# tomvanbraeckel/amv-codec-tools

Measured on AMD Instinct MI355X. Metric: AMV frames/sec/GPU (160x120 decode, bit-exact), higher is better.
Workload: dtype int32; 1 GPU; 160x120 AMV decode, 160000-frame synthetic stream per GPU, chunks resident in HBM; parallelism=frame-range x1, frames_per_gpu=160000, stream=seeded synthetic source (BASELINE.md section 4), every frame

## Files before the change

### amv-codec-tools_amd/__init__.py

```python
import ctypes
import os

_HERE = os.path.dirname(os.path.abspath(__file__))
LIB_PATH = os.environ.get("AMVHIP_LIB") or os.path.join(_HERE, "libamvhip.so")

OK, ERR_ARG, ERR_DEVICE, ERR_NOMEM, ERR_SPACE = 0, -1, -2, -3, -4
ST_FORMAT, ST_OVERRUN, ST_TRUNCATED = 1, 2, 4
FLAG_ZIGZAG_FIXED = 1
FLAG_FFMPEG = 2
FLAG_FFMPEG_KEEP = 4
QBIAS_AMV, QBIAS_MJPEG = 0, 128
K_HUFFMAN, K_RECON, K_FDCT, K_PACK, K_ADPCM_DEC, K_ADPCM_ENC, K_SYNTH, K_HUFFMAN_SERIAL, K_UNSTUFF, K_PACK_SERIAL, K_COMPACT = range(11)
K_AUDIO_RESAMPLE = 11
K_PIXFMT = 12
(PIX_YUV420P, PIX_YUVJ420P, PIX_YUV422P, PIX_YUVJ422P, PIX_YUV444P, PIX_YUVJ444P, PIX_YUYV422, PIX_UYVY422, PIX_RGB24, PIX_BGR24,
 PIX_RGB32, PIX_RGB565, PIX_RGB555, PIX_GRAY8) = range(14)
PIX_COUNT = 14
AUDIO_RATE_MIN, AUDIO_RATE_MAX = 1000, 192000
ENTROPY_AUTO, ENTROPY_SERIAL = 0, 1

_vp, _u8p = ctypes.c_void_p, ctypes.c_void_p
_u32, _u64, _i32, _int = ctypes.c_uint32, ctypes.c_uint64, ctypes.c_int32, ctypes.c_int


class AMVInfo(ctypes.Structure):
    _fields_ = [("dwMicroSecPerFrame", ctypes.c_uint), ("dwWidth", ctypes.c_uint), ("dwHeight", ctypes.c_uint),
                ("dwSpeed", ctypes.c_uint), ("dwTimeSec", ctypes.c_uint), ("dwTimeMin", ctypes.c_uint),
                ("dwTimeHour", ctypes.c_uint), ("wFormatTag", ctypes.c_ushort), ("nChannels", ctypes.c_ushort),
                ("nSamplesPerSec", ctypes.c_uint), ("nAvgBytesPerSec", ctypes.c_uint),
                ("nBlockAlign", ctypes.c_ushort), ("wBitsPerSample", ctypes.c_ushort),
                ("cbSize", ctypes.c_ushort), ("wSamplesPerBlock", ctypes.c_ushort)]


class FRAMEBUFF(ctypes.Structure):
    _fields_ = [("videobuff", ctypes.POINTER(ctypes.c_ubyte)), ("audiobuff", ctypes.POINTER(ctypes.c_ubyte)),
                ("videobufflen", ctypes.c_uint), ("audiobufflen", ctypes.c_uint), ("framenum", ctypes.c_int)]


class VIDEOBUFF(ctypes.Structure):
    _fields_ = [("fbmpdat", ctypes.POINTER(ctypes.c_ubyte)), ("len", ctypes.c_uint)]


class AUDIOBUFF(ctypes.Structure):
    _fields_ = [("audiodata", ctypes.POINTER(ctypes.c_short)), ("len", ctypes.c_uint)]


class AMVDecoder(ctypes.Structure):
    _fields_ = [("amvfilename", ctypes.c_char_p), ("opened", ctypes.c_int), ("dataseekpos", ctypes.c_long),
                ("fileseekpos", ctypes.c_long), ("amvinfo", AMVInfo), ("currentframe", ctypes.c_uint),
                ("totalframe", ctypes.c_uint), ("framebuf", FRAMEBUFF), ("videobuf", VIDEOBUFF),
                ("audiobuf", AUDIOBUFF)]


class ADPCMChannelStatus(ctypes.Structure):
    _fields_ = [("predictor", ctypes.c_int), ("step_index", ctypes.c_short), ("step", ctypes.c_int),
                ("prev_sample", ctypes.c_int)]


class ADPCMContext(ctypes.Structure):
    _fields_ = [("channel", ctypes.c_int), ("status", ADPCMChannelStatus * 2), ("sample_buffer", ctypes.c_short * 32)]


SYMBOLS = {
    "PrepareForVideoDecode": (None, [ctypes.POINTER(AMVInfo)]),
    "AmvJpegDecode": (_int, [ctypes.POINTER(AMVInfo), ctypes.POINTER(FRAMEBUFF), ctypes.POINTER(VIDEOBUFF)]),
    "AdpcmImaDecodeFrame": (_int, [ctypes.POINTER(ADPCMContext), _vp, ctypes.POINTER(_int), _vp, _int]),
    "AdpcmImaEncodeFrame": (_int, [ctypes.POINTER(ADPCMContext), _int, _int, _vp, _int, _vp]),
    "AmvOpen": (ctypes.POINTER(AMVDecoder), [ctypes.c_char_p]),
    "AmvClose": (None, [ctypes.POINTER(AMVDecoder)]),
    "AmvReadNextFrame": (_int, [ctypes.POINTER(AMVDecoder)]),
    "AmvRewindFrameStart": (_int, [ctypes.POINTER(AMVDecoder)]),
    "AmvVideoDecode": (_int, [ctypes.POINTER(AMVDecoder)]),
    "AmvAudioDecode": (_int, [ctypes.POINTER(AMVDecoder)]),
    "AmvJpegPutHeader": (None, [_vp, ctypes.c_ushort, ctypes.c_ushort]),
    "AmvCreateJpegFileFromFrameBuffer": (_int, [ctypes.POINTER(AMVDecoder), ctypes.c_char_p]),
    "AmvCreateJpegFileFromBuffer": (_int, [ctypes.POINTER(AMVInfo), ctypes.POINTER(FRAMEBUFF), ctypes.c_char_p]),
    "AmvConvertJpegFileToBmpFile": (_int, [ctypes.c_char_p, ctypes.c_char_p]),
    "ConvertJpegFileToBmpFile": (_int, [ctypes.c_char_p, ctypes.c_char_p]),
    "AmvCreateWavFileFromAmvFile": (_int, [ctypes.POINTER(AMVDecoder), _int, ctypes.c_char_p]),
    "decode_amv_frame": (_int, [_vp, ctypes.c_uint, ctypes.c_uint, ctypes.c_uint, _vp]),
    "encode_amv_frame": (_int, [_vp, ctypes.c_uint, ctypes.c_uint, ctypes.c_uint, _int, _vp, ctypes.c_uint]),
    "amvhip_create": (_int, [ctypes.POINTER(_vp), _int]),
    "amvhip_destroy": (None, [_vp]),
    "amvhip_last_error": (ctypes.c_char_p, [_vp]),
    "amvhip_device": (_int, [_vp]),
    "amvhip_stride": (_u32, [_u32]),
    "amvhip_frame_bytes": (_u64, [_u32, _u32]),
    "amvhip_yuv420_frame_bytes": (_u64, [_u32, _u32]),
    "amvhip_encode_bound": (_u32, [_u32, _u32]),
    "amvhip_jpeg_header": (_u32, [ctypes.c_ushort, ctypes.c_ushort, _vp, _u32]),
    "amvhip_decode_batch_dev": (_int, [_vp, _vp, _u64, _vp, _vp, _u32, _u32, _u32, _u32, _vp, _vp, _vp]),
    "amvhip_decode_submit_dev": (_int, [_vp, _vp, _u64, _vp, _vp, _u32, _u32, _u32, _u32, _vp, _vp, _vp]),
    "amvhip_decode_collect_dev": (_int, [_vp, _vp]),
    "amvhip_decode_workspace_per_frame": (ctypes.c_double, [_vp]),
    "amvhip_decode_batch": (_int, [_vp, _vp, _u64, _vp, _vp, _u32, _u32, _u32, _u32, _vp, _vp]),
    "amvhip_decode_batch_async": (_int, [_vp, _vp, _u64, _vp, _vp, _u32, _u32, _u32, _u32, _vp, _vp]),
    "amvhip_sync": (_int, [_vp]),
    "amvhip_host_alloc": (_int, [_vp, ctypes.POINTER(_vp), ctypes.c_size_t]),
    "amvhip_host_free": (None, [_vp, _vp]),
    "amvhip_huffman_decode_dev": (_int, [_vp, _vp, _u64, _vp, _vp, _u32, _u32, _u32, _vp, _vp, _vp, _vp]),
    "amvhip_reconstruct_dev": (_int, [_vp, _vp, _vp, _u32, _u32, _u32, _u32, _vp, _vp]),
    "amvhip_encode_batch_dev": (_int, [_vp, _vp, _u32, _int, _u32, _u32, _u32, _u32, _vp, _u64, _vp, _vp, _vp]),
    "amvhip_encode_batch": (_int, [_vp, _vp, _u32, _int, _u32, _u32, _u32, _u32, _vp, _u64, _vp, _vp]),
    "amvhip_encode_yuv420_batch_dev": (_int, [_vp, _vp, _vp, _vp, _u32, _u32, _u64, _u64, _u32, _u32, _u32, _u32, _vp, _u64, _vp, _vp, _vp]),
    "amvhip_encode_yuv422_batch_dev": (_int, [_vp, _vp, _vp, _vp, _u32, _u32, _u64, _u64, _u32, _u32, _u32, _u32, _vp, _u64, _vp, _vp, _vp]),
    "amvhip_encode_yuv420_batch": (_int, [_vp, _vp, _vp, _vp, _u32, _u32, _u64, _u64, _u32, _u32, _u32, _u32, _vp, _u64, _vp, _vp]),
    "amvhip_encode_yuv422_batch": (_int, [_vp, _vp, _vp, _vp, _u32, _u32, _u64, _u64, _u32, _u32, _u32, _u32, _vp, _u64, _vp, _vp]),
    "amvhip_encode_nr_max": (_u32, [_u32, _u32]),
    "amvhip_encode_yuv420_nr_stream_dev": (_int, [_vp, _vp, _vp, _vp, _u32, _u32, _u64, _u64, _u32, _u32, _u32, _u32, _u32, _vp, _vp, _u64, _vp, _vp, _vp]),
    "amvhip_encode_yuv420_nr_stream": (_int, [_vp, _vp, _vp, _vp, _u32, _u32, _u64, _u64, _u32, _u32, _u32, _u32, _u32, _vp, _vp, _u64, _vp, _vp]),
    "amvhip_encode_nr_stream_dev": (_int, [_vp, _vp, _u32, _int, _u32, _u32, _u32, _u32, _u32, _vp, _vp, _u64, _vp, _vp, _vp]),
    "amvhip_encode_nr_stream": (_int, [_vp, _vp, _u32, _int, _u32, _u32, _u32, _u32, _u32, _vp, _vp, _u64, _vp, _vp]),
    "amvhip_resample_yuv420_dev": (_int, [_vp, _vp, _vp, _vp, _u32, _u32, _u64, _u64, _u32, _u32, _vp, _vp, _vp, _u32, _u32, _u64, _u64, _u32, _u32, _u32, _vp]),
    "amvhip_encode_yuv420_scaled_batch_dev": (_int, [_vp, _vp, _vp, _vp, _u32, _u32, _u64, _u64, _u32, _u32, _u32, _u32, _u32, _u32, _vp, _u64, _vp, _vp, _vp]),
    "amvhip_img_convert_supported": (_int, [_int, _int, _u32, _u32]),
    "amvhip_pix_frame_bytes": (_u64, [_int, _u32, _u32]),
    "amvhip_img_convert_dev": (_int, [_vp, _int, _vp, _vp, _vp, _u32, _u32, _u64, _u64, _int, _vp, _vp, _vp, _u32, _u32, _u64, _u64, _u32, _u32, _u32, _vp]),
    "amvhip_img_convert": (_int, [_vp, _int, _vp, _vp, _vp, _u32, _u32, _u64, _u64, _int, _vp, _vp, _vp, _u32, _u32, _u64, _u64, _u32, _u32, _u32]),
    "amvhip_sws_scale_dev": (_int, [_vp, _int, _vp, _vp, _vp, _u32, _u32, _u64, _u64, _u32, _u32, _int, _vp, _vp, _vp, _u32, _u32, _u64, _u64, _u32, _u32, _u32, _vp]),
    "amvhip_encode_fmt_scaled_batch_dev": (_int, [_vp, _int, _vp, _vp, _vp, _u32, _u32, _u64, _u64, _u32, _u32, _u32, _u32, _u32, _u32, _vp, _u64, _vp, _vp, _vp]),
    "amvhip_pad_color_from_rgb": (None, [_u32, _vp]),
    "amvhip_deinterlace_supported": (_int, [_int, _u32, _u32]),
    "amvhip_deinterlace_dev": (_int, [_vp, _int, _vp, _vp, _vp, _u32, _u32, _u64, _u64, _vp, _vp, _vp, _u32, _u32, _u64, _u64, _u32, _u32, _u32, _vp]),
    "amvhip_deinterlace": (_int, [_vp, _int, _vp, _vp, _vp, _u32, _u32, _u64, _u64, _vp, _vp, _vp, _u32, _u32, _u64, _u64, _u32, _u32, _u32]),
    "amvhip_video_frontend_dev": (_int, [_vp, _int, _vp, _vp, _vp, _u32, _u32, _u64, _u64, _u32, _u32, _u32, _vp, _vp, _vp, _vp, _u32, _u32, _u64, _u64, _u32, _u32, _vp]),
    "amvhip_encode_frontend_batch_dev": (_int, [_vp, _int, _vp, _vp, _vp, _u32, _u32, _u64, _u64, _u32, _u32, _u32, _vp, _u32, _u32, _u32, _vp, _u64, _vp, _vp, _vp]),
    "amvhip_decode_fmt_batch_dev": (_int, [_vp, _vp, _u64, _vp, _vp, _u32, _u32, _u32, _u32, _int, _vp, _u32, _vp, _vp]),
    "amvhip_lowres_dim": (_u32, [_u32, _u32]),
    "amvhip_lowres_frame_bytes": (_u64, [_u32, _u32, _u32]),
    "amvhip_decode_lowres_batch_dev": (_int, [_vp, _vp, _u64, _vp, _vp, _u32, _u32, _u32, _u32, _u32, _int, _vp, _u32, _vp, _vp]),
    "amvhip_decode_lowres_batch": (_int, [_vp, _vp, _u64, _vp, _vp, _u32, _u32, _u32, _u32, _u32, _int, _vp, _u32, _vp]),
    "amvhip_reconstruct_lowres_dev": (_int, [_vp, _vp, _vp, _u32, _u32, _u32, _u32, _vp, _vp]),
    "amvhip_audio_resample_out_samples": (_u64, [_u32, _u32, _u64]),
    "amvhip_audio_resample_batch_dev": (_int, [_vp, _vp, _vp, _vp, _u32, _u32, _u32, _vp, _vp, _u32, _u32, _vp]),
    "amvhip_audio_resample_batch": (_int, [_vp, _vp, _u64, _vp, _vp, _u32, _u32, _u32, _vp, _u64, _vp, _u32, _u32]),
    "amvhip_audio_resample_init": (_vp, [_vp, _int, _int, _int, _int]),
    "amvhip_audio_resample": (_int, [_vp, _vp, _vp, _int]),
    "amvhip_audio_resample_close": (None, [_vp]),
    "amvhip_encode_coefs_dev": (_int, [_vp, _vp, _u32, _int, _u32, _u32, _u32, _u32, _vp, _vp]),
    "amvhip_adpcm_decode_batch_dev": (_int, [_vp, _vp, _u64, _vp, _vp, _u32, _vp, _vp, _vp, _vp]),
    "amvhip_adpcm_encode_batch_dev": (_int, [_vp, _vp, _vp, _vp, _u32, _vp, _vp, _vp, _vp]),
    "amvhip_adpcm_decode_batch": (_int, [_vp, _vp, _u64, _vp, _vp, _u32, _vp, _u64, _vp, _vp]),
    "amvhip_adpcm_decode_batch_async": (_int, [_vp, _vp, _u64, _vp, _vp, _u32, _vp, _u64, _vp, _vp]),
    "amvhip_adpcm_encode_batch": (_int, [_vp, _vp, _u64, _vp, _vp, _u32, _vp, _vp, _u64, _vp]),
    "amvhip_adpcm_encode_frame": (_int, [_vp, _vp, _u32, ctypes.POINTER(_i32), _vp, _u32]),
    "amvhip_adpcm_encode_trellis_batch_dev": (_int, [_vp, _vp, _vp, _vp, _u32, _vp, _u32, _vp, _vp, _vp, _vp]),
    "amvhip_adpcm_encode_frame_trellis": (_int, [_vp, _vp, _u32, ctypes.POINTER(_i32), _u32, _vp, _u32]),
    "amvhip_adpcm_encode_trellis_stream_dev": (_int, [_vp, _vp, _vp, _vp, _u32, _i32, _u32, _vp, _vp, _vp, _vp]),
    "amvhip_adpcm_encode_trellis_stream": (_int, [_vp, _vp, _u64, _vp, _vp, _u32, _i32, _u32, _vp, _u64, _vp, _vp]),
    "amvhip_adpcm_trellis_chain_stats": (_int, [_vp, _vp]),
    "amvhip_amv_audio_pairs": (_u32, [_u32, _u32, ctypes.POINTER(_u32), ctypes.POINTER(_u64)]),
    "amvhip_amv_audio_frame_size": (_u32, [_u32, _u32, _u32]),
    "amvhip_adpcm_wav_encode_frame": (_int, [_vp, _vp, _int, _vp, _vp, _int]),
    "amvhip_synth_frames_dev": (_int, [_vp, _u32, _u32, _u32, _u32, _u32, _vp, _vp]),
    "amvhip_synth_audio_dev": (_int, [_vp, _u32, _u64, _u64, _vp, _vp]),
    "amvhip_set_entropy_mode": (_int, [_vp, _int]),
    "amvhip_entropy_stats": (_int, [_vp, _int, _vp]),
    "amvhip_entropy_trace": (_int, [_vp, _vp, _u32]),
    "amvhip_decode_split_stats": (_int, [_vp, _vp]),
    "amvhip_adpcm_chain_stats": (_int, [_vp, _vp]),
    "amvhip_adpcm_quotient_table": (None, [_vp]),
    "amvhip_prof_enable": (None, [_vp, _int]),
    "amvhip_prof_reset": (None, [_vp]),
    "amvhip_prof_read": (_int, [_vp, _int, ctypes.POINTER(_u64), ctypes.POINTER(ctypes.c_double)]),
    "amvhip_kernel_name": (ctypes.c_char_p, [_int]),
    "amvhip_mux_open": (_vp, [ctypes.c_char_p, _u32, _u32, _u32, _u32, _u32, _u32]),
    "amvhip_mux_write_frame": (_int, [_vp, _u8p, _u32, _u8p, _u32]),
    "amvhip_mux_close": (_int, [_vp]),
}

_lib = None


def load_library():
    global _lib
    if _lib is None:
        if not os.path.exists(LIB_PATH):
            raise RuntimeError(
                "libamvhip.so is not built (%s). Run `python amv-codec-tools_amd/build.py`; there is no CPU fallback."
                % LIB_PATH)
        try:
            import torch
        except ImportError:
            pass
        lib = ctypes.CDLL(LIB_PATH)
        for name, (res, args) in SYMBOLS.items():
            fn = getattr(lib, name)
            fn.restype = res
            fn.argtypes = args
        _lib = lib
    return _lib


class AmvHipError(RuntimeError):
    pass


class Frontend(ctypes.Structure):
    _fields_ = [("deinterlace", _u32), ("crop_top", _u32), ("crop_bottom", _u32), ("crop_left", _u32), ("crop_right", _u32),
                ("pad_top", _u32), ("pad_bottom", _u32), ("pad_left", _u32), ("pad_right", _u32), ("pad_color", ctypes.c_uint8 * 3)]

    def __init__(self, deinterlace=0, crop=(0, 0, 0, 0), pad=(0, 0, 0, 0), pad_color=(16, 128, 128)):
        super().__init__(int(deinterlace), *crop, *pad, (ctypes.c_uint8 * 3)(*pad_color))


def pad_color_from_rgb(rrggbb):
    out = (ctypes.c_uint8 * 3)()
    load_library().amvhip_pad_color_from_rgb(rrggbb, ctypes.cast(out, ctypes.c_void_p))
    return tuple(out)


def _ptr(x):
    if x is None:
        return None
    if isinstance(x, int):
        return x
    if hasattr(x, "data_ptr"):
        return x.data_ptr()
    if hasattr(x, "ctypes"):
        return x.ctypes.data
    if isinstance(x, bytes):
        return ctypes.cast(ctypes.c_char_p(x), ctypes.c_void_p).value
    raise TypeError("pass a torch tensor, numpy array, bytes or int address, not %s" % type(x).__name__)


class Context:

    def __init__(self, device=0):
        self.lib = load_library()
        h = ctypes.c_void_p()
        rc = self.lib.amvhip_create(ctypes.byref(h), int(device))
        if rc != OK:
            raise AmvHipError("amvhip_create(device=%d) failed with %d: no usable HIP device" % (device, rc))
        self.h = h

    def close(self):
        if getattr(self, "h", None):
            self.lib.amvhip_destroy(self.h)
            self.h = None

    __del__ = close

    def _check(self, rc, what):
        if rc < 0:
            raise AmvHipError("%s failed (%d): %s" % (what, rc, self.lib.amvhip_last_error(self.h).decode()))
        return rc

    def stride(self, w):
        return self.lib.amvhip_stride(w)

    def frame_bytes(self, w, h):
        return self.lib.amvhip_frame_bytes(w, h)

    def yuv420_frame_bytes(self, w, h):
        return self.lib.amvhip_yuv420_frame_bytes(w, h)

    def encode_bound(self, w, h):
        return self.lib.amvhip_encode_bound(w, h)

    def decode_batch_dev(self, blob, blob_bytes, offs, lens, n, w, h, flags, out, status, stream=None):
        return self._check(self.lib.amvhip_decode_batch_dev(self.h, _ptr(blob), blob_bytes, _ptr(offs), _ptr(lens), n,
                                                            w, h, flags, _ptr(out), _ptr(status), stream), "decode_batch_dev")

    def decode_submit_dev(self, blob, blob_bytes, offs, lens, n, w, h, flags, out, status, stream=None):
        return self._check(self.lib.amvhip_decode_submit_dev(self.h, _ptr(blob), blob_bytes, _ptr(offs), _ptr(lens), n,
                                                             w, h, flags, _ptr(out), _ptr(status), stream), "decode_submit_dev")

    def decode_collect_dev(self, stream=None):
        return self._check(self.lib.amvhip_decode_collect_dev(self.h, stream), "decode_collect_dev")

    def decode_workspace_per_frame(self):
        return self.lib.amvhip_decode_workspace_per_frame(self.h)

    def huffman_decode_dev(self, blob, blob_bytes, offs, lens, n, w, h, coef, status, nmcu_ok, stream=None):
        return self._check(self.lib.amvhip_huffman_decode_dev(self.h, _ptr(blob), blob_bytes, _ptr(offs), _ptr(lens), n,
                                                              w, h, _ptr(coef), _ptr(status), _ptr(nmcu_ok), stream),
                           "huffman_decode_dev")

    def reconstruct_dev(self, coef, nmcu_ok, n, w, h, flags, out, stream=None):
        return self._check(self.lib.amvhip_reconstruct_dev(self.h, _ptr(coef), _ptr(nmcu_ok), n, w, h, flags,
                                                           _ptr(out), stream), "reconstruct_dev")

    def encode_batch_dev(self, pix, pix_stride, is_bgr, n, w, h, qbias, blob, blob_cap, offs, lens, stream=None):
        return self._check(self.lib.amvhip_encode_batch_dev(self.h, _ptr(pix), pix_stride, is_bgr, n, w, h, qbias,
                                                            _ptr(blob), blob_cap, _ptr(offs), _ptr(lens), stream),
                           "encode_batch_dev")

    def encode_yuv420_batch_dev(self, y, cb, cr, y_stride, c_stride, y_frame, c_frame, n, w, h, qbias, blob, blob_cap, offs,
                                lens, stream=None):
        return self._check(self.lib.amvhip_encode_yuv420_batch_dev(self.h, _ptr(y), _ptr(cb), _ptr(cr), y_stride, c_stride,
                                                                   y_frame, c_frame, n, w, h, qbias, _ptr(blob), blob_cap,
                                                                   _ptr(offs), _ptr(lens), stream), "encode_yuv420_batch_dev")

    def encode_nr_max(self, w, h):
        return self.lib.amvhip_encode_nr_max(w, h)

    def encode_yuv420_nr_stream_dev(self, y, cb, cr, y_stride, c_stride, y_frame, c_frame, n, w, h, qbias, nr, state, blob, blob_cap,
                                    offs, lens, stream=None):
        return self._check(self.lib.amvhip_encode_yuv420_nr_stream_dev(self.h, _ptr(y), _ptr(cb), _ptr(cr), y_stride, c_stride,
                                                                       y_frame, c_frame, n, w, h, qbias, nr, _ptr(state), _ptr(blob),
                                                                       blob_cap, _ptr(offs), _ptr(lens), stream),
                           "encode_yuv420_nr_stream_dev")

    def encode_yuv420_nr_stream(self, y, cb, cr, y_stride, c_stride, y_frame, c_frame, n, w, h, qbias, nr, state, blob, blob_cap, offs,
                                lens):
        return self._check(self.lib.amvhip_encode_yuv420_nr_stream(self.h, _ptr(y), _ptr(cb), _ptr(cr), y_stride, c_stride,
                                                                   y_frame, c_frame, n, w, h, qbias, nr, _ptr(state), _ptr(blob),
                                                                   blob_cap, _ptr(offs), _ptr(lens)), "encode_yuv420_nr_stream")

    def encode_nr_stream_dev(self, pix, pix_stride, is_bgr, n, w, h, qbias, nr, state, blob, blob_cap, offs, lens, stream=None):
        return self._check(self.lib.amvhip_encode_nr_stream_dev(self.h, _ptr(pix), pix_stride, is_bgr, n, w, h, qbias, nr,
                                                                _ptr(state), _ptr(blob), blob_cap, _ptr(offs), _ptr(lens), stream),
# ... 35 lines not shown
                           "adpcm_encode_batch_dev")

    def adpcm_encode_trellis_stream_dev(self, pcm, pcm_offs, nsamp, n, first_step_index, trellis, blob, offs, step_out=None,
                                        stream=None):
        return self._check(self.lib.amvhip_adpcm_encode_trellis_stream_dev(self.h, _ptr(pcm), _ptr(pcm_offs), _ptr(nsamp), n,
                                                                           first_step_index, trellis, _ptr(blob), _ptr(offs),
                                                                           _ptr(step_out), stream),
                           "adpcm_encode_trellis_stream_dev")

    @staticmethod
    def _pic(pic):
        planes, stride, c_stride, frame, c_frame = pic
        planes = list(planes) + [None] * (3 - len(planes))
        return [_ptr(planes[0]), _ptr(planes[1]), _ptr(planes[2]), stride, c_stride, frame, c_frame]

    def img_convert_dev(self, src_fmt, src, dst_fmt, dst, w, h, n, stream=None):
        return self._check(self.lib.amvhip_img_convert_dev(self.h, src_fmt, *self._pic(src), dst_fmt, *self._pic(dst), w, h, n, stream),
                           "img_convert_dev")

    def img_convert(self, src_fmt, src, dst_fmt, dst, w, h, n):
        return self._check(self.lib.amvhip_img_convert(self.h, src_fmt, *self._pic(src), dst_fmt, *self._pic(dst), w, h, n), "img_convert")

    def sws_scale_dev(self, src_fmt, src, src_w, src_h, dst_fmt, dst, dst_w, dst_h, n, stream=None):
        return self._check(self.lib.amvhip_sws_scale_dev(self.h, src_fmt, *self._pic(src), src_w, src_h, dst_fmt, *self._pic(dst),
                                                         dst_w, dst_h, n, stream), "sws_scale_dev")

    def encode_fmt_scaled_batch_dev(self, src_fmt, src, src_w, src_h, n, w, h, qbias, blob, blob_cap, offs, lens, stream=None):
        return self._check(self.lib.amvhip_encode_fmt_scaled_batch_dev(self.h, src_fmt, *self._pic(src), src_w, src_h, n, w, h, qbias,
                                                                       _ptr(blob), blob_cap, _ptr(offs), _ptr(lens), stream),
                           "encode_fmt_scaled_batch_dev")

    @staticmethod
    def _fe(fe):
        return None if fe is None else ctypes.addressof(fe)

    def pad_color_from_rgb(self, rrggbb):
        return pad_color_from_rgb(rrggbb)

    def deinterlace_supported(self, fmt, w, h):
        return self.lib.amvhip_deinterlace_supported(fmt, w, h)

    def deinterlace_dev(self, fmt, src, dst, w, h, n, stream=None):
        return self._check(self.lib.amvhip_deinterlace_dev(self.h, fmt, *self._pic(src), *self._pic(dst), w, h, n, stream), "deinterlace_dev")

    def deinterlace(self, fmt, src, dst, w, h, n):
        return self._check(self.lib.amvhip_deinterlace(self.h, fmt, *self._pic(src), *self._pic(dst), w, h, n), "deinterlace")

    def video_frontend_dev(self, src_fmt, src, src_w, src_h, n, fe, dst, w, h, stream=None):
        return self._check(self.lib.amvhip_video_frontend_dev(self.h, src_fmt, *self._pic(src), src_w, src_h, n, self._fe(fe), *self._pic(dst),
                                                              w, h, stream), "video_frontend_dev")

    def encode_frontend_batch_dev(self, src_fmt, src, src_w, src_h, n, fe, w, h, qbias, blob, blob_cap, offs, lens, stream=None):
        return self._check(self.lib.amvhip_encode_frontend_batch_dev(self.h, src_fmt, *self._pic(src), src_w, src_h, n, self._fe(fe), w, h,
                                                                     qbias, _ptr(blob), blob_cap, _ptr(offs), _ptr(lens), stream),
                           "encode_frontend_batch_dev")

    def decode_fmt_batch_dev(self, blob, blob_bytes, offs, lens, n, w, h, flags, dst_fmt, out, out_stride, status, stream=None):
        return self._check(self.lib.amvhip_decode_fmt_batch_dev(self.h, _ptr(blob), blob_bytes, _ptr(offs), _ptr(lens), n, w, h, flags,
                                                                dst_fmt, _ptr(out), out_stride, _ptr(status), stream),
                           "decode_fmt_batch_dev")

    def lowres_dim(self, full, lowres):
        return self.lib.amvhip_lowres_dim(full, lowres)

    def lowres_frame_bytes(self, w, h, lowres):
        return self.lib.amvhip_lowres_frame_bytes(w, h, lowres)

    def decode_lowres_batch_dev(self, blob, blob_bytes, offs, lens, n, w, h, flags, lowres, dst_fmt, out, out_stride, status, stream=None):
        return self._check(self.lib.amvhip_decode_lowres_batch_dev(self.h, _ptr(blob), blob_bytes, _ptr(offs), _ptr(lens), n, w, h, flags,
                                                                   lowres, dst_fmt, _ptr(out), out_stride, _ptr(status), stream),
                           "decode_lowres_batch_dev")

    def decode_lowres_batch(self, blob, blob_bytes, offs, lens, n, w, h, flags, lowres, dst_fmt, out, out_stride, status):
        return self._check(self.lib.amvhip_decode_lowres_batch(self.h, _ptr(blob), blob_bytes, _ptr(offs), _ptr(lens), n, w, h, flags,
                                                               lowres, dst_fmt, _ptr(out), out_stride, _ptr(status)), "decode_lowres_batch")

    def reconstruct_lowres_dev(self, coef, nmcu_ok, n, w, h, lowres, out, stream=None):
        return self._check(self.lib.amvhip_reconstruct_lowres_dev(self.h, _ptr(coef), _ptr(nmcu_ok), n, w, h, lowres, _ptr(out), stream),
                           "reconstruct_lowres_dev")

    def audio_resample_out_samples(self, in_rate, out_rate, in_samples):
        return audio_resample_out_samples(in_rate, out_rate, in_samples)

    def audio_resample_batch_dev(self, pcm, pcm_offs, nsamp, n, in_channels, in_rate, out, out_offs, out_channels, out_rate,
                                 stream=None):
        return self._check(self.lib.amvhip_audio_resample_batch_dev(self.h, _ptr(pcm), _ptr(pcm_offs), _ptr(nsamp), n,
                                                                    in_channels, in_rate, _ptr(out), _ptr(out_offs),
                                                                    out_channels, out_rate, stream), "audio_resample_batch_dev")

    def audio_resampler(self, output_channels, input_channels, output_rate, input_rate):
        return AudioResampler(self, output_channels, input_channels, output_rate, input_rate)

    def synth_frames_dev(self, seed, first, n, w, h, rgb, stream=None):
        return self._check(self.lib.amvhip_synth_frames_dev(self.h, seed, first, n, w, h, _ptr(rgb), stream), "synth_frames_dev")

    def synth_audio_dev(self, seed, first, n, pcm, stream=None):
        return self._check(self.lib.amvhip_synth_audio_dev(self.h, seed, first, n, _ptr(pcm), stream), "synth_audio_dev")

    def decode_batch(self, blob, blob_bytes, offs, lens, n, w, h, flags, out, status):
        return self._check(self.lib.amvhip_decode_batch(self.h, _ptr(blob), blob_bytes, _ptr(offs), _ptr(lens), n, w, h,
                                                        flags, _ptr(out), _ptr(status)), "decode_batch")

    def encode_batch(self, pix, pix_stride, is_bgr, n, w, h, qbias, blob, blob_cap, offs, lens):
        return self._check(self.lib.amvhip_encode_batch(self.h, _ptr(pix), pix_stride, is_bgr, n, w, h, qbias, _ptr(blob),
                                                        blob_cap, _ptr(offs), _ptr(lens)), "encode_batch")

    def adpcm_decode_batch(self, blob, blob_bytes, offs, lens, n, pcm, pcm_samples, pcm_offs, final_state=None):
        return self._check(self.lib.amvhip_adpcm_decode_batch(self.h, _ptr(blob), blob_bytes, _ptr(offs), _ptr(lens), n,
                                                              _ptr(pcm), pcm_samples, _ptr(pcm_offs), _ptr(final_state)),
                           "adpcm_decode_batch")

    def adpcm_encode_batch(self, pcm, pcm_samples, pcm_offs, nsamp, n, step_in, blob, blob_bytes, offs):
        return self._check(self.lib.amvhip_adpcm_encode_batch(self.h, _ptr(pcm), pcm_samples, _ptr(pcm_offs), _ptr(nsamp),
                                                              n, _ptr(step_in), _ptr(blob), blob_bytes, _ptr(offs)),
                           "adpcm_encode_batch")

    def adpcm_encode_trellis_stream(self, pcm, pcm_samples, pcm_offs, nsamp, n, first_step_index, trellis, blob, blob_bytes, offs,
                                    step_out=None):
        return self._check(self.lib.amvhip_adpcm_encode_trellis_stream(self.h, _ptr(pcm), pcm_samples, _ptr(pcm_offs), _ptr(nsamp),
                                                                       n, first_step_index, trellis, _ptr(blob), blob_bytes,
                                                                       _ptr(offs), _ptr(step_out)),
                           "adpcm_encode_trellis_stream")

    def audio_resample_batch(self, pcm, pcm_samples, pcm_offs, nsamp, n, in_channels, in_rate, out, out_samples, out_offs,
                             out_channels, out_rate):
        return self._check(self.lib.amvhip_audio_resample_batch(self.h, _ptr(pcm), pcm_samples, _ptr(pcm_offs), _ptr(nsamp), n,
                                                                in_channels, in_rate, _ptr(out), out_samples, _ptr(out_offs),
                                                                out_channels, out_rate), "audio_resample_batch")

    def set_entropy_mode(self, mode):
        return self._check(self.lib.amvhip_set_entropy_mode(self.h, mode), "set_entropy_mode")

    def entropy_stats(self, enable=True):
        out = (ctypes.c_uint64 * 10)()
        self._check(self.lib.amvhip_entropy_stats(self.h, 1 if enable else 0, out), "entropy_stats")
        waves = max(out[9], 1)
        return {"frames": out[0], "rounds": out[1], "max_rounds": out[2], "handed_to_serial": out[3], "waves": out[9],
                "clocks_per_wave": {"zero": out[4] / waves, "first_walk": out[5] / waves, "sync_rounds": out[6] / waves,
                                    "write": out[7] / waves, "dc": out[8] / waves}}

    def entropy_trace(self, tasks):
        import numpy as np
        out = np.zeros((tasks, 8), np.uint64)
        got = self.lib.amvhip_entropy_trace(self.h, out.ctypes.data, tasks)
        if got < 0:
            self._check(got, "entropy_trace")
        return out[:got]

    def decode_split_stats(self):
        out = (ctypes.c_uint32 * 2)()
        self._check(self.lib.amvhip_decode_split_stats(self.h, out), "decode_split_stats")
        return {"heavy": int(out[0]), "light": int(out[1])}

    def adpcm_chain_stats(self):
        out = (ctypes.c_uint32 * 64)()
        self._check(self.lib.amvhip_adpcm_chain_stats(self.h, out), "adpcm_chain_stats")
        rec = list(out[1:63])
        while rec and rec[-1] == 0:
            rec.pop()
        return {"exhaustive": bool(out[0]), "recoded": rec}

    def adpcm_trellis_chain_stats(self):
        out = (ctypes.c_uint32 * 64)()
        self._check(self.lib.amvhip_adpcm_trellis_chain_stats(self.h, out), "adpcm_trellis_chain_stats")
        rec = list(out[1:63])
        while rec and rec[-1] == 0:
            rec.pop()
        return {"exhaustive": bool(out[0]), "recoded": rec}

    def prof_enable(self, on=True):
        self.lib.amvhip_prof_enable(self.h, 1 if on else 0)

    def prof_reset(self):
        self.lib.amvhip_prof_reset(self.h)

    def prof_read(self, kernel):
        n, ms = ctypes.c_uint64(), ctypes.c_double()
        self.lib.amvhip_prof_read(self.h, kernel, ctypes.byref(n), ctypes.byref(ms))
        return n.value, ms.value

    def kernel_name(self, kernel):
        return self.lib.amvhip_kernel_name(kernel).decode()


def audio_resample_out_samples(in_rate, out_rate, in_samples):
    return load_library().amvhip_audio_resample_out_samples(in_rate, out_rate, in_samples)


class AudioResampler:

    def __init__(self, ctx, output_channels, input_channels, output_rate, input_rate):
        self.ctx, self.out_ch, self.in_ch = ctx, output_channels, input_channels
        self.ratio = ctypes.c_float(ctypes.c_float(output_rate).value / ctypes.c_float(input_rate).value).value
        self.h = ctx.lib.amvhip_audio_resample_init(ctx.h, output_channels, input_channels, output_rate, input_rate)
        if not self.h:
            raise AmvHipError("amvhip_audio_resample_init failed: %s" % ctx.lib.amvhip_last_error(ctx.h).decode())

    def resample(self, pcm):
        import numpy as np
        pcm = np.ascontiguousarray(pcm, np.int16)
        nb = pcm.size // self.in_ch
        out = np.zeros((int(4 * nb * self.ratio) + 18) * self.out_ch, np.int16)
        got = self.ctx._check(self.ctx.lib.amvhip_audio_resample(self.h, out.ctypes.data, pcm.ctypes.data, nb), "audio_resample")
        return out[:got * self.out_ch]

    def close(self):
        if getattr(self, "h", None):
            self.ctx.lib.amvhip_audio_resample_close(self.h)
            self.h = None

    __del__ = close
```

### amv-codec-tools_amd/build.py

```python
import concurrent.futures
import os
import shutil
import subprocess
import sys

HERE = os.path.dirname(os.path.abspath(__file__))
OUT = os.path.join(HERE, "libamvhip.so")
OBJ = os.path.join(HERE, "build")
ARCH = "gfx950"

HIP_SOURCES = ["csrc/amv_decode.hip", "csrc/amv_decode_sync.hip", "csrc/amv_reconstruct.hip", "csrc/amv_reconstruct_ff.hip", "csrc/amv_reconstruct_lowres.hip", "csrc/amv_encode.hip", "csrc/amv_encode_par.hip", "csrc/amv_encode_nr.hip", "csrc/amv_resample.hip", "csrc/amv_pixfmt.hip", "csrc/amv_frontend.hip", "csrc/amv_audio_resample.hip", "csrc/amv_adpcm.hip", "csrc/amv_synth.hip",
               "csrc/amvhip_context.hip", "csrc/amvhip_decode.hip", "csrc/amvhip_encode.hip", "csrc/amvhip_pixfmt.hip", "csrc/amvhip_audio.hip"]
C_SOURCES = ["host/amvlib_compat.c", "host/amv_container.c"]
HEADERS = ["csrc/amv_tables.h", "csrc/amv_kernels.h", "csrc/amv_block_load.h", "csrc/amv_piece_map.h", "csrc/amv_segment.h", "csrc/amv_ff_dequant.h", "csrc/amv_encode_common.h", "csrc/amv_host_plan.h", "csrc/amv_nr_plan.h",
           "csrc/amvhip_ctx.h", "../include/amvhip.h"]

HIPFLAGS = ["-O3", "-std=c++17", "-fPIC", "-fwrapv", "-fno-strict-aliasing", f"--offload-arch={ARCH}",
            "-Wall", "-Wno-unused-function"]
CFLAGS = ["-O2", "-fPIC", "-Wall", "-Wextra", "-std=gnu11"]


def _hipcc():
    for cand in (shutil.which("hipcc"), "/opt/rocm/bin/hipcc"):
        if cand and os.path.exists(cand):
            return cand
    raise RuntimeError("hipcc not found: libamvhip.so cannot be built (there is no CPU fallback)")


def _stale(target, deps):
    if not os.path.exists(target):
        return True
    t = os.path.getmtime(target)
    return any(os.path.getmtime(d) > t for d in deps)


def _run(cmd):
    p = subprocess.run(cmd, cwd=HERE, capture_output=True, text=True)
    if p.returncode != 0:
        raise RuntimeError("command failed: %s\n%s\n%s" % (" ".join(cmd), p.stdout, p.stderr))
    return p.stderr


def build(force=False, verbose=False):
    os.makedirs(OBJ, exist_ok=True)
    hipcc = _hipcc()
    hdrs = [os.path.join(HERE, h) for h in HEADERS] + [os.path.abspath(__file__)]
    jobs = []
    objs = []
    for src in HIP_SOURCES:
        o = os.path.join(OBJ, os.path.basename(src) + ".o")
        objs.append(o)
        if force or _stale(o, [os.path.join(HERE, src)] + hdrs):
            jobs.append([hipcc] + HIPFLAGS + ["-c", src, "-o", o])
    for src in C_SOURCES:
        o = os.path.join(OBJ, os.path.basename(src) + ".o")
        objs.append(o)
        if force or _stale(o, [os.path.join(HERE, src)] + hdrs):
            jobs.append(["gcc"] + CFLAGS + ["-c", src, "-o", o])
    if jobs:
        with concurrent.futures.ThreadPoolExecutor(max_workers=4) as ex:
            for warn in ex.map(_run, jobs):
                if verbose and warn:
                    sys.stderr.write(warn)
    if jobs or force or _stale(OUT, objs):
        _run([hipcc, "-shared", "-fPIC", f"--offload-arch={ARCH}", "-o", OUT] + objs + ["-lpthread"])
    return OUT


if __name__ == "__main__":
    print(build(force="--force" in sys.argv, verbose=True))
```

### amv-codec-tools_amd/csrc/amv_block_load.h

```cpp
#pragma once
#include <cstdlib>

#include "amv_kernels.h"
#include "amv_piece_map.h"

namespace amv {

constexpr uint32_t kSegImageBytes = 60u * 128u;
constexpr uint32_t kScatterSwizzleMask = 0x38u;
constexpr uint32_t kScatterFieldShift = 6u;
constexpr uint32_t kScatterAddressMask = 0x11ffeu;

__device__ __forceinline__ void seg_sync() {
    __builtin_amdgcn_fence(__ATOMIC_SEQ_CST, "wavefront");
    __builtin_amdgcn_wave_barrier();
}

__device__ __forceinline__ bool select_frame(const FrameSel& sel, uint32_t n, uint32_t item, uint32_t& f, uint32_t& slot) {
    f = slot = item;
    if (!sel.round) return true;
    const uint32_t p = sel.base + item;
    if (item >= sel.round || p >= (sel.count ? *sel.count : n)) return false;
    f = sel.list ? sel.list[p] : p;
    return true;
}

struct Segment {
    uint32_t f, slot;
    uint32_t m0, cnt, ok, mcu0;
    uint32_t segidx, nsegs;
};
__device__ __forceinline__ Segment segment_of(uint32_t f, uint32_t slot, const uint32_t* __restrict__ nmcu_ok, const FrameGeom& g,
                                              uint32_t nseg, uint32_t my, uint32_t seg) {
    const uint32_t m0 = seg * kSegMcus;
    return {f, slot, m0, min(kSegMcus, g.mcu_cols - m0), nmcu_ok[f], my * g.mcu_cols + m0, my * nseg + seg, g.mcu_rows * nseg};
}
template <bool kRound>
__device__ __forceinline__ bool next_item(const PieceMap& pm, uint32_t& item) {
    if (!kRound) return false;
    seg_sync();
    item += piece_stride(pm);
    return true;
}

__device__ __forceinline__ bool load_segment_blocks(const SyncSinks& in, const Segment& sg, bool dense_only, const FrameGeom& g,
                                                    uint32_t lane, uint8_t* s_img, uint32_t (&c)[32], bool& skip) {
    const uint32_t f = sg.f, slot = sg.slot, segidx = sg.segidx, nsegs = sg.nsegs, mcu0 = sg.mcu0, cnt = sg.cnt, ok = sg.ok;
    const uint32_t nb = cnt * 6u;
    uint32_t rc = 0xffffffffu, r0 = 0u, r1 = 0u;
    if (in.rec != nullptr && !dense_only) {
        const uint32_t* ss = in.seg_start + ((uint64_t)f * (nsegs + 1u) + segidx) * 2u;
        rc = in.rec_count[f];
        r0 = ss[0];
        r1 = ss[3];
    }
    const bool records = rc != 0xffffffffu;
    skip = !records && in.rec != nullptr && !dense_only;
    if (skip) return false;
    int dc_base = 0;
    if (records) {
        const uint32_t ok_blocks = in.ok_in_blocks ? ok : ok * 6u;
        const uint32_t blocks_ok_here = ok_blocks > mcu0 * 6u ? min(nb, ok_blocks - mcu0 * 6u) : 0u;
        if (!blocks_ok_here) r1 = r0;
        struct __attribute__((packed, aligned(4))) Rec4 { uint32_t w[4]; };
        constexpr uint32_t kAhead = 3;
        const uint32_t* rec = in.rec + (uint64_t)in.rec_line[f] * 32u + r0;
        const uint32_t nrec = r1 - r0;
        Rec4 q[kAhead];
#pragma unroll
        for (uint32_t j = 0; j < kAhead; ++j) {
            const uint32_t i = j * 4u * kWave + lane * 4u;
            q[j] = Rec4{{kDummyRecord, kDummyRecord, kDummyRecord, kDummyRecord}};
            if (i < nrec) q[j] = *reinterpret_cast<const Rec4*>(rec + i);
        }
        uint4* img16 = reinterpret_cast<uint4*>(s_img);
        for (uint32_t i = lane; i < nb * 8u; i += kWave) img16[i] = make_uint4(0, 0, 0, 0);
        seg_sync();
        const uint32_t field0 = (mcu0 * 6u - g.blocks) & 63u;
        const uint32_t first6 = (uint32_t)__builtin_amdgcn_readfirstlane((int)((64u - field0) << kScatterFieldShift));
        const uint32_t ok7 = blocks_ok_here << 7;
        const uint32_t spare = kSegImageBytes + lane * 2u;
        for (uint32_t base = 0;;) {
#pragma unroll
            for (uint32_t j = 0; j < kAhead; ++j) {
                if (base + j * 4u * kWave >= nrec) break;
                if (base + (j + 1u) * 4u * kWave > nrec) {
                    const int32_t left = (int32_t)(nrec - base - j * 4u * kWave) - (int32_t)(lane * 4u);
#pragma unroll
                    for (uint32_t e = 0; e < 4u; ++e)
                        if (left <= (int32_t)e) q[j].w[e] = kDummyRecord;
                }
#pragma unroll
                for (uint32_t e = 0; e < 4u; ++e) {
                    const uint32_t w = q[j].w[e];
                    uint32_t t;
                    asm("v_add_lshl_u32 %0, %1, %2, 1" : "=v"(t) : "v"(w ^ ((w >> 3) & kScatterSwizzleMask)), "s"(first6));
                    const uint32_t at = t & kScatterAddressMask;
                    *reinterpret_cast<int16_t*>(s_img + (at < ok7 ? at : spare)) = (int16_t)(w >> 16);
                }
            }
            base += kAhead * 4u * kWave;
            if (base >= nrec) break;
#pragma unroll
            for (uint32_t j = 0; j < kAhead; ++j) {
                const uint32_t i = base + j * 4u * kWave + lane * 4u;
                if (i < nrec) q[j] = *reinterpret_cast<const Rec4*>(rec + i);
            }
        }
        const uint32_t frame_lanes = ((rc >> 24) & 63u) + 1u;
        if (frame_lanes > 1u) {
            const uint32_t babs = mcu0 * 6u + lane, k6 = lane % 6u;
            const uint4 ent = lane < frame_lanes ? reinterpret_cast<const uint4*>(in.lane_tab)[(uint64_t)f * in.lanes + lane]
                                                 : make_uint4(0xffffffffu, 0u, 0u, 0u);
            uint32_t at = 0u;
#pragma unroll
            for (uint32_t step = 32u; step >= 1u; step >>= 1) {
                const uint32_t probe = at + step;
                const uint32_t first = (uint32_t)__shfl((int)ent.x, (int)(probe & 63u));
                if (probe < frame_lanes && first <= babs) at = probe;
            }
            const int by = __shfl((int)ent.y, (int)at), bu = __shfl((int)ent.z, (int)at), bv = __shfl((int)ent.w, (int)at);
            dc_base = at ? (k6 < 4u ? by : (k6 == 4u ? bu : bv)) : 0;
        }
        seg_sync();
    }
    if (lane >= nb) return false;
    if (records) {
        const uint4* src = reinterpret_cast<const uint4*>(s_img) + lane * 8u;
        const uint32_t swz = (lane + mcu0 * 6u - g.blocks) & 7u;
#pragma unroll
        for (int i = 0; i < 8; ++i) {
            const uint4 q = src[(uint32_t)i ^ swz];
            c[4 * i] = q.x; c[4 * i + 1] = q.y; c[4 * i + 2] = q.z; c[4 * i + 3] = q.w;
        }
        c[0] = (c[0] & 0xffff0000u) | ((c[0] + (uint32_t)dc_base) & 0xffffu);
    } else {
        const uint4* src = reinterpret_cast<const uint4*>(in.coef + (((uint64_t)slot * g.mcus + mcu0) * 6u + lane) * 64u);
#pragma unroll
        for (int i = 0; i < 8; ++i) {
            const uint4 q = src[i];
            c[4 * i] = q.x; c[4 * i + 1] = q.y; c[4 * i + 2] = q.z; c[4 * i + 3] = q.w;
        }
    }
    return true;
}

__device__ __forceinline__ int coef_at(const uint32_t (&c)[32], int i) {
    return (i & 1) ? ((int)c[i >> 1] >> 16) : (int)(int16_t)(c[i >> 1] & 0xffffu);
}

template <class Kernel, class... Tail>
static inline void launch_segments(Kernel part, Kernel walk, uint32_t block, uint32_t row_groups, const SyncSinks& sinks, const uint32_t* nmcu_ok,
                            uint32_t n, const FrameSel& sel, uint32_t items, const FrameGeom& g, hipStream_t s, Tail... tail) {
    for_each_launch(row_groups, segs_per_row(g), items, sel.round != 0u, [&](const PieceMap& pm, uint32_t grid) {
        hipLaunchKernelGGL(sel.round ? walk : part, dim3(grid), dim3(block), 0, s, sinks, nmcu_ok, n, sel, g, pm, tail...);
    });
}

}
```

### amv-codec-tools_amd/csrc/amv_decode_sync.hip

```cpp
#include <atomic>

#include "amv_kernels.h"
#include "amv_segment.h"

namespace amv {

namespace {

constexpr uint32_t kRingWords = 16;
constexpr uint32_t kNever = 0xffffffffu;

__device__ __forceinline__ void wave_sync() {
    __builtin_amdgcn_fence(__ATOMIC_SEQ_CST, "wavefront");
    __builtin_amdgcn_wave_barrier();
}

template <int kWidth>
__device__ __forceinline__ uint32_t seg_excl_sum(uint32_t v, uint32_t sub, uint32_t& total) {
    uint32_t x = v;
#pragma unroll
    for (int d = 1; d < kWidth; d <<= 1) {
        const uint32_t y = __shfl_up(x, d, kWidth);
        if (sub >= (uint32_t)d) x += y;
    }
// ... 145 lines not shown
        }
    }
    if (lane == 0) {
        ws_bytes[frame] = retry ? kNever : total;
        if (retry) retry_list[atomicAdd(retry_count, 1u)] = frame;
    }
}

namespace {

struct Stream {
    const uint32_t* g;
    uint32_t nwords;
    uint32_t* ring;
    uint32_t hi;
    uint4 pf0, pf1;
};

constexpr int kStrideWrite = 8;

__device__ __forceinline__ uint4 stream_piece(const Stream& s, uint32_t x) {
    uint4 v = make_uint4(0, 0, 0, 0);
    if (x < s.nwords) v = *reinterpret_cast<const uint4*>(s.g + x);
    return v;
}

__device__ __forceinline__ void stream_request(Stream& s) {
    s.pf0 = stream_piece(s, s.hi);
    s.pf1 = stream_piece(s, s.hi + 4u);
}

struct SegGeom {
    uint32_t mcu_cols;
    uint32_t per_row;
    uint32_t count;
};

template <uint32_t kFlush>
__device__ __forceinline__ void stage_put(uint32_t* stage, uint32_t pos, uint32_t word) {
    stage[(pos & (2u * kFlush - 1u)) * kWave] = word;
}

template <uint32_t kFlush>
__device__ __forceinline__ void stage_flush(const uint32_t* stage, uint32_t* __restrict__ rec, uint32_t from, uint32_t rec_cap) {
    const uint32_t* p = stage + (from & (2u * kFlush - 1u)) * kWave;
    uint4 v[kFlush / 4u];
#pragma unroll
    for (uint32_t q = 0; q < kFlush / 4u; ++q)
        v[q] = make_uint4(p[(4u * q) * kWave], p[(4u * q + 1u) * kWave], p[(4u * q + 2u) * kWave], p[(4u * q + 3u) * kWave]);
    if (from + kFlush <= rec_cap) {
#pragma unroll
        for (uint32_t q = 0; q < kFlush / 4u; ++q) *reinterpret_cast<uint4*>(rec + from + 4u * q) = v[q];
    }
}

}

struct SyncOut {
    uint32_t* rec;
    const uint32_t* rec_line;
    uint32_t* seg_start;
    uint32_t* lane_tab;
    SegGeom sg;
    uint32_t lane_stride;
    uint32_t* rec_count;
    uint32_t* retry_list;
    uint32_t* retry_count;
    uint32_t ok_in_blocks;
};


namespace {

constexpr uint32_t kFastRegion = kFastWords * 4u;
constexpr uint32_t kFastTableBytes = 4u * kFastRegion;
constexpr uint32_t kServicePace = 4u;
template <int L> constexpr uint32_t skip_pace() { return L >= 16 ? 1u : kServicePace; }
constexpr uint32_t kSlot = kWave * 4u;
constexpr uint32_t kFastRingBytes = (kRingWords + 1u) * kSlot;
constexpr uint32_t kFastSumBytes = 4u * kSlot;
constexpr uint32_t fast_stage_bytes(uint32_t flush) { return 2u * flush * kSlot; }
constexpr uint32_t fast_per_wave(uint32_t flush) { return fast_stage_bytes(flush) + kFastSumBytes + kFastRingBytes; }
constexpr uint32_t fast_waves(uint32_t flush) {
    const uint32_t w = (160u * 1024u - kFastTableBytes) / fast_per_wave(flush);
    return w > 16u ? 16u : w;
}

struct FastState {
    uint32_t t;
    uint32_t k;
    uint32_t j;
    uint32_t togo6;
    uint32_t rp8;
    uint32_t dc;
};

typedef __attribute__((address_space(3))) uint32_t lds_u32;
__device__ __forceinline__ uint32_t lds_get(uint32_t a) { return *(const lds_u32*)(uintptr_t)a; }
__device__ __forceinline__ void lds_put(uint32_t a, uint32_t v) { *(lds_u32*)(uintptr_t)a = v; }
__device__ __forceinline__ uint32_t shl3_add(uint32_t x, uint32_t y) {
    uint32_t d;
    asm("v_lshl_add_u32 %0, %1, 3, %2" : "=v"(d) : "v"(x), "v"(y));
    return d;
}

__device__ __forceinline__ void fast_ring_put(const Stream& s, uint32_t x, const uint4& v) {
    uint32_t* d = s.ring + (x & (kRingWords - 1u)) * kWave;
    d[0] = v.x; d[kWave] = v.y; d[2 * kWave] = v.z; d[3 * kWave] = v.w;
    if ((x & (kRingWords - 1u)) == 0u) s.ring[kRingWords * kWave] = v.x;
}

__device__ __forceinline__ void fast_open(Stream& s) {
    const uint4 a = stream_piece(s, 0u), b = stream_piece(s, 4u), c = stream_piece(s, 8u), d = stream_piece(s, 12u);
    fast_ring_put(s, 0u, a);
    fast_ring_put(s, 4u, b);
    fast_ring_put(s, 8u, c);
    fast_ring_put(s, 12u, d);
    s.hi = kRingWords;
    stream_request(s);
}

template <uint32_t kPace>
__device__ __forceinline__ void fast_service_paced(Stream& s, uint32_t w, bool alive, bool& have, uint32_t stride_no) {
    if (alive && w + 9u > s.hi) {
        do {
            if (!have) stream_request(s);
            fast_ring_put(s, s.hi, s.pf0);
            fast_ring_put(s, s.hi + 4u, s.pf1);
            s.hi += 8u;
            have = false;
        } while (w + 9u > s.hi);
    }
    if ((stride_no & (kPace - 1u)) == 0u) {
        if (alive && !have) {
            stream_request(s);
            have = true;
        }
    }
}

__device__ __forceinline__ uint32_t fast_window(uint32_t ringb, uint32_t t) {
    const uint32_t ra = shl3_add(t & 0x1e0u, ringb);
    return __builtin_amdgcn_alignbit(lds_get(ra), lds_get(ra + kSlot), ~t);
}

__device__ __forceinline__ uint32_t fast_lookup(const FastState& s, uint32_t v) {
    const uint32_t toff = (((3u * kFastRegion) >> s.j) & kFastRegion) | (~s.dc & (2u * kFastRegion));
    const uint32_t e1 = lds_get(((v >> 21) & 0x7fcu) | toff);
    const uint32_t x2 = max(v >> 16, kFastLongFirst - 1u);
    const uint32_t e2 = lds_get((x2 << 2) + (toff + (kFastM2Word * 4u - 4u * (kFastLongFirst - 1u))));
    return e1 | e2;
}

template <uint32_t kFlush, bool kLimit>
__device__ __forceinline__ void fast_stride(uint32_t ringb, uint32_t stageb, uint32_t sumb, uint32_t lim1, FastState& s, uint32_t& seen,
                                            uint32_t& worst) {
#pragma unroll
    for (int it = 0; it < kStrideWrite; ++it) {
        const uint32_t ca = (((2u * kSlot) >> s.j) & (3u * kSlot)) | sumb;
        const uint32_t sum = lds_get(ca);
        const uint32_t v = fast_window(ringb, s.t);
        __builtin_amdgcn_sched_barrier(0);
        uint32_t run = (uint32_t)((int32_t)s.togo6 >> 31);
        if (kLimit) run &= (uint32_t)((int32_t)(s.t - lim1) >> 31);
        const uint32_t e = fast_lookup(s, v) & run;
        seen |= e;
        const uint32_t used = e >> 24;
        const int x = __builtin_amdgcn_sbfe((int)v, 0u - used, e);
        const uint32_t full = __builtin_amdgcn_ubfe(0xffffffffu, 0u, e);
        const uint32_t val = (uint32_t)x - (full ^ (uint32_t)(x >> 31));
        s.t += used;
        const uint32_t kn = s.k + ((e >> 16) & 255u);
        worst = min(worst, kn - 65u);
        uint32_t dcn = (uint32_t)__builtin_amdgcn_sbfe((int)kn, 6u, 1u);
        asm("" : "+v"(dcn));
        lds_put(ca, sum + (val & s.dc));
        const uint32_t rv = val + (sum & s.dc);
        lds_put((s.rp8 & ((2u * kFlush - 1u) << 8)) | stageb, (rv << 16) | (s.togo6 & 0xfc0u) | (kn - 1u));
        s.rp8 += e & kFastEmit;
        s.k = kn & ~dcn;
        s.togo6 += kn & 64u;
        s.j = min(s.j + dcn, 5u);
        s.dc = dcn;
    }
}

template <bool kLimit>
__device__ __forceinline__ uint32_t fast_replay(uint32_t ringb, uint32_t lim1, FastState& s) {
    for (int it = 0; it < kStrideWrite; ++it) {
        if (s.togo6 == 0u) break;
        if (kLimit && (int32_t)(s.t - lim1) >= 0) break;
        const uint32_t e = fast_lookup(s, fast_window(ringb, s.t));
        if (e & kFastInvalid) return 1u;
        const uint32_t kn = s.k + ((e >> 16) & 255u);
        s.t += e >> 24;
        if (kn - 65u < 15u) return 2u;
        const bool end = (kn & 64u) != 0u;
        s.rp8 += e & kFastEmit;
        s.k = end ? 0u : kn;
        s.togo6 += kn & 64u;
        s.j = end ? (s.j == 0u ? 5u : s.j - 1u) : s.j;
        s.dc = end ? ~0u : 0u;
    }
    return 0u;
}

__device__ __forceinline__ void fast_open_at(Stream& s, uint32_t w) {
    const uint32_t lo = w & ~7u;
    const uint4 a = stream_piece(s, lo), b = stream_piece(s, lo + 4u), c = stream_piece(s, lo + 8u), d = stream_piece(s, lo + 12u);
    fast_ring_put(s, lo, a);
    fast_ring_put(s, lo + 4u, b);
    fast_ring_put(s, lo + 8u, c);
    fast_ring_put(s, lo + 12u, d);
    s.hi = lo + kRingWords;
    stream_request(s);
}

template <uint32_t kPace>
__device__ __forceinline__ void fast_skip(Stream& win, uint32_t ringb, FastState& s, uint32_t lim1, uint32_t& nblk6, uint32_t& nrec8) {
    nblk6 = nrec8 = 0u;
    bool active = (int32_t)(s.t - lim1) < 0;
    if (!__ballot(active)) return;
    fast_open_at(win, active ? (s.t + 1u) >> 5 : 0u);
    bool have = true;
    uint32_t stride_no = 1u;
    while (__ballot(active) != 0ull) {
        fast_service_paced<kPace>(win, (s.t + 1u) >> 5, active, have, stride_no++);
#pragma unroll
        for (int it = 0; it < kStrideWrite; ++it) {
            const uint32_t v = fast_window(ringb, s.t);
            const uint32_t e = fast_lookup(s, v) & (uint32_t)((int32_t)(s.t - lim1) >> 31);
            s.t += e >> 24;
            const uint32_t kn = s.k + ((e >> 16) & 255u);
            uint32_t dcn = (uint32_t)__builtin_amdgcn_sbfe((int)kn, 6u, 1u);
            asm("" : "+v"(dcn));
            nrec8 += e & kFastEmit;
            nblk6 += kn & 64u;
            s.k = kn & ~dcn;
            s.j = min(s.j + dcn, 5u);
            s.dc = dcn;
        }
        active = (int32_t)(s.t - lim1) < 0;
    }
}

}

template <uint32_t kFlush>
__global__ __launch_bounds__(kWave * 16) void amv_huffman_fast_kernel(
    const uint32_t* __restrict__ ws, const uint32_t* __restrict__ ws_bytes, uint32_t n,
    const uint32_t* __restrict__ list, const uint32_t* __restrict__ list_count,
    uint32_t blocks_per_frame, const uint32_t* __restrict__ ws_line,
    const HuffDecodeImage* __restrict__ img, SyncOut out, int32_t* __restrict__ status,
    uint32_t* __restrict__ nmcu_ok, uint32_t* __restrict__ queue, unsigned long long* __restrict__ stats) {
    static_assert(kFlush == 8u, "amv_huffman_fast_kernel stages a stride's eight record slots");
    extern __shared__ __attribute__((aligned(16))) uint8_t s_mem[];
    const uint32_t wave = threadIdx.x >> 6, lane = threadIdx.x & 63u, nwaves = blockDim.x >> 6;
    {
        const uint4* src = reinterpret_cast<const uint4*>(&img->fast[0][0]);
        uint4* dst = reinterpret_cast<uint4*>(s_mem);
        for (uint32_t i = threadIdx.x; i < kFastTableBytes / 16u; i += blockDim.x) dst[i] = src[i];
    }
    __syncthreads();
    const bool lds_at_zero = (uint32_t)(uintptr_t)(__attribute__((address_space(3))) uint8_t*)s_mem == 0u;
    const uint32_t stageb = kFastTableBytes + wave * fast_stage_bytes(kFlush) + lane * 4u;
    const uint32_t sumb = kFastTableBytes + nwaves * fast_stage_bytes(kFlush) + wave * kFastSumBytes + lane * 4u;
    const uint32_t ringb = kFastTableBytes + nwaves * (fast_stage_bytes(kFlush) + kFastSumBytes) + wave * kFastRingBytes + lane * 4u;
    uint32_t* const stage = reinterpret_cast<uint32_t*>(s_mem + stageb);
    if (list) n = *list_count;
    const uint32_t ntasks = (n + kWave - 1) / kWave;
    const SegGeom sg = out.sg;
    for (;;) {
        uint32_t task = 0;
        if (lane == 0) task = atomicAdd(queue, 1u);
        task = __shfl(task, 0);
        if (task >= ntasks) return;
        const uint32_t idx = task * kWave + lane;
        const uint32_t frame = idx < n ? (list ? list[idx] : idx) : kNever;
        uint32_t total = frame != kNever ? ws_bytes[frame] : kNever;
        if (!lds_at_zero && total != kNever) {
            out.retry_list[atomicAdd(out.retry_count, 1u)] = frame;
            total = kNever;
        }
        if (frame != kNever && total == kNever) out.rec_count[frame] = kNever;
        if (!lds_at_zero) continue;
        const bool live = total != kNever;
        const uint32_t fsafe = live ? frame : 0u;
        const uint32_t line0 = out.rec_line[fsafe];
        uint32_t* const rec = out.rec + (uint64_t)line0 * 32u;
        const uint32_t line1 = out.rec_line[fsafe + 1u];
        const uint32_t cap_rec = line1 > line0 ? (line1 - line0) * 32u : 0u;
        uint2* const seg_out = reinterpret_cast<uint2*>(out.seg_start) + (uint64_t)fsafe * (sg.count + 1u);
        const uint32_t valid_bits = live ? total * 8u : 0u;
        Stream win{ws + (uint64_t)ws_line[fsafe] * 4u, live ? ((total + 15u) >> 4) * 4u : 0u, reinterpret_cast<uint32_t*>(s_mem + ringb), 0u,
                   make_uint4(0, 0, 0, 0), make_uint4(0, 0, 0, 0)};
        fast_open(win);
        for (uint32_t c = 0; c < 3u; ++c) lds_put(sumb + c * kSlot, 0u);

        FastState s{0xffffffffu, 0u, 5u, live ? 0u - (blocks_per_frame << 6) : 0u, 0u, ~0u};
        bool alive = live;
        uint32_t stop = 0;
        uint32_t stride_no = 0;
        bool have_words = true;
        uint32_t recpos = 0;
        uint32_t seg_next = 0, seg_col = 0, seg_blk = 0;
        uint32_t end_blocks = 0;
#pragma unroll
        for (uint32_t q = 0; q < 2u * kFlush; ++q) stage_put<kFlush>(stage, q, kDummyRecord);
        if (__ballot(alive) != 0ull) do {
            const bool line_live = alive;
            uint4 line[8];
#pragma unroll
            for (int quarter = 0; quarter < 4; ++quarter) {
                fast_service_paced<kServicePace>(win, (s.t + 1u) >> 5, alive, have_words, stride_no);
                const bool running = alive;
                s.rp8 = stride_no << 11;
                const FastState start = s;
                uint32_t worst = ~0u, seen = 0u;
                fast_stride<kFlush, false>(ringb, stageb, sumb, 0u, s, seen, worst);
                const bool trouble = alive && (worst < 15u || (seen & kFastInvalid) != 0u);
                if (__ballot(trouble) != 0ull) {
                    if (trouble) {
                        s = start;
                        stop = fast_replay<false>(ringb, 0u, s);
                        alive = false;
                        for (uint32_t q = s.rp8 >> 8; q < stride_no * 8u + 8u; ++q) stage_put<kFlush>(stage, q, kDummyRecord);
                    }
                }
                if (alive && s.togo6 == 0u) { stop = 3u; alive = false; }
                stage_put<kFlush>(stage, s.rp8 >> 8, kDummyRecord);
                {
                    uint32_t* p = stage + ((stride_no & 1u) * kFlush) * kWave;
                    line[2 * quarter] = make_uint4(p[0], p[kWave], p[2 * kWave], p[3 * kWave]);
                    line[2 * quarter + 1] = make_uint4(p[4 * kWave], p[5 * kWave], p[6 * kWave], p[7 * kWave]);
#pragma unroll
                    for (uint32_t q = 0; q < 8u; ++q) p[q * kWave] = kDummyRecord;
                }
                bool hit = false;
                uint32_t blocks = 0;
                if (running) {
                    blocks = blocks_per_frame + (uint32_t)((int32_t)s.togo6 >> 6);
                    hit = seg_next < sg.count && blocks + (s.k ? 1u : 0u) > seg_blk;
                    if (!alive) { end_blocks = blocks; s.togo6 = 0u; }
                }
                if (__ballot(hit) != 0ull) {
                    if (hit) {
                        seg_out[seg_next++] = make_uint2(start.rp8 >> 8, s.rp8 >> 8);
                        const bool last = seg_col + 1u == sg.per_row;
                        seg_blk += 6u * (last ? sg.mcu_cols - seg_col * kSegMcus : kSegMcus);
                        seg_col = last ? 0u : seg_col + 1u;
                    }
                }
                ++stride_no;
            }
            if (line_live) {
                const uint32_t at = (stride_no - 4u) * 8u;
                if (at + 32u <= cap_rec) {
                    uint4* d = reinterpret_cast<uint4*>(rec + at);
#pragma unroll
                    for (int q = 0; q < 8; ++q) d[q] = line[q];
                }
                recpos = at + 32u;
            }
        } while (__ballot(alive) != 0ull);
        if (live) {
            const uint32_t bits = s.t + 1u + (stop == 1u ? 17u : 0u);
            uint32_t st = stop == 1u ? kStFormat : (stop == 2u ? kStOverrun : 0u);
            if (bits > valid_bits) st |= kStTruncated;
            reinterpret_cast<uint4*>(out.lane_tab)[(uint64_t)frame * out.lane_stride] = make_uint4(0u, 0u, 0u, 0u);
            for (uint32_t m = seg_next; m <= sg.count; ++m) seg_out[m] = make_uint2(recpos, recpos);
            if (stats) atomicAdd(&stats[0], 1ull);
            if (recpos > cap_rec) {
                out.rec_count[frame] = kNever;
                out.retry_list[atomicAdd(out.retry_count, 1u)] = frame;
            } else {
                status[frame] = (int32_t)st;
                nmcu_ok[frame] = out.ok_in_blocks ? end_blocks : end_blocks / 6u;
                out.rec_count[frame] = recpos;
            }
        }
    }
}

template <int L>
__global__ __launch_bounds__(kWave * 16) void amv_huffman_sync2_kernel(
    const uint32_t* __restrict__ ws, const uint32_t* __restrict__ ws_bytes, uint32_t n,
    const uint32_t* __restrict__ list, const uint32_t* __restrict__ list_count,
    uint32_t blocks_per_frame, const uint32_t* __restrict__ ws_line,
    const HuffDecodeImage* __restrict__ img, SyncOut out, int32_t* __restrict__ status,
    uint32_t* __restrict__ nmcu_ok, uint32_t* __restrict__ queue, unsigned long long* __restrict__ stats) {
    constexpr int kFrames = kWave / L;
    constexpr uint32_t kFlush = 8u;
    constexpr uint32_t kNoLimit = 0x7ffffffeu;
    extern __shared__ __attribute__((aligned(16))) uint8_t s_mem[];
    const uint32_t wave = threadIdx.x >> 6, lane = threadIdx.x & 63u, nwaves = blockDim.x >> 6;
    const uint32_t slot = lane / L, sub = lane % L;
    if (list && *list_count == 0u) return;
    {
        const uint4* src = reinterpret_cast<const uint4*>(&img->fast[0][0]);
        uint4* dst = reinterpret_cast<uint4*>(s_mem);
        for (uint32_t i = threadIdx.x; i < kFastTableBytes / 16u; i += blockDim.x) dst[i] = src[i];
    }
    __syncthreads();
    const bool lds_at_zero = (uint32_t)(uintptr_t)(__attribute__((address_space(3))) uint8_t*)s_mem == 0u;
    const uint32_t stageb = kFastTableBytes + wave * fast_stage_bytes(kFlush) + lane * 4u;
    const uint32_t sumb = kFastTableBytes + nwaves * fast_stage_bytes(kFlush) + wave * kFastSumBytes + lane * 4u;
    const uint32_t ringb = kFastTableBytes + nwaves * (fast_stage_bytes(kFlush) + kFastSumBytes) + wave * kFastRingBytes + lane * 4u;
    uint32_t* const stage = reinterpret_cast<uint32_t*>(s_mem + stageb);
    if (list) n = *list_count;
    const uint32_t ntasks = (n + kFrames - 1) / kFrames;
    const SegGeom sg = out.sg;
    for (;;) {
        uint32_t task = 0;
        if (lane == 0) task = atomicAdd(queue, 1u);
        task = __shfl(task, 0);
        if (task >= ntasks) return;

        const bool timing = stats != nullptr && lane == 0;
        unsigned long long tc[6] = {0, 0, 0, 0, 0, 0};
        unsigned long long wall0 = 0;
        if (timing) { tc[0] = tc[1] = clock64(); wall0 = wall_clock64(); }

        const uint32_t idx = task * kFrames + slot;
        const uint32_t frame = idx < n ? (list ? list[idx] : idx) : kNever;
        uint32_t total = frame != kNever ? ws_bytes[frame] : kNever;
        if (!lds_at_zero && total != kNever) {
            if (sub == 0) out.retry_list[atomicAdd(out.retry_count, 1u)] = frame;
            total = kNever;
        }
        if (frame != kNever && total == kNever && sub == 0) out.rec_count[frame] = kNever;
        if (!lds_at_zero) continue;
        const bool live = total != kNever;
        const uint32_t fsafe = live ? frame : 0u;
        const uint32_t line0 = out.rec_line[fsafe];
        uint32_t* const rec = out.rec + (uint64_t)line0 * 32u;
        const uint32_t line1 = out.rec_line[fsafe + 1u];
        const uint32_t cap_rec = line1 > line0 ? (line1 - line0) * 32u : 0u;
        uint2* const seg_out = reinterpret_cast<uint2*>(out.seg_start) + (uint64_t)fsafe * (sg.count + 1u);
        const uint32_t valid_bits = live ? total * 8u : 0u;
        Stream win{ws + (uint64_t)ws_line[fsafe] * 4u, live ? ((total + 15u) >> 4) * 4u : 0u, reinterpret_cast<uint32_t*>(s_mem + ringb), 0u,
                   make_uint4(0, 0, 0, 0), make_uint4(0, 0, 0, 0)};

        uint32_t S = ((valid_bits + L - 1) / L + 31u) & ~31u;
        if (S < 64u) S = 64u;
        constexpr uint32_t kMemo = 5u, kPend = 4u;
        constexpr uint32_t kGuess = 5u << 11;
        const uint32_t stage0 = stageb - lane * 4u, sum0 = sumb - lane * 4u, col0 = slot * L;
        const uint64_t seg = L == 64 ? ~0ull : (((1ull << (L & 63)) - 1ull) << (slot * L));
        auto col_addr = [&](uint32_t col, uint32_t w) { return (w < 16u ? stage0 + w * kSlot : sum0 + (w - 16u) * kSlot) + col * 4u; };
        const bool walks = live && sub != L - 1;
        uint32_t my_blocks6 = 0u, my_recs8 = 0u, seeded = 0u, rounds = 0u;
        lds_put(col_addr(lane, 19u), 0u);
        {
            FastState st{sub * S - 1u, 0u, 5u, 0u, 0u, ~0u};
            const uint32_t lim1 = walks ? (sub + 1u) * S - 1u : 0u;
            if (!walks) st.t = lim1;
            uint32_t b6, r8;
            fast_skip<skip_pace<L>()>(win, ringb, st, lim1, b6, r8);
            if (walks) {
                lds_put(col_addr(lane, 0u), kGuess | (((st.t - lim1) | (st.k << 5) | (st.j << 11)) << 16));
                lds_put(col_addr(lane, 1u), b6);
                lds_put(col_addr(lane, 2u), r8);
                lds_put(col_addr(lane, 19u), 1u);
            }
        }
        if (timing) tc[2] = clock64();
        constexpr uint32_t kNone = 7u;
        uint32_t final_at = kNone, final_code = kGuess;
        bool settled = !live;
        for (int round = 0; round < L + 1; ++round) {
            wave_sync();
            const uint32_t held = lds_get(col_addr(lane, 19u));
            const uint32_t left_n = sub ? lds_get(col_addr(lane - 1u, 19u)) : 0u;
            uint32_t mine[kMemo], cand[kMemo];
#pragma unroll
            for (uint32_t q = 0; q < kMemo; ++q) {
                const uint32_t a = lds_get(col_addr(lane, 3u * q)), b = lds_get(col_addr(sub ? lane - 1u : lane, 3u * q));
                mine[q] = q < held ? a : kNever;
                cand[q] = q < left_n ? b >> 16 : kNever;
            }
            uint32_t link = (kNone << 15) | (kNone << 18) | (kNone << 21);
#pragma unroll
            for (uint32_t qp = 0; qp < kMemo; ++qp) {
                uint32_t to = kNone;
#pragma unroll
                for (uint32_t q = 0; q < kMemo; ++q) to = (mine[q] != kNever && (mine[q] & 0xffffu) == cand[qp]) ? q : to;
                if (sub == L - 1) to = cand[qp] != kNever ? 0u : kNone;
                link |= to << (3u * qp);
            }
            if (sub == 0) link = 0u;
            if (!live) link = 0u;
#pragma unroll
            for (int d = 1; d < L; d <<= 1) {
                const uint32_t before = __shfl_up(link, d, L);
                uint32_t both = 0u;
#pragma unroll
                for (uint32_t f = 0; f < 8u; ++f) both |= ((link >> (3u * ((before >> (3u * f)) & 7u))) & 7u) << (3u * f);
                if (sub >= (uint32_t)d) link = both;
            }
            final_at = link & 7u;
            const uint32_t left_at = wave_shr1(final_at);
            settled = !live || final_at != kNone;
            const bool front = live && !settled && sub != 0 && left_at != kNone;
            if (sub == 0) final_code = kGuess;
            else {
#pragma unroll
                for (uint32_t q = 0; q < kMemo; ++q) if (left_at == q) final_code = cand[q];
            }
            const uint64_t open = __ballot(!settled);
            if (!open) break;
            if (open & seg) ++rounds;
            uint32_t p = 0u;
            if (walks && front) {
                lds_put(col_addr(lane, 15u), final_code);
                p = 1u;
            } else if (walks && !settled) {
                const uint32_t most = min(kMemo - min(held, kMemo), kPend);
                uint32_t taken[kPend] = {kNever, kNever, kNever, kNever};
#pragma unroll
                for (uint32_t qq = 0; qq < kMemo; ++qq) {
                    const uint32_t c = cand[kMemo - 1u - qq];
                    bool known = c == kNever;
#pragma unroll
                    for (uint32_t m = 0; m < kMemo; ++m) known = known || (mine[m] & 0xffffu) == c;
#pragma unroll
                    for (uint32_t m = 0; m < kPend; ++m) known = known || taken[m] == c;
                    if (!known && p < most) {
#pragma unroll
                        for (uint32_t m = 0; m < kPend; ++m) if (m == p) taken[m] = c;
                        lds_put(col_addr(lane, 15u + p), c);
                        ++p;
                    }
                }
                while (seeded < 5u && p + 1u < most) {
                    ++seeded;
                    lds_put(col_addr(lane, 15u + p), (5u - seeded) << 11);
                    ++p;
                }
            }
            const uint32_t extras = p ? p - 1u : 0u;
            const bool idle = live && p == 0u;
            uint32_t all_extras, all_idle;
            const uint32_t ex_at = seg_excl_sum<L>(extras, sub, all_extras);
            const uint32_t id_at = seg_excl_sum<L>(idle ? 1u : 0u, sub, all_idle);
            wave_sync();
            uint32_t owner = sub, rank = 0u;
            bool work = p != 0u;
            if (__ballot(all_extras != 0u) != 0ull) {
                uint32_t lo = 0u;
#pragma unroll
                for (int d = L >> 1; d >= 1; d >>= 1) {
                    const uint32_t probe = __shfl(ex_at, (int)(lo + (uint32_t)d), L);
                    if (lo + (uint32_t)d < (uint32_t)L && probe <= id_at) lo += (uint32_t)d;
                }
                const uint32_t lo_at = __shfl(ex_at, (int)lo, L), lo_n = __shfl(extras, (int)lo, L);
                if (idle && id_at < all_extras && id_at - lo_at < lo_n) { owner = lo; rank = id_at - lo_at + 1u; work = true; }
            }
            FastState st{0u, 0u, 5u, 0u, 0u, ~0u};
            uint32_t lim1 = 0u, code = 0u;
            if (work) {
                code = lds_get(col_addr(col0 + owner, 15u + rank));
                lim1 = (owner + 1u) * S - 1u;
                st.t = owner * S - 1u + (code & 31u);
                st.k = (code >> 5) & 63u;
                st.j = code >> 11;
                st.dc = st.k ? 0u : ~0u;
            }
            uint32_t b6 = 0u, r8 = 0u;
            fast_skip<skip_pace<L>()>(win, ringb, st, lim1, b6, r8);
            if (work) {
                const uint32_t arr = (st.t - lim1) | (st.k << 5) | (st.j << 11);
                uint32_t at = lds_get(col_addr(col0 + owner, 19u)) + rank;
                if (rank == 0u && front) at = min(at, kMemo - 1u);
                if (at < kMemo) {
                    lds_put(col_addr(col0 + owner, 3u * at), code | (arr << 16));
                    lds_put(col_addr(col0 + owner, 3u * at + 1u), b6);
                    lds_put(col_addr(col0 + owner, 3u * at + 2u), r8);
                }
            }
            wave_sync();
            if (p) {
                const uint32_t done = 1u + min(extras, all_idle > ex_at ? all_idle - ex_at : 0u);
                lds_put(col_addr(lane, 19u), min(held + done, kMemo));
            }
        }
        if (walks && final_at != kNone) {
            my_blocks6 = lds_get(col_addr(lane, 3u * final_at + 1u));
            my_recs8 = lds_get(col_addr(lane, 3u * final_at + 2u));
        }
        if (timing) tc[3] = clock64();
        static_assert(16 + 11 < 32, "an arrival's offset behind the share's end must fit the state code's five bits");
        FastState entry{sub * S - 1u + (final_code & 31u), (final_code >> 5) & 63u, final_code >> 11, 0u, 0u, 0u};
        entry.dc = entry.k ? 0u : ~0u;
        if (sub == L - 1 || !live) { my_blocks6 = 0u; my_recs8 = 0u; }
        const bool unsettled = (__ballot(!settled) & seg) != 0ull;

        uint32_t all_blocks, all_recs;
        const uint32_t blk0 = seg_excl_sum<L>(my_blocks6 >> 6, sub, all_blocks);
        const uint32_t rec0 = seg_excl_sum<L>(((my_recs8 >> 8) + kFlush - 1u) & ~(kFlush - 1u), sub, all_recs);

        for (uint32_t c = 0; c < 3u; ++c) lds_put(sumb + c * kSlot, 0u);
        FastState s = entry;
        s.togo6 = (blk0 - blocks_per_frame) << 6;
        s.rp8 = rec0 << 8;
        bool alive = live && blk0 < blocks_per_frame;
        if (!alive) s.togo6 = 0u;
        const uint32_t wlim1 = sub == L - 1 ? kNoLimit : (sub + 1u) * S - 1u;
        const uint32_t dc_first = blk0 + (s.k ? 1u : 0u);
        uint32_t stop = 0;
        uint32_t flushed = rec0;
        uint32_t end_blocks = 0;
        uint32_t seg_next, seg_col, seg_blk;
        {
            const uint32_t m_first = (dc_first + 5u) / 6u;
            uint32_t row = m_first / sg.mcu_cols;
            const uint32_t col = m_first - row * sg.mcu_cols;
            seg_col = (col + kSegMcus - 1u) / kSegMcus;
            if (seg_col >= sg.per_row) { ++row; seg_col = 0u; }
            seg_next = row * sg.per_row + seg_col;
            seg_blk = (row * sg.mcu_cols + seg_col * kSegMcus) * 6u;
        }
        if (__ballot(alive) != 0ull) {
        fast_open_at(win, alive ? (s.t + 1u) >> 5 : 0u);
        bool have_words = true;
        uint32_t stride_no = 1u;
        do {
            fast_service_paced<kServicePace>(win, (s.t + 1u) >> 5, alive, have_words, stride_no++);
            if ((s.rp8 >> 8) - flushed >= kFlush) {
                stage_flush<kFlush>(stage, rec, flushed, cap_rec);
                flushed += kFlush;
            }
            const bool running = alive;
            const FastState start = s;
            uint32_t worst = ~0u, seen = 0u;
            fast_stride<kFlush, true>(ringb, stageb, sumb, wlim1, s, seen, worst);
            const bool trouble = alive && (worst < 15u || (seen & kFastInvalid) != 0u);
            if (__ballot(trouble) != 0ull) {
                if (trouble) {
                    s = start;
                    stop = fast_replay<true>(ringb, wlim1, s);
                    alive = false;
                }
            }
            if (alive && s.togo6 == 0u) { stop = 3u; alive = false; }
            if (alive && (int32_t)(s.t - wlim1) >= 0) alive = false;
            bool hit = false;
            if (running) {
                const uint32_t blocks = blocks_per_frame + (uint32_t)((int32_t)s.togo6 >> 6);
                hit = seg_next < sg.count && blocks + (s.k ? 1u : 0u) > seg_blk;
                if (!alive) { end_blocks = blocks; s.togo6 = 0u; }
            }
            if (__ballot(hit) != 0ull) {
                if (hit) {
                    seg_out[seg_next++] = make_uint2(start.rp8 >> 8, s.rp8 >> 8);
                    const bool last = seg_col + 1u == sg.per_row;
                    seg_blk += 6u * (last ? sg.mcu_cols - seg_col * kSegMcus : kSegMcus);
                    seg_col = last ? 0u : seg_col + 1u;
                }
            }
        } while (__ballot(alive) != 0ull);
        }
        const uint32_t recpos = s.rp8 >> 8;
        {
            const uint32_t end = (recpos + kFlush - 1u) & ~(kFlush - 1u);
            for (uint32_t q = recpos; q < end; ++q) stage_put<kFlush>(stage, q, kDummyRecord);
            while (flushed < end) {
                stage_flush<kFlush>(stage, rec, flushed, cap_rec);
                flushed += kFlush;
            }
        }
        if (timing) tc[4] = clock64();
        const uint32_t err = stop == 1u ? kStFormat : (stop == 2u ? kStOverrun : 0u);
        const uint32_t stop_p = s.t + 1u + (stop == 1u ? 17u : 0u);
        const uint64_t stop_mask = __ballot(stop != 0u) & seg;
        uint32_t st = 0, good_blocks = blocks_per_frame, rec_total = 0, seg_seen = 0;
        int stop_lane = 0;
        if (stop_mask) {
            stop_lane = __builtin_ctzll(stop_mask);
            const uint32_t e = __shfl(err, stop_lane);
            const uint32_t eb = __shfl(end_blocks, stop_lane);
            const uint32_t sp = __shfl(stop_p, stop_lane);
            rec_total = __shfl(recpos, stop_lane);
            seg_seen = __shfl(seg_next, stop_lane);
            st = e;
            if (e) good_blocks = eb;
            if (sp > valid_bits) st |= kStTruncated;
        } else {
            st = kStFormat; good_blocks = 0;
        }

        uint32_t tot;
        const uint32_t by = seg_excl_sum<L>(lds_get(sumb), sub, tot);
        const uint32_t bu = seg_excl_sum<L>(lds_get(sumb + kSlot), sub, tot);
        const uint32_t bv = seg_excl_sum<L>(lds_get(sumb + 2u * kSlot), sub, tot);
        if (live) {
            const bool real = (int)lane <= stop_lane && blk0 < blocks_per_frame;
            reinterpret_cast<uint4*>(out.lane_tab)[(uint64_t)frame * out.lane_stride + sub] = make_uint4(real ? dc_first : kNever, by, bu, bv);
            for (uint32_t m = seg_seen + sub; m <= sg.count; m += L) seg_out[m] = make_uint2(rec_total, rec_total);
        }
        uint32_t wave_rounds = rounds;
        if (stats) {
#pragma unroll
            for (int off = 32; off; off >>= 1) wave_rounds = max(wave_rounds, (uint32_t)__shfl_xor((int)wave_rounds, off));
        }
        if (timing) {
            tc[5] = clock64();
            for (int q = 0; q < 5; ++q) atomicAdd(&stats[4 + q], tc[q + 1] - tc[q]);
            atomicAdd(&stats[9], 1ull);
            if (task < kTraceTasks) {
                unsigned long long* tr = stats + kTraceBase + (unsigned long long)task * 8ull;
                tr[0] = wall0;
                tr[1] = wall_clock64();
                for (int q = 0; q < 4; ++q) tr[2 + q] = tc[q + 2] - tc[q + 1];
                tr[6] = wave_rounds | (unsigned long long)S << 32;
                tr[7] = (unsigned long long)blockIdx.x << 32 | (unsigned long long)wave << 16 | (unsigned long long)L;
            }
        }
        if (live && sub == 0) {
            if (stats) {
                atomicAdd(&stats[0], 1ull);
                atomicAdd(&stats[1], (unsigned long long)rounds);
                atomicMax(&stats[2], (unsigned long long)rounds);
            }
            if (rec_total > cap_rec || unsettled) {
                out.rec_count[frame] = kNever;
                out.retry_list[atomicAdd(out.retry_count, 1u)] = frame;
            } else {
                status[frame] = (int32_t)st;
                nmcu_ok[frame] = out.ok_in_blocks ? good_blocks : good_blocks / 6u;
                out.rec_count[frame] = rec_total | ((uint32_t)(L - 1) << 24);
            }
        }
    }
}

namespace {

template <uint32_t kFlush>
void launch_fast(const uint32_t* ws, const uint32_t* ws_bytes, uint32_t n, const uint32_t* list,
                 const uint32_t* list_count, const FrameGeom& g, const uint32_t* ws_line,
                 const HuffDecodeImage* d_img, const SyncOut& out, int32_t* status, uint32_t* nmcu_ok,
                 uint32_t* queue, unsigned long long* stats, uint32_t cus, hipStream_t s) {
    constexpr uint32_t kMaxWaves = fast_waves(kFlush);
    static std::atomic<uint64_t> raised{0};
    int dev = 0;
    (void)hipGetDevice(&dev);
    const uint64_t bit = 1ull << (dev & 63);
    if (!(raised.load(std::memory_order_relaxed) & bit)) {
        (void)hipFuncSetAttribute(reinterpret_cast<const void*>(amv_huffman_fast_kernel<kFlush>),
                                  hipFuncAttributeMaxDynamicSharedMemorySize, (int)(kFastTableBytes + kMaxWaves * fast_per_wave(kFlush)));
        raised.fetch_or(bit, std::memory_order_relaxed);
    }
    const uint32_t tasks = (n + (uint32_t)kWave - 1u) / (uint32_t)kWave;
    uint32_t waves = (tasks + cus - 1u) / cus;
    if (waves < 4u) waves = 4u;
    if (waves > kMaxWaves) waves = kMaxWaves;
    const uint32_t grid = tasks < cus ? tasks : cus;
    hipLaunchKernelGGL((amv_huffman_fast_kernel<kFlush>), dim3(grid), dim3(kWave * waves), kFastTableBytes + waves * fast_per_wave(kFlush), s,
                       ws, ws_bytes, n, list, list_count, g.blocks, ws_line, d_img, out, status, nmcu_ok, queue, stats);
}

template <int L>
void launch_sync2(const uint32_t* ws, const uint32_t* ws_bytes, uint32_t n, const uint32_t* list,
                  const uint32_t* list_count, const FrameGeom& g, const uint32_t* ws_line,
                  const HuffDecodeImage* d_img, const SyncOut& out, int32_t* status, uint32_t* nmcu_ok,
                  uint32_t* queue, unsigned long long* stats, uint32_t cus, hipStream_t s) {
    constexpr uint32_t kMaxWaves = fast_waves(8u);
    static std::atomic<uint64_t> raised{0};
    int dev = 0;
    (void)hipGetDevice(&dev);
    const uint64_t bit = 1ull << (dev & 63);
    if (!(raised.load(std::memory_order_relaxed) & bit)) {
        (void)hipFuncSetAttribute(reinterpret_cast<const void*>(amv_huffman_sync2_kernel<L>),
                                  hipFuncAttributeMaxDynamicSharedMemorySize, (int)(kFastTableBytes + kMaxWaves * fast_per_wave(8u)));
        raised.fetch_or(bit, std::memory_order_relaxed);
    }
    const uint32_t tasks = (n + (uint32_t)(kWave / L) - 1u) / (uint32_t)(kWave / L);
    uint32_t waves = (tasks + cus - 1u) / cus;
    if (waves < 4u) waves = 4u;
    if (waves > kMaxWaves) waves = kMaxWaves;
    const uint32_t grid = tasks < cus ? tasks : cus;
    hipLaunchKernelGGL((amv_huffman_sync2_kernel<L>), dim3(grid), dim3(kWave * waves), kFastTableBytes + waves * fast_per_wave(8u), s, ws,
                       ws_bytes, n, list, list_count, g.blocks, ws_line, d_img, out, status, nmcu_ok, queue, stats);
}

}

int huffman_sync_lanes(uint32_t n, uint32_t cus, int wanted, uint64_t pixels) {
    if (wanted == 1 || wanted == 2 || wanted == 4 || wanted == 8 || wanted == 16 || wanted == 32 || wanted == 64) return wanted;
    if (n >= cus * 230u) return 1;
    if (n >= cus * 150u) return 2;
    const uint64_t resident = (uint64_t)cus * fast_waves(8u);
    if (pixels <= 30000u && (uint64_t)n * 8u > resident * 64u) return 2;
    int full = 8;
    while (full < 64 && (uint64_t)full * 25000u <= pixels) full *= 2;
    int fill = 8;
    if (n <= resident) fill = 64;
    else if (n <= 2u * resident) fill = 32;
    else if (n <= 4u * resident) fill = 16;
    int cap = 8;
    while (cap < 64 && (uint64_t)cap * 2u * 500u <= pixels) cap *= 2;
    if (n <= cus * 5u) cap = 64;
    if (fill > cap) fill = cap;
    return fill > full ? fill : full;
}

__global__ __launch_bounds__(256) void amv_split_kernel(const uint32_t* __restrict__ lens, uint32_t n, const uint32_t* __restrict__ ws_line,
                                                        uint32_t* __restrict__ heavy, uint32_t* __restrict__ light, uint32_t* __restrict__ count) {
    const uint32_t i = blockIdx.x * 256u + threadIdx.x, lane = threadIdx.x & 63u;
    const bool in = i < n;
    const uint64_t all = ws_line[n];
    const bool is_heavy = in && (((uint64_t)lens[in ? i : 0u] + 47u) >> 4) * n > 2u * all;
    const uint64_t hm = __ballot(is_heavy), lm = __ballot(in && !is_heavy);
    uint32_t hb = 0u, lb = 0u;
    if (lane == 0u) {
        if (hm) hb = atomicAdd(&count[0], (uint32_t)__builtin_popcountll(hm));
        if (lm) lb = atomicAdd(&count[1], (uint32_t)__builtin_popcountll(lm));
    }
    hb = (uint32_t)__shfl((int)hb, 0);
    lb = (uint32_t)__shfl((int)lb, 0);
    const uint64_t below = (1ull << lane) - 1ull;
    if (is_heavy) heavy[hb + (uint32_t)__builtin_popcountll(hm & below)] = i;
    else if (in) light[lb + (uint32_t)__builtin_popcountll(lm & below)] = i;
}

void launch_split_by_weight(const uint32_t* lens, uint32_t n, const uint32_t* ws_line, uint32_t* heavy, uint32_t* light, uint32_t* count,
                            hipStream_t s) {
    if (n == 0) return;
    hipLaunchKernelGGL(amv_split_kernel, dim3((n + 255u) / 256u), dim3(256), 0, s, lens, n, ws_line, heavy, light, count);
}

void launch_unstuff(const uint8_t* blob, uint64_t blob_bytes, const uint64_t* offs, const uint32_t* lens, uint32_t n,
                    const uint32_t* ws_line, uint32_t* ws, uint32_t* ws_bytes, uint32_t* retry_list, uint32_t* retry_count,
                    hipStream_t s) {
    if (n == 0) return;
    hipLaunchKernelGGL(amv_unstuff_kernel, dim3((n + 3u) / 4u), dim3(256), 0, s, blob, blob_bytes, offs, lens, n,
                       ws_line, ws, ws_bytes, retry_list, retry_count);
}

void launch_huffman_sync(const uint32_t* ws, const uint32_t* ws_bytes, uint32_t n, const uint32_t* list,
                         const uint32_t* list_count, const FrameGeom& g, const uint32_t* ws_line, int lanes_per_frame,
                         const HuffDecodeImage* d_img, const SyncSinks& sinks, int32_t* status, uint32_t* nmcu_ok,
                         uint32_t* queue, unsigned long long* stats, uint32_t cus, hipStream_t s) {
    if (n == 0) return;
    const uint32_t per_row = segs_per_row(g);
    SyncOut out{sinks.rec, sinks.rec_line, sinks.seg_start, sinks.lane_tab, SegGeom{g.mcu_cols, per_row, per_row * g.mcu_rows},
                sinks.lanes, sinks.rec_count, sinks.retry_list, sinks.retry_count, sinks.ok_in_blocks};
#define AMV_SYNC_ARGS ws, ws_bytes, n, list, list_count, g, ws_line, d_img, out, status, nmcu_ok, queue, stats, cus, s
    switch (lanes_per_frame) {
        case 64: launch_sync2<64>(AMV_SYNC_ARGS); break;
        case 32: launch_sync2<32>(AMV_SYNC_ARGS); break;
        case 8: launch_sync2<8>(AMV_SYNC_ARGS); break;
        case 4: launch_sync2<4>(AMV_SYNC_ARGS); break;
        case 2: launch_sync2<2>(AMV_SYNC_ARGS); break;
        case 1: launch_fast<8>(AMV_SYNC_ARGS); break;
        default: launch_sync2<16>(AMV_SYNC_ARGS); break;
    }
#undef AMV_SYNC_ARGS
}

namespace {
constexpr uint32_t kLayoutBlock = 256;

__device__ __forceinline__ uint32_t layout_lines(uint32_t len, const LayoutSpec& sp) {
    const uint64_t want = ((uint64_t)len * sp.per_byte_x2 >> 1) + sp.add;
    return (uint32_t)((min(want, (uint64_t)sp.hi) + ((1u << sp.unit_shift) - 1u)) >> sp.unit_shift);
}

struct Sum2 { uint64_t x, y; };
__device__ __forceinline__ Sum2 block_scan2(uint2 v, Sum2* s_wave, Sum2& tot) {
    const uint32_t lane = threadIdx.x & 63u, wave = threadIdx.x >> 6;
    Sum2 inc{v.x, v.y};
#pragma unroll
    for (int d = 1; d < 64; d <<= 1) {
        const uint64_t ax = (uint64_t)__shfl_up((unsigned long long)inc.x, d), ay = (uint64_t)__shfl_up((unsigned long long)inc.y, d);
        if (lane >= (uint32_t)d) { inc.x += ax; inc.y += ay; }
    }
    if (lane == 63u) s_wave[wave] = inc;
    __syncthreads();
    Sum2 base{0u, 0u};
    tot = Sum2{0u, 0u};
    for (uint32_t k = 0; k < kLayoutBlock / 64u; ++k) {
        const Sum2 w = s_wave[k];
// ... 148 lines not shown
```

### amv-codec-tools_amd/csrc/amv_reconstruct.hip

```cpp
#include "amv_block_load.h"

namespace amv {

namespace {

struct __attribute__((aligned(4))) Px12 { uint32_t w[3]; };

constexpr int kRowsPerGroup = 4;

__device__ __forceinline__ int mad24(int x, int w, int c) {
    int d;
    asm("v_mad_i32_i24 %0, %1, %2, %3" : "=v"(d) : "v"(x), "s"(w), "v"(c));
    return d;
}

enum RowKind { kRowPlain, kRow0, kRow4 };

template <bool kColumn, RowKind kKind = kRowPlain>
__device__ __forceinline__ void idct8(int& v0, int& v1, int& v2, int& v3, int& v4, int& v5, int& v6, int& v7) {
    constexpr int W1 = 2841, W2 = 2676, W3 = 2408, W5 = 1609, W6 = 1108, W7 = 565;
    constexpr int kBias = kKind == kRow0 ? 128 + 8192 : 128;
    constexpr int kRound = kColumn ? 4 : 0;
    constexpr int kDown = kColumn ? 3 : 0;
    constexpr int kOut = kColumn ? 14 : 8;
    int a0 = kColumn ? v0 : v0 * 2048 + kBias, a1 = kColumn ? v4 : v4 * 2048;
    const int i2 = v6, i3 = v2, i4 = v1, i5 = v7, i6 = v5, i7 = v3;
    int t;
    int a4 = mad24(i4, W1, mad24(i5, W7, kRound)) >> kDown;
    int a5 = mad24(i4, W7, mad24(i5, -W1, kRound)) >> kDown;
    int a6 = mad24(i6, W5, mad24(i7, W3, kRound)) >> kDown;
    int a7 = mad24(i6, W3, mad24(i7, -W5, kRound)) >> kDown;
    t = a0 + a1;
    a0 -= a1;
    int a2 = mad24(i3, W6, mad24(i2, -W2, kRound)) >> kDown;
    int a3 = mad24(i3, W2, mad24(i2, W6, kRound)) >> kDown;
    a1 = a4 + a6;
    a4 -= a6;
    a6 = a5 + a7;
    a5 -= a7;
    a7 = t + a3;
    t -= a3;
    a3 = a0 + a2;
    a0 -= a2;
    a2 = (181 * (a4 + a5) + 128) >> 8;
    a4 = (181 * (a4 - a5) + 128) >> 8;
    v0 = a7 + a1;
    v1 = a3 + a2;
    v2 = a0 + a4;
    v3 = t + a6;
    v4 = t - a6;
    v5 = a0 - a4;
    v6 = a3 - a2;
    v7 = a7 - a1;
    if (kKind == kRowPlain) {
        v0 >>= kOut; v1 >>= kOut; v2 >>= kOut; v3 >>= kOut; v4 >>= kOut; v5 >>= kOut; v6 >>= kOut; v7 >>= kOut;
    } else {
        v0 &= ~255; v1 &= ~255; v2 &= ~255; v3 &= ~255; v4 &= ~255; v5 &= ~255; v6 &= ~255; v7 &= ~255;
    }
}

struct QuantWords { uint32_t w[2][16]; };
constexpr QuantWords pack_quant() {
    QuantWords q{};
    for (int i = 0; i < 64; ++i) {
        q.w[0][i >> 2] |= (uint32_t)kQuantLuma[i] << (8 * (i & 3));
        q.w[1][i >> 2] |= (uint32_t)kQuantChroma[i] << (8 * (i & 3));
    }
    return q;
}
__device__ const QuantWords kQuantWords = pack_quant();

__device__ __forceinline__ int clamp_iclp(int x) { return min(max(x, -256), 255); }

constexpr uint32_t pair16(int lo, int hi) { return ((uint32_t)lo & 0xffffu) | ((uint32_t)hi << 16); }
__device__ __forceinline__ uint32_t dot2_bias(uint32_t a, uint32_t w) {
    uint32_t d;
    asm("v_dot2_i32_i16 %0, %1, %2, %3" : "=v"(d) : "v"(a), "s"(w), "v"(32768u));
    return d;
}

__device__ __forceinline__ uint32_t sat_pair(uint32_t yy, uint32_t cc) {
    uint32_t sum, d;
    asm("v_pk_add_i16 %0, %1, %2" : "=v"(sum) : "v"(yy), "v"(cc));
    asm("v_sat_pk_u8_i16 %0, %1" : "=v"(d) : "v"(sum));
    return d;
}

}

template <bool kRound, int kRows>
__global__ __launch_bounds__(kWave * kRows) void amv_reconstruct_kernel(
    SyncSinks in, const uint32_t* __restrict__ nmcu_ok, uint32_t n, FrameSel sel,
    FrameGeom g, PieceMap pm, uint32_t flags, uint8_t* __restrict__ out) {
    constexpr uint32_t kPitchY = kSegMcus * 16, kPitchC = kSegMcus * 8;
    __shared__ __attribute__((aligned(16))) int16_t s_all[kRows][16 * kPitchY + 2 * 8 * kPitchC + 64];
    static_assert((16 * kPitchY + 2 * 8 * kPitchC) * 2 == kSegImageBytes, "the planes reuse the image");
    const uint32_t lane = threadIdx.x & 63u, wave = (uint32_t)__builtin_amdgcn_readfirstlane((int)(threadIdx.x >> 6));
    uint32_t item, row_group, seg;
    if (!locate_piece(pm, blockIdx.x, item, row_group, seg)) return;
    const uint32_t my = row_group * kRows + wave;
    if (my >= g.mcu_rows) return;
    int16_t* const s_mem = s_all[wave];
    int16_t* const s_y = s_mem;
    int16_t* const s_u = s_mem + 16 * kPitchY;
    int16_t* const s_v = s_u + 8 * kPitchC;
    uint8_t* const s_img = reinterpret_cast<uint8_t*>(s_mem);

    uint32_t qw[16];
    {
        const uint4* q4 = reinterpret_cast<const uint4*>(kQuantWords.w[lane % 6u >= 4u ? 1 : 0]);
#pragma unroll
        for (int i = 0; i < 4; ++i) {
            const uint4 q = q4[i];
            qw[4 * i] = q.x; qw[4 * i + 1] = q.y; qw[4 * i + 2] = q.z; qw[4 * i + 3] = q.w;
        }
    }
    do {
    uint32_t f, slot;
    if (!select_frame(sel, n, item, f, slot)) return;
    const Segment sg = segment_of(f, slot, nmcu_ok, g, pm.nseg, my, seg);
    const uint32_t m0 = sg.m0, cnt = sg.cnt, ok = sg.ok, mcu0 = sg.mcu0;

    uint32_t c[32];
    bool skip;
    if (load_segment_blocks(in, sg, kRound, g, lane, s_img, c, skip)) {
        const uint32_t m = lane / 6u, k6 = lane % 6u;
        const bool chroma = k6 >= 4u;
        int v[64];
#pragma unroll
        for (int nat = 0; nat < 64; ++nat) {
            const int scan = kScanOfNatural[nat];
            v[nat] = coef_at(c, scan) * (int)((qw[scan >> 2] >> (8 * (scan & 3))) & 255u);
        }
        if (!(flags & kFlagZigzagFixed))
            v[kAmvlibQuirkNatural] = coef_at(c, kAmvlibQuirkScan) * (int)((qw[kAmvlibQuirkScan >> 2] >> (8 * (kAmvlibQuirkScan & 3))) & 255u);
#pragma unroll
        for (int r = 0; r < 8; ++r) {
            if (r == 0) idct8<false, kRow0>(v[0], v[1], v[2], v[3], v[4], v[5], v[6], v[7]);
            else if (r == 4) idct8<false, kRow4>(v[32], v[33], v[34], v[35], v[36], v[37], v[38], v[39]);
            else idct8<false>(v[8 * r], v[8 * r + 1], v[8 * r + 2], v[8 * r + 3], v[8 * r + 4], v[8 * r + 5], v[8 * r + 6], v[8 * r + 7]);
        }
#pragma unroll
        for (int col = 0; col < 8; ++col)
            idct8<true>(v[col], v[8 + col], v[16 + col], v[24 + col], v[32 + col], v[40 + col], v[48 + col], v[56 + col]);
        int16_t* dst = chroma ? (k6 == 4u ? s_u : s_v) + m * 8u
                              : s_y + ((k6 >> 1) * 8u) * kPitchY + m * 16u + (k6 & 1u) * 8u;
        const uint32_t pitch = chroma ? kPitchC : kPitchY;
#pragma unroll
        for (int r = 0; r < 8; ++r) {
            uint32_t w[4];
#pragma unroll
            for (int q = 0; q < 4; ++q) {
                const int lo = clamp_iclp(v[8 * r + 2 * q]);
                const int hi = clamp_iclp(v[8 * r + 2 * q + 1]);
                w[q] = __builtin_amdgcn_perm((uint32_t)hi, (uint32_t)lo, 0x05040100u);
            }
            *reinterpret_cast<uint4*>(dst + r * pitch) = make_uint4(w[0], w[1], w[2], w[3]);
        }
    }
    if (skip) return;
    seg_sync();

    const uint32_t vr = min(16u, g.height - my * 16u);
    const uint32_t px = min(cnt * 16u, g.width - m0 * 16u);
    const uint32_t groups = cnt * 4u;
    const bool all_decoded = mcu0 + cnt <= ok;
    const uint32_t pairs = (vr + 1u) >> 1;
    const uint32_t step_i2 = kWave / groups, step_gi = kWave - step_i2 * groups;
    uint32_t i2 = lane / groups, gi = lane - i2 * groups;
    uint8_t* const frame = out + (uint64_t)f * g.frame_bytes;
    const uint32_t row0 = (g.height - 1u - my * 16u) * g.stride + m0 * 48u;
    for (; i2 < pairs; i2 += step_i2, gi += step_gi) {
        if (gi >= groups) { gi -= groups; ++i2; if (i2 >= pairs) break; }
        const uint32_t lc = gi * 4u;
        uint2 ya = *reinterpret_cast<const uint2*>(s_y + (2u * i2) * kPitchY + lc);
        uint2 yb = *reinterpret_cast<const uint2*>(s_y + (2u * i2 + 1u) * kPitchY + lc);
        uint32_t uu = *reinterpret_cast<const uint32_t*>(s_u + i2 * kPitchC + (lc >> 1));
        uint32_t vv = *reinterpret_cast<const uint32_t*>(s_v + i2 * kPitchC + (lc >> 1));
        if (!all_decoded && (mcu0 + (gi >> 2)) >= ok) {
            constexpr uint32_t kDark = 0xfc00fc00u;
            ya.x = ya.y = yb.x = yb.y = kDark;
            uu = vv = 0u;
        }
        uint32_t cr[2], cg[2], cb[2];
#pragma unroll
        for (int e = 0; e < 2; ++e) {
            const uint32_t uv = __builtin_amdgcn_perm(vv, uu, e ? 0x07060302u : 0x05040100u);
            const uint32_t r = dot2_bias(uv, pair16(18, 367));
            const uint32_t gg = dot2_bias(uv, pair16(-159, -220));
            const uint32_t b = dot2_bias(uv, pair16(411, -29));
            cr[e] = __builtin_amdgcn_perm(r, r, 0x02010201u);
            cg[e] = __builtin_amdgcn_perm(gg, gg, 0x02010201u);
            cb[e] = __builtin_amdgcn_perm(b, b, 0x02010201u);
        }
        if (lc >= px) continue;
        uint32_t off = row0 - 2u * i2 * g.stride + lc * 3u;
#pragma unroll
        for (int row = 0; row < 2; ++row) {
            const uint2 yy = row ? yb : ya;
            const uint32_t b01 = sat_pair(yy.x, cb[0]), g01 = sat_pair(yy.x, cg[0]), r01 = sat_pair(yy.x, cr[0]);
            const uint32_t b23 = sat_pair(yy.y, cb[1]), g23 = sat_pair(yy.y, cg[1]), r23 = sat_pair(yy.y, cr[1]);
            const uint32_t gr = g01 | (r01 << 16);
            const uint32_t bg = b23 | (g23 << 16);
            Px12 v;
            v.w[0] = __builtin_amdgcn_perm(gr, b01, 0x01060400u);
            v.w[1] = __builtin_amdgcn_perm(bg, gr, 0x06040301u);
            v.w[2] = __builtin_amdgcn_perm(bg, r23, 0x01070500u);
            if (2u * i2 + (uint32_t)row >= vr) break;
            if (lc + 4u <= px) {
                *reinterpret_cast<Px12*>(frame + off) = v;
            } else {
#pragma unroll
                for (uint32_t q = 0; q < 9u; ++q)
                    if (q < (px - lc) * 3u) frame[off + q] = (uint8_t)(v.w[q >> 2] >> (8u * (q & 3u)));
            }
            off -= g.stride;
        }
    }
    } while (next_item<kRound>(pm, item));
}

template <int kRows, class... Args>
static void launch_rows(const FrameGeom& g, Args... args) {
    launch_segments(amv_reconstruct_kernel<false, kRows>, amv_reconstruct_kernel<true, kRows>, kWave * kRows, (g.mcu_rows + kRows - 1) / kRows, args...);
}

void launch_reconstruct(const SyncSinks& sinks, const uint32_t* nmcu_ok, uint32_t n, const FrameSel& sel, uint32_t items,
                        const FrameGeom& g, uint32_t flags, uint8_t* out, hipStream_t s) {
    const uint32_t slots4 = (g.mcu_rows + 3u) / 4u * 4u, slots5 = (g.mcu_rows + 4u) / 5u * 5u;
    const uint32_t waste4 = slots4 - g.mcu_rows, waste5 = slots5 - g.mcu_rows;
    if (10u * waste4 * slots5 >= 10u * waste5 * slots4 + slots4 * slots5) launch_rows<5>(g, sinks, nmcu_ok, n, sel, items, g, s, flags, out);
    else launch_rows<kRowsPerGroup>(g, sinks, nmcu_ok, n, sel, items, g, s, flags, out);
}

__global__ __launch_bounds__(kWave * 4) void amv_expand_records_kernel(SyncSinks in, const uint32_t* __restrict__ nmcu_ok, uint32_t n,
                                                                        FrameGeom g, uint32_t nseg, int16_t* __restrict__ coef) {
    __shared__ __attribute__((aligned(16))) uint8_t s_img[4][kSegImageBytes + 128];
    const uint32_t lane = threadIdx.x & 63u, wave = threadIdx.x >> 6;
    const uint32_t segs = g.mcu_rows * nseg;
    const uint64_t pairs = (uint64_t)n * segs;
    for (uint64_t p = (uint64_t)blockIdx.x * 4u + wave; p < pairs; p += (uint64_t)gridDim.x * 4u) {
        const uint32_t f = (uint32_t)(p / segs), segidx = (uint32_t)(p % segs);
        const Segment sg = segment_of(f, f, nmcu_ok, g, nseg, segidx / nseg, segidx % nseg);
        uint32_t c[32];
        bool skip;
        if (load_segment_blocks(in, sg, false, g, lane, s_img[wave], c, skip)) {
            const uint32_t blk = sg.mcu0 * 6u + lane;
            if (blk >= (in.ok_in_blocks ? sg.ok : sg.ok * 6u)) {
#pragma unroll
                for (int i = 0; i < 32; ++i) c[i] = 0u;
            }
            uint4* d = reinterpret_cast<uint4*>(coef + ((uint64_t)f * g.blocks + blk) * 64u);
#pragma unroll
            for (int i = 0; i < 8; ++i) d[i] = make_uint4(c[4 * i], c[4 * i + 1], c[4 * i + 2], c[4 * i + 3]);
        }
        seg_sync();
    }
}

void launch_expand_records(const SyncSinks& sinks, const uint32_t* nmcu_ok, uint32_t n, const FrameGeom& g, int16_t* coef,
                           hipStream_t s) {
    const uint32_t nseg = segs_per_row(g);
    const uint64_t groups = ((uint64_t)n * g.mcu_rows * nseg + 3u) / 4u;
    if (groups == 0) return;
    hipLaunchKernelGGL(amv_expand_records_kernel, dim3(groups < 65536u ? (uint32_t)groups : 65536u), dim3(kWave * 4), 0, s, sinks,
                       nmcu_ok, n, g, nseg, coef);
}

}
```

### amv-codec-tools_amd/csrc/amv_segment.h

```cpp
#pragma once
#include "amv_tables.h"
#if defined(__HIPCC__)
#define AMV_HD __host__ __device__
#else
#define AMV_HD
#endif
namespace amv {
constexpr int kWave = 64;
constexpr uint32_t kSegMcus = 10;
AMV_HD inline uint32_t segs_per_row(const FrameGeom& g) { return (g.mcu_cols + kSegMcus - 1u) / kSegMcus; }
constexpr uint32_t kDummyRecord = 0x8000u;
constexpr uint32_t kRoundWalkers = 512;
}
```

### amv-codec-tools_amd/csrc/amvhip_context.hip

```cpp
#include <stdlib.h>

#include "amvhip_ctx.h"

using namespace amv;

namespace amv {

int fail(amvhip_ctx* c, int code, const char* fmt, ...) {
    char buf[512];
    va_list ap;
    va_start(ap, fmt);
    vsnprintf(buf, sizeof buf, fmt, ap);
    va_end(ap);
    if (c) c->err = buf;
    return code;
}

int ensure(amvhip_ctx* c, DevBuf& b, size_t bytes) {
    if (bytes <= b.cap) return AMVHIP_OK;
    if (c->front) {
        HIP_TRY(c, hipStreamSynchronize(c->front));
        HIP_TRY(c, hipStreamSynchronize(c->back));
    }
    if (b.p) HIP_TRY(c, hipFree(b.p));
// ... 67 lines not shown
    if (const char* e = getenv("AMVHIP_LAYOUT")) c->layout_large = strcmp(e, "large") == 0;
    if (const char* e = getenv("AMVHIP_ADPCM_SWEEPS")) {
        if (strcmp(e, "nosettle") == 0) {
            c->adpcm_settle = false;
        } else {
            c->adpcm_sweeps_set = true;
            c->adpcm_sweeps = strcmp(e, "map") == 0 ? -1 : (atoi(e) < 0 ? 0 : (atoi(e) > 60 ? 60 : atoi(e)));
        }
    }
    if (const char* e = getenv("AMVHIP_ADPCM_TRELLIS_SWEEPS"))
        c->trellis_sweeps = strcmp(e, "map") == 0 ? -1 : (atoi(e) < 0 ? 0 : (atoi(e) > (int)kTrellisSweepsMost ? (int)kTrellisSweepsMost : atoi(e)));
}

extern "C" int amvhip_create(amvhip_ctx** out, int device) {
    if (!out) return AMVHIP_ERR_ARG;
    *out = nullptr;
    int count = 0;
    if (hipGetDeviceCount(&count) != hipSuccess || count <= 0 || device < 0 || device >= count)
        return AMVHIP_ERR_DEVICE;
    amvhip_ctx* c = new amvhip_ctx;
    c->device = device;
    static HuffDecodeImage dec;
    static HuffEncodeImage enc;
    static std::once_flag once;
    std::call_once(once, [] { build_images(dec, enc); });
    auto die = [&](int code) { amvhip_destroy(c); return code; };
    if (hipSetDevice(device) != hipSuccess) return die(AMVHIP_ERR_DEVICE);
    int cus = 0;
    if (hipDeviceGetAttribute(&cus, hipDeviceAttributeMultiprocessorCount, device) == hipSuccess && cus > 0) c->cus = (uint32_t)cus;
    read_knobs(c);
    if (hipMalloc(&c->d_dec.p, sizeof dec) != hipSuccess) return die(AMVHIP_ERR_NOMEM);
    if (hipMalloc(&c->d_enc.p, sizeof enc) != hipSuccess) return die(AMVHIP_ERR_NOMEM);
    if (hipMemcpy(c->d_dec.p, &dec, sizeof dec, hipMemcpyHostToDevice) != hipSuccess) return die(AMVHIP_ERR_DEVICE);
    if (hipMemcpy(c->d_enc.p, &enc, sizeof enc, hipMemcpyHostToDevice) != hipSuccess) return die(AMVHIP_ERR_DEVICE);
    *out = c;
    return AMVHIP_OK;
}

extern "C" void amvhip_destroy(amvhip_ctx* c) {
    if (!c) return;
    (void)hipSetDevice(c->device);
    drain(c);
    for (hipEvent_t e : c->pool) (void)hipEventDestroy(e);
    if (c->hstream) { (void)hipStreamSynchronize(c->hstream); (void)hipStreamDestroy(c->hstream); }
    if (c->dstream) { (void)hipStreamSynchronize(c->dstream); (void)hipStreamDestroy(c->dstream); }
    for (hipEvent_t e : {c->ev_decoded, c->ev_copied[0], c->ev_copied[1]})
        if (e) (void)hipEventDestroy(e);
    for (hipStream_t q : {c->front, c->back})
        if (q) { (void)hipStreamSynchronize(q); (void)hipStreamDestroy(q); }
    for (hipEvent_t e : {c->ev_in, c->ev_front, c->ev_done[0], c->ev_done[1]})
        if (e) (void)hipEventDestroy(e);
    delete c;
}

extern "C" const char* amvhip_last_error(const amvhip_ctx* c) { return c ? c->err.c_str() : "null context"; }
extern "C" int amvhip_device(const amvhip_ctx* c) { return c ? c->device : -1; }

extern "C" uint32_t amvhip_stride(uint32_t w) { return (w * 24 + 31) / 32 * 4; }
extern "C" uint64_t amvhip_frame_bytes(uint32_t w, uint32_t h) { return (uint64_t)amvhip_stride(w) * h; }
extern "C" uint64_t amvhip_yuv420_frame_bytes(uint32_t w, uint32_t h) {
    return (uint64_t)w * h + 2ull * ((w + 1) / 2) * ((h + 1) / 2);
}
extern "C" uint32_t amvhip_encode_bound(uint32_t w, uint32_t h) {
    return 4 + ((w + 15) / 16) * ((h + 15) / 16) * 6 * 64 * 4 * 2;
}

extern "C" int amvhip_sync(amvhip_ctx* c) {
    if (!c) return AMVHIP_ERR_ARG;
    if (int r = use_device(c)) return r;
    if (c->hstream) HIP_TRY(c, hipStreamSynchronize(c->hstream));
    if (c->dstream) HIP_TRY(c, hipStreamSynchronize(c->dstream));
    return AMVHIP_OK;
}

extern "C" int amvhip_host_alloc(amvhip_ctx* c, void** p, size_t bytes) {
    if (!c || !p) return AMVHIP_ERR_ARG;
    *p = nullptr;
    if (int r = use_device(c)) return r;
    HIP_TRY(c, hipHostMalloc(p, bytes ? bytes : 1, hipHostMallocDefault));
    return AMVHIP_OK;
}

extern "C" void amvhip_host_free(amvhip_ctx* c, void* p) {
    if (!c || !p) return;
    (void)hipSetDevice(c->device);
    (void)hipHostFree(p);
}

extern "C" int amvhip_synth_frames_dev(amvhip_ctx* c, uint32_t seed, uint32_t first, uint32_t n, uint32_t w,
                                       uint32_t h, uint8_t* d_rgb, void* stream) {
    if (!c) return AMVHIP_ERR_ARG;
    if (!size_ok(w, h) || (n && !d_rgb)) return fail(c, AMVHIP_ERR_ARG, "synth: bad argument");
    if (int r = use_device(c)) return r;
    {
        Timed t(c, AMVHIP_K_SYNTH, (hipStream_t)stream);
        launch_synth_frames(seed, first, n, w, h, d_rgb, (hipStream_t)stream);
    }
    return check_launch(c, "synth_frames");
}

extern "C" int amvhip_synth_audio_dev(amvhip_ctx* c, uint32_t seed, uint64_t first, uint64_t n, int16_t* d_pcm, void* stream) {
    if (!c) return AMVHIP_ERR_ARG;
    if (n && !d_pcm) return fail(c, AMVHIP_ERR_ARG, "synth: bad argument");
    if (int r = use_device(c)) return r;
    launch_synth_audio(seed, first, n, d_pcm, (hipStream_t)stream);
    return check_launch(c, "synth_audio");
}

extern "C" int amvhip_set_entropy_mode(amvhip_ctx* c, int mode) {
    if (!c || (mode != AMVHIP_ENTROPY_AUTO && mode != AMVHIP_ENTROPY_SERIAL)) return AMVHIP_ERR_ARG;
    c->entropy_mode = mode;
    return AMVHIP_OK;
}

extern "C" int amvhip_entropy_stats(amvhip_ctx* c, int enable, uint64_t out[10]) {
    if (!c) return AMVHIP_ERR_ARG;
    if (int r = use_device(c)) return r;
    std::lock_guard<std::mutex> lk(c->mu);
    if (int r = ensure(c, c->stats, amv::kStatsBytes)) return r;
    HIP_TRY(c, hipDeviceSynchronize());
    if (out) {
        if (c->want_stats) HIP_TRY(c, hipMemcpy(out, c->stats.p, 80, hipMemcpyDeviceToHost));
        else memset(out, 0, 80);
        uint32_t handed = 0;
        if (c->last_decode_retry && c->last_decode_retry->p) HIP_TRY(c, hipMemcpy(&handed, c->last_decode_retry->p, 4, hipMemcpyDeviceToHost));
        out[3] = handed;
    }
    HIP_TRY(c, hipMemset(c->stats.p, 0, enable ? amv::kStatsBytes : 128));
    c->want_stats = enable != 0;
    return AMVHIP_OK;
}

extern "C" int amvhip_entropy_trace(amvhip_ctx* c, uint64_t* out, uint32_t tasks) {
    if (!c || (tasks && !out)) return AMVHIP_ERR_ARG;
    if (int r = use_device(c)) return r;
    std::lock_guard<std::mutex> lk(c->mu);
    if (tasks > amv::kTraceTasks) tasks = amv::kTraceTasks;
    if (!c->stats.p || c->stats.cap < amv::kStatsBytes) return fail(c, AMVHIP_ERR_ARG, "entropy_trace: gathering was never switched on");
    HIP_TRY(c, hipDeviceSynchronize());
    HIP_TRY(c, hipMemcpy(out, (const uint64_t*)c->stats.p + amv::kTraceBase, (size_t)tasks * 64, hipMemcpyDeviceToHost));
    return (int)tasks;
}

extern "C" int amvhip_decode_split_stats(amvhip_ctx* c, uint32_t out[2]) {
    if (!c || !out) return AMVHIP_ERR_ARG;
    if (int r = use_device(c)) return r;
    std::lock_guard<std::mutex> lk(c->mu);
    HIP_TRY(c, hipDeviceSynchronize());
    out[0] = out[1] = 0;
    if (c->last_split && c->split.p) HIP_TRY(c, hipMemcpy(out, c->split.p, 8, hipMemcpyDeviceToHost));
    return AMVHIP_OK;
}

extern "C" void amvhip_prof_enable(amvhip_ctx* c, int on) { if (c) c->prof = on != 0; }

extern "C" void amvhip_prof_reset(amvhip_ctx* c) {
    if (!c) return;
    (void)hipSetDevice(c->device);
    drain(c);
    for (int k = 0; k < AMVHIP_K_COUNT; ++k) { c->launches[k] = 0; c->total_ms[k] = 0; }
}

extern "C" int amvhip_prof_read(amvhip_ctx* c, int kernel, uint64_t* launches, double* total_ms) {
    if (!c || kernel < 0 || kernel >= AMVHIP_K_COUNT) return AMVHIP_ERR_ARG;
    (void)hipSetDevice(c->device);
    drain(c);
    if (launches) *launches = c->launches[kernel];
    if (total_ms) *total_ms = c->total_ms[kernel];
    return AMVHIP_OK;
}

extern "C" uint32_t amvhip_jpeg_header(uint16_t height, uint16_t width, uint8_t* out, uint32_t cap) {
    std::vector<uint8_t> b;
    auto put = [&](std::initializer_list<int> v) { for (int x : v) b.push_back((uint8_t)x); };
    put({0xff, 0xd8});
    put({0xff, 0xe0, 0x00, 0x10, 'J', 'F', 'I', 'F', 0x00, 0x01, 0x01, 0x01, 0x00, 0x60, 0x00, 0x60, 0x00, 0x00});
    for (int t = 0; t < 2; ++t) {
        put({0xff, 0xdb, 0x00, 2 + 1 + 64, t});
        for (int i = 0; i < 64; ++i) b.push_back(t ? kQuantChroma[i] : kQuantLuma[i]);
    }
    put({0xff, 0xc0, 0, 17, 8, height >> 8, height & 0xff, width >> 8, width & 0xff, 3,
         1, 0x22, 0, 2, 0x11, 1, 3, 0x11, 1});
    const int order[4] = {0, 2, 1, 3};
    for (int j = 0; j < 4; ++j) {
        const int t = order[j];
        int nsym = 0;
        for (int l = 0; l < 16; ++l) nsym += kHuffCount[t][l];
        const int len = 2 + 1 + 16 + nsym;
        put({0xff, 0xc4, len >> 8, len & 0xff, ((t >= 2 ? 1 : 0) << 4) | (t & 1)});
        for (int l = 0; l < 16; ++l) b.push_back(kHuffCount[t][l]);
        const uint8_t* syms = symbols_of(t);
        for (int i = 0; i < nsym; ++i) b.push_back(syms[i]);
    }
    put({0xff, 0xda, 0, 12, 3, 1, 0x00, 2, 0x11, 3, 0x11, 0, 63, 0});
    if (out && cap >= b.size()) memcpy(out, b.data(), b.size());
    return (uint32_t)b.size();
}

extern "C" const char* amvhip_kernel_name(int kernel) {
    switch (kernel) {
        case AMVHIP_K_HUFFMAN: return "amv_huffman_fast_kernel|sync2|sync";
        case AMVHIP_K_UNSTUFF: return "amv_unstuff_kernel";
        case AMVHIP_K_HUFFMAN_SERIAL: return "amv_huffman_kernel";
        case AMVHIP_K_RECON: return "amv_reconstruct_kernel";
        case AMVHIP_K_FDCT: return "amv_forward_kernel";
        case AMVHIP_K_PACK: return "amv_encode_frame_kernel";
        case AMVHIP_K_PACK_SERIAL: return "amv_pack_kernel";
        case AMVHIP_K_COMPACT: return "amv_scan_kernel+amv_gather_kernel";
        case AMVHIP_K_ADPCM_DEC: return "amv_adpcm_decode_kernel";
        case AMVHIP_K_ADPCM_ENC: return "amv_adpcm_guess_kernel+amv_adpcm_sweep_kernel*+front+settle+check (+map, chain, encode_mapped when the chain does not settle)";
        case AMVHIP_K_SYNTH: return "amv_synth_frames_kernel";
        case AMVHIP_K_AUDIO_RESAMPLE: return "amv_audio_tiles_kernel+amv_audio_resample_kernel";
        case AMVHIP_K_PIXFMT: return "amv_pix_*_kernel";
        default: return "";
    }
}
```

### amv-codec-tools_amd/csrc/amvhip_ctx.h

```cpp
#pragma once
#include <hip/hip_runtime.h>
#include <stdarg.h>
#include <stdio.h>

#include <map>
#include <mutex>
#include <string>
#include <utility>
#include <vector>

#include "amv_host_plan.h"
#include "amv_kernels.h"
#include "amv_nr_plan.h"

namespace amv {

struct DevBuf {
    void* p = nullptr;
    size_t cap = 0;
    DevBuf() = default;
    DevBuf(const DevBuf&) = delete;
    DevBuf& operator=(const DevBuf&) = delete;
    ~DevBuf() {
        if (p) (void)hipFree(p);
    }
};

struct DecodeSet {
    DevBuf nmcu, retry, rec, rec_line, seg_start, lane_tab, rec_count;
    size_t cap() const { return nmcu.cap + retry.cap + rec.cap + rec_line.cap + seg_start.cap + lane_tab.cap + rec_count.cap; }
};

struct ProfRec {
    int kernel;
    hipEvent_t a, b;
};

}

struct amvhip_ctx {
    using DevBuf = amv::DevBuf;
    int device = 0;
    std::string err;
    DevBuf d_dec, d_enc;
    DevBuf coef, tmp, flag, map, start, enc_retry, stats, ws, ws_line, layout, ws_bytes, scaled, trellis_ws, trellis_chain, chain, split;
    DevBuf nr_ws, nr_state;
    DevBuf pix_in, pix_out, pix_dec;
    DevBuf fe_deint;
    std::map<uint64_t, DevBuf> audio_banks;
    DevBuf audio_tiles;
    amv::DecodeSet set[2];
    hipStream_t front = nullptr, back = nullptr;
    hipEvent_t ev_in = nullptr, ev_front = nullptr, ev_done[2] = {nullptr, nullptr};
    uint64_t submitted = 0, collected = 0;
    DevBuf* last_decode_retry = nullptr;
    int sync_lanes = 0;
    bool split_heavy = true;
    uint32_t heavy_lanes = 16;
    bool last_split = false;
    uint32_t cus = 256;
    bool want_stats = false;
    bool layout_large = false;
    double ws_bytes_per_frame = 0.0;
    int entropy_mode = AMVHIP_ENTROPY_AUTO;
    int adpcm_sweeps = 0;
    bool adpcm_sweeps_set = false;
    bool adpcm_settle = true;
    uint32_t chain_n = 0;
    int trellis_sweeps = (int)amv::kTrellisSweeps;
    uint32_t trellis_chain_n = 0;
    DevBuf h_in, h_offs, h_lens, h_out, h_status, h_aux, a_in, a_tab, a_out, r_in, r_tab, r_out;
    hipStream_t hstream = nullptr;
    hipStream_t dstream = nullptr;
    DevBuf v_out[2], v_status[2];
    hipEvent_t ev_decoded = nullptr, ev_copied[2] = {nullptr, nullptr};
    uint64_t async_calls = 0;
    bool prof = false;
    std::vector<amv::ProfRec> recs;
    std::vector<hipEvent_t> pool;
    uint64_t launches[AMVHIP_K_COUNT] = {};
    double total_ms[AMVHIP_K_COUNT] = {};
    std::mutex mu;
    std::mutex hmu;
};

namespace amv {

int fail(amvhip_ctx* c, int code, const char* fmt, ...);

#define HIP_TRY(ctx, expr)                                                                     \
    do {                                                                                       \
        hipError_t e_ = (expr);                                                                \
        if (e_ != hipSuccess)                                                                  \
            return fail((ctx), e_ == hipErrorOutOfMemory ? AMVHIP_ERR_NOMEM : AMVHIP_ERR_DEVICE, \
                        "%s: %s", #expr, hipGetErrorString(e_));                               \
    } while (0)

int ensure(amvhip_ctx* c, DevBuf& b, size_t bytes);
int stage(amvhip_ctx* c, DevBuf& b, size_t room, const void* src, size_t bytes, hipStream_t st);
void drain(amvhip_ctx* c);
int check_launch(amvhip_ctx* c, const char* what);
int select_device(amvhip_ctx* c);
int use_device(amvhip_ctx* c);
int host_stream(amvhip_ctx* c, hipStream_t* out);

struct Timed {
    amvhip_ctx* c;
    hipStream_t s;
    ProfRec r{};
    bool on;
    Timed(amvhip_ctx* ctx, int kernel, hipStream_t st) : c(ctx), s(st), on(ctx->prof) {
        if (!on) return;
        r.kernel = kernel;
        for (hipEvent_t* e : {&r.a, &r.b}) {
            if (!c->pool.empty()) { *e = c->pool.back(); c->pool.pop_back(); }
            else if (hipEventCreate(e) != hipSuccess) { on = false; return; }
        }
        (void)hipEventRecord(r.a, s);
    }
    ~Timed() {
        if (!on) return;
        (void)hipEventRecord(r.b, s);
        c->recs.push_back(r);
    }
};

constexpr FrameSel kAllFrames{};

inline PixPicture make_picture(const uint8_t* p0, const uint8_t* p1, const uint8_t* p2, uint32_t stride, uint32_t c_stride, uint64_t frame,
                               uint64_t c_frame) {
    return PixPicture{{const_cast<uint8_t*>(p0), const_cast<uint8_t*>(p1), const_cast<uint8_t*>(p2)}, {stride, c_stride, c_stride},
                      {frame, c_frame, c_frame}};
}

inline PixPicture tight_420(uint8_t* p, uint32_t w, uint32_t h) {
    const uint32_t cw = (w + 1) / 2, chh = (h + 1) / 2;
    const uint64_t fb = (uint64_t)w * h + 2ull * cw * chh;
    return PixPicture{{p, p + (uint64_t)w * h, p + (uint64_t)w * h + (uint64_t)cw * chh}, {w, cw, cw}, {fb, fb, fb}};
}

inline YuvSource yuv_source_of(const PixPicture& p) {
    return YuvSource{p.p[0], p.p[1], p.p[2], p.stride[0], p.stride[1], p.frame[0], p.frame[1], 0u};
}

int decode_args_ok(amvhip_ctx* c, const uint8_t* d_blob, const uint64_t* d_offs, const uint32_t* d_lens, uint32_t n, uint32_t w,
                   uint32_t h, uint32_t flags, const uint8_t* d_out, const int32_t* d_status);
int decode_core(amvhip_ctx* c, const uint8_t* d_blob, uint64_t blob_bytes, const uint64_t* d_offs, const uint32_t* d_lens,
                uint32_t n, uint32_t w, uint32_t h, uint32_t flags, uint8_t* d_out, int32_t* d_status, DecodeSet& b,
                hipStream_t front, hipStream_t back, uint32_t lowres = 0);

int pix_convert_launch(amvhip_ctx* c, int src_fmt, const PixPicture& src, int dst_fmt, const PixPicture& dst, uint32_t w, uint32_t h, uint32_t n,
                       hipStream_t st);

inline bool encode_size_ok(uint32_t w, uint32_t h, uint32_t qbias) { return size_ok(w, h) && !(w & 1) && !(h & 1) && qbias <= 255; }
int encode_scaled_tail(amvhip_ctx* c, uint32_t n, uint32_t w, uint32_t h, uint32_t qbias, uint8_t* d_blob, uint64_t blob_cap,
                       uint64_t* d_offs, uint32_t* d_lens, hipStream_t stream);
int resample_launch(amvhip_ctx* c, const PixPicture& src, uint32_t src_w, uint32_t src_h, const PixPicture& dst, uint32_t dst_w, uint32_t dst_h,
                    uint32_t n, bool to_jpeg, hipStream_t st);

}
```

### amv-codec-tools_amd/csrc/amvhip_decode.hip

```cpp
#include "amvhip_ctx.h"

using namespace amv;

struct Fallback {
    const uint32_t* list;
    const uint32_t* count;
    uint32_t items;
};

static int entropy_front(amvhip_ctx* c, const uint8_t* d_blob, uint64_t blob_bytes, const uint64_t* d_offs, const uint32_t* d_lens, uint32_t n,
                         const FrameGeom& g, SyncSinks sinks, int32_t* d_status, uint32_t* d_nmcu_ok, DevBuf& retry, hipStream_t st,
                         Fallback& fb, int lanes, int heavy_lanes, uint64_t ws_lines, const LayoutSpec& rec_layout) {
    if (c->entropy_mode == AMVHIP_ENTROPY_SERIAL || g.blocks >= 16384u) {
        HIP_TRY(c, hipMemsetAsync(sinks.rec_count, 0xff, (size_t)n * 4, st));
        fb = Fallback{nullptr, nullptr, n};
        c->last_split = false;
        return AMVHIP_OK;
    }
    if (int r = ensure(c, retry, ((size_t)n + 8) * 4)) return r;
    if (int r = ensure(c, c->ws, (size_t)ws_lines * 16 + 64)) return r;
    if (int r = ensure(c, c->ws_line, ((size_t)n + 1) * 4)) return r;
    if (int r = ensure(c, c->ws_bytes, (size_t)n * 4)) return r;
    if (int r = ensure(c, c->layout, layout_workspace(n))) return r;
    uint32_t* retry_count = (uint32_t*)retry.p;
    uint32_t* retry_list = retry_count + 8;
    sinks.retry_list = retry_list;
    sinks.retry_count = retry_count;
    launch_layout(d_lens, n, LayoutSpec{2u, 32u, 0xffffffe0u, 4u, (uint32_t)ws_lines, (uint32_t*)c->ws_line.p}, rec_layout, c->layout.p,
                  retry_count, 8u, c->layout_large, st);
    if (int r = check_launch(c, "layout")) return r;
    {
        Timed t(c, AMVHIP_K_UNSTUFF, st);
        launch_unstuff(d_blob, blob_bytes, d_offs, d_lens, n, (const uint32_t*)c->ws_line.p, (uint32_t*)c->ws.p, (uint32_t*)c->ws_bytes.p,
                       retry_list, retry_count, st);
    }
    if (int r = check_launch(c, "unstuff")) return r;
    unsigned long long* stats = c->want_stats ? (unsigned long long*)c->stats.p : nullptr;
    const HuffDecodeImage* dec = (const HuffDecodeImage*)c->d_dec.p;
    c->last_split = heavy_lanes != 0;
    if (heavy_lanes) {
        if (int r = ensure(c, c->split, ((size_t)n * 2 + 8) * 4)) return r;
        uint32_t* split_count = (uint32_t*)c->split.p;
        uint32_t *heavy = split_count + 8, *light = heavy + n;
        HIP_TRY(c, hipMemsetAsync(split_count, 0, 32, st));
        launch_split_by_weight(d_lens, n, (const uint32_t*)c->ws_line.p, heavy, light, split_count, st);
        if (int r = check_launch(c, "split")) return r;
        Timed t(c, AMVHIP_K_HUFFMAN, st);
        launch_huffman_sync((const uint32_t*)c->ws.p, (const uint32_t*)c->ws_bytes.p, n, heavy, split_count, g, (const uint32_t*)c->ws_line.p,
                            heavy_lanes, dec, sinks, d_status, d_nmcu_ok, retry_count + 2, stats, c->cus, st);
        launch_huffman_sync((const uint32_t*)c->ws.p, (const uint32_t*)c->ws_bytes.p, n, light, split_count + 1, g, (const uint32_t*)c->ws_line.p,
                            lanes, dec, sinks, d_status, d_nmcu_ok, retry_count + 1, stats, c->cus, st);
    } else {
        Timed t(c, AMVHIP_K_HUFFMAN, st);
        launch_huffman_sync((const uint32_t*)c->ws.p, (const uint32_t*)c->ws_bytes.p, n, nullptr, nullptr, g, (const uint32_t*)c->ws_line.p,
                            lanes, dec, sinks, d_status, d_nmcu_ok, retry_count + 1, stats, c->cus, st);
    }
    fb = Fallback{retry_list, retry_count, n};
    return check_launch(c, "huffman_sync");
}

struct BackHalf {
    enum Kind { kBgr, kYuv, kYuvLowres } kind;
    uint32_t flags, lowres;
    uint64_t frame_bytes;
    bool covered;
};
static BackHalf back_half(uint32_t flags, uint32_t lowres, const FrameGeom& g) {
    const bool keep = (flags & AMVHIP_FLAG_FFMPEG_KEEP) != 0;
    if (lowres)
        return {BackHalf::kYuvLowres, flags, lowres, lowres_frame_bytes(g.width, g.height, lowres), keep || lowres_store_covers_planes(g.height, lowres)};
    if (flags & AMVHIP_FLAG_FFMPEG)
        return {BackHalf::kYuv, flags, 0u, amvhip_yuv420_frame_bytes(g.width, g.height), keep || yuv_store_covers_planes(g)};
    return {BackHalf::kBgr, flags, 0u, g.frame_bytes, keep || g.stride == g.width * 3};
}

static int reconstruct_launch(amvhip_ctx* c, const SyncSinks& sinks, const uint32_t* d_nmcu_ok, uint32_t n, const FrameSel& sel,
                              uint32_t items, const FrameGeom& g, const BackHalf& bh, uint8_t* d_out, hipStream_t st) {
    Timed t(c, AMVHIP_K_RECON, st);
    switch (bh.kind) {
        case BackHalf::kYuvLowres: launch_reconstruct_yuv_lowres(sinks, d_nmcu_ok, n, sel, items, g, bh.lowres, d_out, st); break;
        case BackHalf::kYuv: launch_reconstruct_yuv(sinks, d_nmcu_ok, n, sel, items, g, bh.frame_bytes, d_out, st); break;
        case BackHalf::kBgr: launch_reconstruct(sinks, d_nmcu_ok, n, sel, items, g, bh.flags, d_out, st); break;
    }
    return check_launch(c, "reconstruct");
}

static int clear_unwritten(amvhip_ctx* c, uint32_t n, const BackHalf& bh, uint8_t* d_out, hipStream_t st) {
    if (!bh.covered) HIP_TRY(c, hipMemsetAsync(d_out, 0, bh.frame_bytes * n, st));
    return AMVHIP_OK;
}

static int reconstruct_dense(amvhip_ctx* c, const char* who, const int16_t* d_coef, const uint32_t* d_nmcu_ok, uint32_t n, uint32_t w,
                             uint32_t h, uint32_t flags, uint32_t lowres, uint8_t* d_out, void* stream) {
    if (!size_ok(w, h) || (n && (!d_coef || !d_nmcu_ok || !d_out))) return fail(c, AMVHIP_ERR_ARG, "%s: bad argument", who);
    if (((uintptr_t)d_out & 3u) || ((uintptr_t)d_coef & 15u)) return fail(c, AMVHIP_ERR_ARG, "%s: out must be 4-byte, coef 16-byte aligned", who);
    if (int r = use_device(c)) return r;
    if (n == 0) return AMVHIP_OK;
    const FrameGeom g = make_geom(w, h);
    const BackHalf bh = back_half(flags, lowres, g);
    SyncSinks sinks{};
    sinks.coef = const_cast<int16_t*>(d_coef);
    if (int r = clear_unwritten(c, n, bh, d_out, (hipStream_t)stream)) return r;
    return reconstruct_launch(c, sinks, d_nmcu_ok, n, kAllFrames, n, g, bh, d_out, (hipStream_t)stream);
}

extern "C" int amvhip_reconstruct_dev(amvhip_ctx* c, const int16_t* d_coef, const uint32_t* d_nmcu_ok, uint32_t n, uint32_t w, uint32_t h,
                                      uint32_t flags, uint8_t* d_out, void* stream) {
    if (!c) return AMVHIP_ERR_ARG;
    return reconstruct_dense(c, "reconstruct", d_coef, d_nmcu_ok, n, w, h, flags, 0u, d_out, stream);
}

int amv::decode_args_ok(amvhip_ctx* c, const uint8_t* d_blob, const uint64_t* d_offs, const uint32_t* d_lens, uint32_t n, uint32_t w,
                          uint32_t h, uint32_t flags, const uint8_t* d_out, const int32_t* d_status) {
    if (!size_ok(w, h)) return fail(c, AMVHIP_ERR_ARG, "decode: bad size %ux%u", w, h);
    if ((flags & AMVHIP_FLAG_FFMPEG_KEEP) && !(flags & AMVHIP_FLAG_FFMPEG))
        return fail(c, AMVHIP_ERR_ARG, "decode: AMVHIP_FLAG_FFMPEG_KEEP is a mode of AMVHIP_FLAG_FFMPEG");
    if (n == 0) return AMVHIP_OK;
    if (!d_blob || !d_offs || !d_lens || !d_out || !d_status) return fail(c, AMVHIP_ERR_ARG, "decode: null argument");
    if (((uintptr_t)d_blob & 3u) || ((uintptr_t)d_out & 3u)) return fail(c, AMVHIP_ERR_ARG, "decode: blob and out must be 4-byte aligned");
    return AMVHIP_OK;
}

static int entropy_records(amvhip_ctx* c, const uint8_t* d_blob, uint64_t blob_bytes, const uint64_t* d_offs, const uint32_t* d_lens,
                           uint32_t n, const FrameGeom& g, bool ok_in_blocks, int32_t* d_status, uint32_t* d_nmcu_ok, DecodeSet& b,
                           hipStream_t st, SyncSinks& sinks, Fallback& fb) {
    const EntropyPlan p = entropy_plan(n, blob_bytes, g);
    const uint32_t lanes = (uint32_t)huffman_sync_lanes(n, c->cus, c->sync_lanes, (uint64_t)g.width * g.height);
    const uint32_t heavy_lanes = lanes == 1u && c->split_heavy ? c->heavy_lanes : 0u;
    const uint32_t tab_lanes = heavy_lanes ? heavy_lanes : lanes;
    if (int r = ensure(c, b.rec, (size_t)p.cap_lines * 128 + 16)) return r;
    if (int r = ensure(c, b.rec_line, ((size_t)n + 1) * 4)) return r;
    const LayoutSpec rec_layout{4u, p.add_rec, p.hi_rec, 5u, (uint32_t)p.cap_lines, (uint32_t*)b.rec_line.p};
    if (int r = ensure(c, b.seg_start, (size_t)n * (p.segs + 1) * 8)) return r;
    if (int r = ensure(c, b.lane_tab, (size_t)n * tab_lanes * 16)) return r;
    if (int r = ensure(c, b.rec_count, (size_t)n * 4)) return r;
    sinks = SyncSinks{};
    sinks.rec = (uint32_t*)b.rec.p;
    sinks.rec_line = (const uint32_t*)b.rec_line.p;
    sinks.seg_start = (uint32_t*)b.seg_start.p;
    sinks.lane_tab = (uint32_t*)b.lane_tab.p;
    sinks.lanes = tab_lanes;
    sinks.rec_count = (uint32_t*)b.rec_count.p;
    sinks.ok_in_blocks = ok_in_blocks ? 1u : 0u;
    c->last_decode_retry = &b.retry;
    return entropy_front(c, d_blob, blob_bytes, d_offs, d_lens, n, g, sinks, d_status, d_nmcu_ok, b.retry, st, fb, (int)lanes, (int)heavy_lanes,
                         p.ws_lines, rec_layout);
}

extern "C" int amvhip_huffman_decode_dev(amvhip_ctx* c, const uint8_t* d_blob, uint64_t blob_bytes, const uint64_t* d_offs,
                                         const uint32_t* d_lens, uint32_t n, uint32_t w, uint32_t h, int16_t* d_coef, int32_t* d_status,
                                         uint32_t* d_nmcu_ok, void* stream) {
    if (!c) return AMVHIP_ERR_ARG;
    if (!size_ok(w, h) || (n && (!d_blob || !d_offs || !d_lens || !d_coef || !d_status || !d_nmcu_ok)))
        return fail(c, AMVHIP_ERR_ARG, "huffman_decode: bad argument");
    if (((uintptr_t)d_blob & 3u) || ((uintptr_t)d_coef & 15u)) return fail(c, AMVHIP_ERR_ARG, "huffman_decode: blob must be 4-byte, coef 16-byte aligned");
    if (int r = use_device(c)) return r;
    if (n == 0) return AMVHIP_OK;
    std::lock_guard<std::mutex> lk(c->mu);
    const FrameGeom g = make_geom(w, h);
    hipStream_t st = (hipStream_t)stream;
    SyncSinks sinks;
    Fallback fb;
    if (int r = entropy_records(c, d_blob, blob_bytes, d_offs, d_lens, n, g, false, d_status, d_nmcu_ok, c->set[0], st, sinks, fb))
        return r;
    if (fb.list) {
        launch_expand_records(sinks, d_nmcu_ok, n, g, d_coef, st);
        if (int r = check_launch(c, "expand_records")) return r;
    }
    {
        Timed t(c, AMVHIP_K_HUFFMAN_SERIAL, st);
        launch_huffman(d_blob, blob_bytes, d_offs, d_lens, n, g, (const HuffDecodeImage*)c->d_dec.p, d_coef, d_status, d_nmcu_ok, fb.list,
                       fb.count, 0u, fb.items, false, false, st);
    }
    return check_launch(c, "huffman");
}

int amv::decode_core(amvhip_ctx* c, const uint8_t* d_blob, uint64_t blob_bytes, const uint64_t* d_offs, const uint32_t* d_lens,
                       uint32_t n, uint32_t w, uint32_t h, uint32_t flags, uint8_t* d_out, int32_t* d_status, DecodeSet& b,
                       hipStream_t front, hipStream_t back, uint32_t lowres) {
    const FrameGeom g = make_geom(w, h);
    const BackHalf bh = back_half(flags, lowres, g);
    const uint32_t round = fallback_round(n, g, 16384u, 4u);
    if (int r = ensure(c, c->coef, (size_t)round * g.blocks * 128)) return r;
    if (int r = ensure(c, b.nmcu, (size_t)n * 4)) return r;
    uint32_t* d_nmcu = (uint32_t*)b.nmcu.p;
    SyncSinks sinks;
    Fallback fb;
    if (int r = entropy_records(c, d_blob, blob_bytes, d_offs, d_lens, n, g, (flags & AMVHIP_FLAG_FFMPEG_KEEP) != 0, d_status, d_nmcu, b, front,
                                sinks, fb))
        return r;
    sinks.coef = (int16_t*)c->coef.p;
    if (back != front) {
// ... 198 lines not shown
```

### include/amvhip.h

```cpp
#ifndef AMVHIP_H
#define AMVHIP_H

#include <stdint.h>
#include <stddef.h>
#include <stdio.h>

#ifdef __cplusplus
extern "C" {
#endif


typedef struct _amv_important_header_data {
    unsigned int dwMicroSecPerFrame;
    unsigned int dwWidth;
    unsigned int dwHeight;
    unsigned int dwSpeed;
    unsigned int dwTimeSec;
    unsigned int dwTimeMin;
    unsigned int dwTimeHour;
    unsigned short wFormatTag;
    unsigned short nChannels;
    unsigned int nSamplesPerSec;
    unsigned int nAvgBytesPerSec;
    unsigned short nBlockAlign;
    unsigned short wBitsPerSample;
    unsigned short cbSize;
    unsigned short wSamplesPerBlock;
} AMVInfo;

typedef struct _frame_buffer_struct {
    unsigned char *videobuff;
    unsigned char *audiobuff;
    unsigned int videobufflen;
    unsigned int audiobufflen;
    int framenum;
} FRAMEBUFF;

typedef struct _video_buffer_struct {
    unsigned char *fbmpdat;
    unsigned int len;
} VIDEOBUFF;

#define AUDIO_FILE_TYPE_PCM 0
#define AUDIO_FILE_TYPE_ADPCM_IMA 1
typedef struct _audio_buffer_struct {
    short *audiodata;
    unsigned int len;
} AUDIOBUFF;

typedef struct _amv_decode_struct {
    char *amvfilename;
    int opened;
    long dataseekpos;
    long fileseekpos;
    AMVInfo amvinfo;
    unsigned int currentframe;
    unsigned int totalframe;
    FRAMEBUFF framebuf;
    VIDEOBUFF videobuf;
    AUDIOBUFF audiobuf;
} AMVDecoder;

typedef struct ADPCMChannelStatus {
    int predictor;
    short int step_index;
    int step;
    int prev_sample;
} ADPCMChannelStatus;

typedef struct ADPCMContext {
    int channel;
    ADPCMChannelStatus status[2];
    short sample_buffer[32];
} ADPCMContext;

void PrepareForVideoDecode(AMVInfo *info);
int AmvJpegDecode(AMVInfo *info, FRAMEBUFF *inbuff, VIDEOBUFF *video);

int AdpcmImaDecodeFrame(ADPCMContext *c, void *data, int *data_size, unsigned char *buf, int buf_size);
int AdpcmImaEncodeFrame(ADPCMContext *c, int channels, int frame_size, unsigned char *frame,
                        int buf_size, void *data);

AMVDecoder *AmvOpen(const char *amvname);
void AmvClose(AMVDecoder *amv);
int AmvReadNextFrame(AMVDecoder *amv);
int AmvRewindFrameStart(AMVDecoder *amv);
int AmvVideoDecode(AMVDecoder *amv);
int AmvAudioDecode(AMVDecoder *amv);

void AmvJpegPutHeader(FILE *fp, unsigned short height, unsigned short width);
int AmvCreateJpegFileFromFrameBuffer(AMVDecoder *amv, const char *dirname);
int AmvCreateJpegFileFromBuffer(AMVInfo *amvinfo, FRAMEBUFF *framebuf, const char *filename);
int AmvConvertJpegFileToBmpFile(const char *jpgname, const char *bmpname);
int ConvertJpegFileToBmpFile(const char *jpgname, const char *bmpname);
int AmvCreateWavFileFromAmvFile(AMVDecoder *amv, int type, const char *wavfile);

int decode_amv_frame(const unsigned char *chunk, unsigned int len, unsigned int width,
                     unsigned int height, unsigned char *bgr_out);
int encode_amv_frame(const unsigned char *pixels, unsigned int stride, unsigned int width,
                     unsigned int height, int is_bgr, unsigned char *chunk_out, unsigned int cap);


typedef struct amvhip_ctx amvhip_ctx;

#define AMVHIP_MAX_DIM 16384
#define AMVHIP_OK 0
#define AMVHIP_ERR_ARG -1
#define AMVHIP_ERR_DEVICE -2
#define AMVHIP_ERR_NOMEM -3
#define AMVHIP_ERR_SPACE -4

#define AMVHIP_ST_FORMAT 1u
#define AMVHIP_ST_OVERRUN 2u
#define AMVHIP_ST_TRUNCATED 4u

#define AMVHIP_FLAG_ZIGZAG_FIXED 1u
#define AMVHIP_FLAG_FFMPEG 2u
#define AMVHIP_FLAG_FFMPEG_KEEP 4u

#define AMVHIP_QBIAS_AMV 0
#define AMVHIP_QBIAS_MJPEG 128

int amvhip_create(amvhip_ctx **ctx, int device);
void amvhip_destroy(amvhip_ctx *ctx);
const char *amvhip_last_error(const amvhip_ctx *ctx);
int amvhip_device(const amvhip_ctx *ctx);

uint32_t amvhip_stride(uint32_t width);
uint64_t amvhip_frame_bytes(uint32_t width, uint32_t height);
uint64_t amvhip_yuv420_frame_bytes(uint32_t width, uint32_t height);
uint32_t amvhip_encode_bound(uint32_t width, uint32_t height);
uint32_t amvhip_jpeg_header(uint16_t height, uint16_t width, uint8_t *out, uint32_t cap);

int amvhip_decode_batch_dev(amvhip_ctx *ctx, const uint8_t *d_blob, uint64_t blob_bytes,
                            const uint64_t *d_offs, const uint32_t *d_lens, uint32_t n,
                            uint32_t width, uint32_t height, uint32_t flags,
                            uint8_t *d_out, int32_t *d_status, void *stream);

int amvhip_decode_submit_dev(amvhip_ctx *ctx, const uint8_t *d_blob, uint64_t blob_bytes,
                             const uint64_t *d_offs, const uint32_t *d_lens, uint32_t n,
                             uint32_t width, uint32_t height, uint32_t flags,
                             uint8_t *d_out, int32_t *d_status, void *stream);
int amvhip_decode_collect_dev(amvhip_ctx *ctx, void *stream);

double amvhip_decode_workspace_per_frame(const amvhip_ctx *ctx);

int amvhip_decode_batch(amvhip_ctx *ctx, const uint8_t *blob, uint64_t blob_bytes,
                        const uint64_t *offs, const uint32_t *lens, uint32_t n,
                        uint32_t width, uint32_t height, uint32_t flags,
                        uint8_t *out, int32_t *status);

int amvhip_decode_batch_async(amvhip_ctx *ctx, const uint8_t *blob, uint64_t blob_bytes,
                              const uint64_t *offs, const uint32_t *lens, uint32_t n,
                              uint32_t width, uint32_t height, uint32_t flags,
                              uint8_t *out, int32_t *status);
int amvhip_sync(amvhip_ctx *ctx);
int amvhip_host_alloc(amvhip_ctx *ctx, void **p, size_t bytes);
void amvhip_host_free(amvhip_ctx *ctx, void *p);

#define AMVHIP_ENTROPY_AUTO 0
#define AMVHIP_ENTROPY_SERIAL 1
int amvhip_set_entropy_mode(amvhip_ctx *ctx, int mode);
int amvhip_entropy_stats(amvhip_ctx *ctx, int enable, uint64_t out[10]);
int amvhip_entropy_trace(amvhip_ctx *ctx, uint64_t *out, uint32_t tasks);
int amvhip_decode_split_stats(amvhip_ctx *ctx, uint32_t out[2]);

int amvhip_huffman_decode_dev(amvhip_ctx *ctx, const uint8_t *d_blob, uint64_t blob_bytes,
                              const uint64_t *d_offs, const uint32_t *d_lens, uint32_t n,
                              uint32_t width, uint32_t height,
                              int16_t *d_coef, int32_t *d_status, uint32_t *d_nmcu_ok, void *stream);
int amvhip_reconstruct_dev(amvhip_ctx *ctx, const int16_t *d_coef, const uint32_t *d_nmcu_ok,
                           uint32_t n, uint32_t width, uint32_t height, uint32_t flags,
                           uint8_t *d_out, void *stream);

int amvhip_encode_batch_dev(amvhip_ctx *ctx, const uint8_t *d_pix, uint32_t pix_stride, int is_bgr,
                            uint32_t n, uint32_t width, uint32_t height, uint32_t qbias,
                            uint8_t *d_blob, uint64_t blob_cap, uint64_t *d_offs, uint32_t *d_lens,
                            void *stream);
int amvhip_encode_batch(amvhip_ctx *ctx, const uint8_t *pix, uint32_t pix_stride, int is_bgr,
                        uint32_t n, uint32_t width, uint32_t height, uint32_t qbias,
                        uint8_t *blob, uint64_t blob_cap, uint64_t *offs, uint32_t *lens);
int amvhip_encode_yuv420_batch_dev(amvhip_ctx *ctx, const uint8_t *d_y, const uint8_t *d_cb, const uint8_t *d_cr,
                                   uint32_t y_stride, uint32_t c_stride, uint64_t y_frame_stride,
                                   uint64_t c_frame_stride, uint32_t n, uint32_t width, uint32_t height,
                                   uint32_t qbias, uint8_t *d_blob, uint64_t blob_cap, uint64_t *d_offs,
                                   uint32_t *d_lens, void *stream);
int amvhip_encode_yuv420_batch(amvhip_ctx *ctx, const uint8_t *y, const uint8_t *cb, const uint8_t *cr,
                               uint32_t y_stride, uint32_t c_stride, uint64_t y_frame_stride,
                               uint64_t c_frame_stride, uint32_t n, uint32_t width, uint32_t height,
                               uint32_t qbias, uint8_t *blob, uint64_t blob_cap, uint64_t *offs, uint32_t *lens);
uint32_t amvhip_encode_nr_max(uint32_t width, uint32_t height);
int amvhip_encode_yuv420_nr_stream_dev(amvhip_ctx *ctx, const uint8_t *d_y, const uint8_t *d_cb, const uint8_t *d_cr,
                                       uint32_t y_stride, uint32_t c_stride, uint64_t y_frame_stride,
                                       uint64_t c_frame_stride, uint32_t n, uint32_t width, uint32_t height,
                                       uint32_t qbias, uint32_t nr, int32_t *d_state, uint8_t *d_blob, uint64_t blob_cap,
                                       uint64_t *d_offs, uint32_t *d_lens, void *stream);
int amvhip_encode_yuv420_nr_stream(amvhip_ctx *ctx, const uint8_t *y, const uint8_t *cb, const uint8_t *cr,
                                   uint32_t y_stride, uint32_t c_stride, uint64_t y_frame_stride,
                                   uint64_t c_frame_stride, uint32_t n, uint32_t width, uint32_t height,
                                   uint32_t qbias, uint32_t nr, int32_t *state, uint8_t *blob, uint64_t blob_cap,
                                   uint64_t *offs, uint32_t *lens);
int amvhip_encode_nr_stream_dev(amvhip_ctx *ctx, const uint8_t *d_pix, uint32_t pix_stride, int is_bgr,
                                uint32_t n, uint32_t width, uint32_t height, uint32_t qbias, uint32_t nr,
                                int32_t *d_state, uint8_t *d_blob, uint64_t blob_cap, uint64_t *d_offs,
                                uint32_t *d_lens, void *stream);
int amvhip_encode_nr_stream(amvhip_ctx *ctx, const uint8_t *pix, uint32_t pix_stride, int is_bgr,
                            uint32_t n, uint32_t width, uint32_t height, uint32_t qbias, uint32_t nr,
                            int32_t *state, uint8_t *blob, uint64_t blob_cap, uint64_t *offs, uint32_t *lens);
int amvhip_encode_yuv422_batch_dev(amvhip_ctx *ctx, const uint8_t *d_y, const uint8_t *d_cb, const uint8_t *d_cr,
                                   uint32_t y_stride, uint32_t c_stride, uint64_t y_frame_stride,
                                   uint64_t c_frame_stride, uint32_t n, uint32_t width, uint32_t height,
                                   uint32_t qbias, uint8_t *d_blob, uint64_t blob_cap, uint64_t *d_offs,
                                   uint32_t *d_lens, void *stream);
int amvhip_encode_yuv422_batch(amvhip_ctx *ctx, const uint8_t *y, const uint8_t *cb, const uint8_t *cr,
                               uint32_t y_stride, uint32_t c_stride, uint64_t y_frame_stride,
                               uint64_t c_frame_stride, uint32_t n, uint32_t width, uint32_t height,
                               uint32_t qbias, uint8_t *blob, uint64_t blob_cap, uint64_t *offs, uint32_t *lens);
int amvhip_resample_yuv420_dev(amvhip_ctx *ctx, const uint8_t *d_src_y, const uint8_t *d_src_cb, const uint8_t *d_src_cr,
                               uint32_t src_y_stride, uint32_t src_c_stride, uint64_t src_y_frame_stride,
                               uint64_t src_c_frame_stride, uint32_t src_width, uint32_t src_height,
                               uint8_t *d_dst_y, uint8_t *d_dst_cb, uint8_t *d_dst_cr,
                               uint32_t dst_y_stride, uint32_t dst_c_stride, uint64_t dst_y_frame_stride,
                               uint64_t dst_c_frame_stride, uint32_t dst_width, uint32_t dst_height, uint32_t n, void *stream);
int amvhip_encode_yuv420_scaled_batch_dev(amvhip_ctx *ctx, const uint8_t *d_y, const uint8_t *d_cb, const uint8_t *d_cr,
                                          uint32_t y_stride, uint32_t c_stride, uint64_t y_frame_stride,
                                          uint64_t c_frame_stride, uint32_t src_width, uint32_t src_height, uint32_t n,
                                          uint32_t width, uint32_t height, uint32_t qbias, uint8_t *d_blob,
                                          uint64_t blob_cap, uint64_t *d_offs, uint32_t *d_lens, void *stream);
#define AMVHIP_PIX_YUV420P 0
#define AMVHIP_PIX_YUVJ420P 1
#define AMVHIP_PIX_YUV422P 2
#define AMVHIP_PIX_YUVJ422P 3
#define AMVHIP_PIX_YUV444P 4
#define AMVHIP_PIX_YUVJ444P 5
#define AMVHIP_PIX_YUYV422 6
#define AMVHIP_PIX_UYVY422 7
#define AMVHIP_PIX_RGB24 8
#define AMVHIP_PIX_BGR24 9
#define AMVHIP_PIX_RGB32 10
#define AMVHIP_PIX_RGB565 11
#define AMVHIP_PIX_RGB555 12
#define AMVHIP_PIX_GRAY8 13
#define AMVHIP_PIX_COUNT 14
int amvhip_img_convert_supported(int src_fmt, int dst_fmt, uint32_t width, uint32_t height);
uint64_t amvhip_pix_frame_bytes(int fmt, uint32_t stride, uint32_t height);
int amvhip_img_convert_dev(amvhip_ctx *ctx, int src_fmt, const uint8_t *d_src0, const uint8_t *d_src1, const uint8_t *d_src2,
                           uint32_t src_stride, uint32_t src_c_stride, uint64_t src_frame_stride, uint64_t src_c_frame_stride,
                           int dst_fmt, uint8_t *d_dst0, uint8_t *d_dst1, uint8_t *d_dst2,
                           uint32_t dst_stride, uint32_t dst_c_stride, uint64_t dst_frame_stride, uint64_t dst_c_frame_stride,
                           uint32_t width, uint32_t height, uint32_t n, void *stream);
int amvhip_img_convert(amvhip_ctx *ctx, int src_fmt, const uint8_t *src0, const uint8_t *src1, const uint8_t *src2,
                       uint32_t src_stride, uint32_t src_c_stride, uint64_t src_frame_stride, uint64_t src_c_frame_stride,
                       int dst_fmt, uint8_t *dst0, uint8_t *dst1, uint8_t *dst2,
                       uint32_t dst_stride, uint32_t dst_c_stride, uint64_t dst_frame_stride, uint64_t dst_c_frame_stride,
                       uint32_t width, uint32_t height, uint32_t n);
int amvhip_sws_scale_dev(amvhip_ctx *ctx, int src_fmt, const uint8_t *d_src0, const uint8_t *d_src1, const uint8_t *d_src2,
                         uint32_t src_stride, uint32_t src_c_stride, uint64_t src_frame_stride, uint64_t src_c_frame_stride,
                         uint32_t src_width, uint32_t src_height,
                         int dst_fmt, uint8_t *d_dst0, uint8_t *d_dst1, uint8_t *d_dst2,
                         uint32_t dst_stride, uint32_t dst_c_stride, uint64_t dst_frame_stride, uint64_t dst_c_frame_stride,
                         uint32_t dst_width, uint32_t dst_height, uint32_t n, void *stream);
int amvhip_encode_fmt_scaled_batch_dev(amvhip_ctx *ctx, int src_fmt, const uint8_t *d_src0, const uint8_t *d_src1, const uint8_t *d_src2,
                                       uint32_t src_stride, uint32_t src_c_stride, uint64_t src_frame_stride,
                                       uint64_t src_c_frame_stride, uint32_t src_width, uint32_t src_height, uint32_t n,
                                       uint32_t width, uint32_t height, uint32_t qbias, uint8_t *d_blob, uint64_t blob_cap,
                                       uint64_t *d_offs, uint32_t *d_lens, void *stream);
typedef struct amvhip_frontend {
    uint32_t deinterlace;
    uint32_t crop_top, crop_bottom, crop_left, crop_right;
    uint32_t pad_top, pad_bottom, pad_left, pad_right;
    uint8_t pad_color[3];
} amvhip_frontend;
void amvhip_pad_color_from_rgb(uint32_t rrggbb, uint8_t out[3]);
int amvhip_deinterlace_supported(int fmt, uint32_t width, uint32_t height);
int amvhip_deinterlace_dev(amvhip_ctx *ctx, int fmt, const uint8_t *d_src0, const uint8_t *d_src1, const uint8_t *d_src2,
                           uint32_t src_stride, uint32_t src_c_stride, uint64_t src_frame_stride, uint64_t src_c_frame_stride,
                           uint8_t *d_dst0, uint8_t *d_dst1, uint8_t *d_dst2,
                           uint32_t dst_stride, uint32_t dst_c_stride, uint64_t dst_frame_stride, uint64_t dst_c_frame_stride,
                           uint32_t width, uint32_t height, uint32_t n, void *stream);
int amvhip_deinterlace(amvhip_ctx *ctx, int fmt, const uint8_t *src0, const uint8_t *src1, const uint8_t *src2,
                       uint32_t src_stride, uint32_t src_c_stride, uint64_t src_frame_stride, uint64_t src_c_frame_stride,
                       uint8_t *dst0, uint8_t *dst1, uint8_t *dst2,
                       uint32_t dst_stride, uint32_t dst_c_stride, uint64_t dst_frame_stride, uint64_t dst_c_frame_stride,
                       uint32_t width, uint32_t height, uint32_t n);
int amvhip_video_frontend_dev(amvhip_ctx *ctx, int src_fmt, const uint8_t *d_src0, const uint8_t *d_src1, const uint8_t *d_src2,
                              uint32_t src_stride, uint32_t src_c_stride, uint64_t src_frame_stride, uint64_t src_c_frame_stride,
                              uint32_t src_width, uint32_t src_height, uint32_t n, const amvhip_frontend *fe,
                              uint8_t *d_y, uint8_t *d_cb, uint8_t *d_cr, uint32_t y_stride, uint32_t c_stride,
                              uint64_t y_frame_stride, uint64_t c_frame_stride, uint32_t width, uint32_t height, void *stream);
int amvhip_encode_frontend_batch_dev(amvhip_ctx *ctx, int src_fmt, const uint8_t *d_src0, const uint8_t *d_src1, const uint8_t *d_src2,
                                     uint32_t src_stride, uint32_t src_c_stride, uint64_t src_frame_stride,
                                     uint64_t src_c_frame_stride, uint32_t src_width, uint32_t src_height, uint32_t n,
                                     const amvhip_frontend *fe, uint32_t width, uint32_t height, uint32_t qbias, uint8_t *d_blob,
                                     uint64_t blob_cap, uint64_t *d_offs, uint32_t *d_lens, void *stream);
int amvhip_decode_fmt_batch_dev(amvhip_ctx *ctx, const uint8_t *d_blob, uint64_t blob_bytes,
                                const uint64_t *d_offs, const uint32_t *d_lens, uint32_t n,
                                uint32_t width, uint32_t height, uint32_t flags, int dst_fmt,
                                uint8_t *d_out, uint32_t out_stride, int32_t *d_status, void *stream);
uint32_t amvhip_lowres_dim(uint32_t full, uint32_t lowres);
uint64_t amvhip_lowres_frame_bytes(uint32_t width, uint32_t height, uint32_t lowres);
int amvhip_decode_lowres_batch_dev(amvhip_ctx *ctx, const uint8_t *d_blob, uint64_t blob_bytes,
                                   const uint64_t *d_offs, const uint32_t *d_lens, uint32_t n,
                                   uint32_t width, uint32_t height, uint32_t flags, uint32_t lowres, int dst_fmt,
                                   uint8_t *d_out, uint32_t out_stride, int32_t *d_status, void *stream);
int amvhip_decode_lowres_batch(amvhip_ctx *ctx, const uint8_t *blob, uint64_t blob_bytes,
                               const uint64_t *offs, const uint32_t *lens, uint32_t n,
                               uint32_t width, uint32_t height, uint32_t flags, uint32_t lowres, int dst_fmt,
                               uint8_t *out, uint32_t out_stride, int32_t *status);
int amvhip_reconstruct_lowres_dev(amvhip_ctx *ctx, const int16_t *d_coef, const uint32_t *d_nmcu_ok, uint32_t n,
                                  uint32_t width, uint32_t height, uint32_t lowres, uint8_t *d_out, void *stream);
#define AMVHIP_AUDIO_RATE_MIN 1000
#define AMVHIP_AUDIO_RATE_MAX 192000
uint64_t amvhip_audio_resample_out_samples(uint32_t in_rate, uint32_t out_rate, uint64_t in_samples);
int amvhip_audio_resample_batch_dev(amvhip_ctx *ctx, const int16_t *d_pcm, const uint64_t *d_pcm_offs, const uint64_t *d_nsamp,
                                    uint32_t n, uint32_t in_channels, uint32_t in_rate, int16_t *d_out,
                                    const uint64_t *d_out_offs, uint32_t out_channels, uint32_t out_rate, void *stream);
int amvhip_audio_resample_batch(amvhip_ctx *ctx, const int16_t *pcm, uint64_t pcm_samples, const uint64_t *pcm_offs,
                                const uint64_t *nsamp, uint32_t n, uint32_t in_channels, uint32_t in_rate, int16_t *out,
// ... 87 lines not shown
```

Before: 29.79 million frames/s.

## Mark big-AC frames in Huffman pass and use packed 16-bit row IDCT

The Huffman sync decoder now tracks the largest AC size code seen per frame using an SDWA max, and flags frames whose coefficients exceed a threshold in the record count high bit, counting them atomically. The reconstruct kernel reads that flag and, for unflagged frames, runs a new packed path: coefficients are dequantized as 16-bit pairs and the row IDCT uses dot2_i16 and mad24 instructions, while flagged frames keep the general 32-bit path. This aims to cut row-IDCT ALU work and register pressure for typical blocks, at the cost of extra branching, an atomic per flagged frame and a new diagnostic API.

New measurement: 29.69 million frames/s. No clear change (-0.3%).

```diff
diff --git a/amv-codec-tools_amd/__init__.py b/amv-codec-tools_amd/__init__.py
--- a/amv-codec-tools_amd/__init__.py
+++ b/amv-codec-tools_amd/__init__.py
@@ -158,6 +158,7 @@
     "amvhip_entropy_stats": (_int, [_vp, _int, _vp]),
     "amvhip_entropy_trace": (_int, [_vp, _vp, _u32]),
     "amvhip_decode_split_stats": (_int, [_vp, _vp]),
+    "amvhip_decode_marked_frames": (_int, [_vp, _vp]),
     "amvhip_adpcm_chain_stats": (_int, [_vp, _vp]),
     "amvhip_adpcm_quotient_table": (None, [_vp]),
     "amvhip_prof_enable": (None, [_vp, _int]),
@@ -499,6 +500,11 @@
         self._check(self.lib.amvhip_decode_split_stats(self.h, out), "decode_split_stats")
         return {"heavy": int(out[0]), "light": int(out[1])}
 
+    def decode_marked_frames(self):
+        out = ctypes.c_uint32(0)
+        self._check(self.lib.amvhip_decode_marked_frames(self.h, ctypes.byref(out)), "decode_marked_frames")
+        return int(out.value)
+
     def adpcm_chain_stats(self):
         out = (ctypes.c_uint32 * 64)()
         self._check(self.lib.amvhip_adpcm_chain_stats(self.h, out), "adpcm_chain_stats")
diff --git a/amv-codec-tools_amd/build.py b/amv-codec-tools_amd/build.py
--- a/amv-codec-tools_amd/build.py
+++ b/amv-codec-tools_amd/build.py
@@ -12,7 +12,7 @@
 HIP_SOURCES = ["csrc/amv_decode.hip", "csrc/amv_decode_sync.hip", "csrc/amv_reconstruct.hip", "csrc/amv_reconstruct_ff.hip", "csrc/amv_reconstruct_lowres.hip", "csrc/amv_encode.hip", "csrc/amv_encode_par.hip", "csrc/amv_encode_nr.hip", "csrc/amv_resample.hip", "csrc/amv_pixfmt.hip", "csrc/amv_frontend.hip", "csrc/amv_audio_resample.hip", "csrc/amv_adpcm.hip", "csrc/amv_synth.hip",
                "csrc/amvhip_context.hip", "csrc/amvhip_decode.hip", "csrc/amvhip_encode.hip", "csrc/amvhip_pixfmt.hip", "csrc/amvhip_audio.hip"]
 C_SOURCES = ["host/amvlib_compat.c", "host/amv_container.c"]
-HEADERS = ["csrc/amv_tables.h", "csrc/amv_kernels.h", "csrc/amv_block_load.h", "csrc/amv_piece_map.h", "csrc/amv_segment.h", "csrc/amv_ff_dequant.h", "csrc/amv_encode_common.h", "csrc/amv_host_plan.h", "csrc/amv_nr_plan.h",
+HEADERS = ["csrc/amv_tables.h", "csrc/amv_kernels.h", "csrc/amv_block_load.h", "csrc/amv_piece_map.h", "csrc/amv_segment.h", "csrc/amv_idct_rows.h", "csrc/amv_ff_dequant.h", "csrc/amv_encode_common.h", "csrc/amv_host_plan.h", "csrc/amv_nr_plan.h",
            "csrc/amvhip_ctx.h", "../include/amvhip.h"]
 
 HIPFLAGS = ["-O3", "-std=c++17", "-fPIC", "-fwrapv", "-fno-strict-aliasing", f"--offload-arch={ARCH}",
diff --git a/amv-codec-tools_amd/csrc/amv_block_load.h b/amv-codec-tools_amd/csrc/amv_block_load.h
--- a/amv-codec-tools_amd/csrc/amv_block_load.h
+++ b/amv-codec-tools_amd/csrc/amv_block_load.h
@@ -43,9 +43,13 @@
     return true;
 }
 
-__device__ __forceinline__ bool load_segment_blocks(const SyncSinks& in, const Segment& sg, bool dense_only, const FrameGeom& g,
-                                                    uint32_t lane, uint8_t* s_img, uint32_t (&c)[32], bool& skip) {
-    const uint32_t f = sg.f, slot = sg.slot, segidx = sg.segidx, nsegs = sg.nsegs, mcu0 = sg.mcu0, cnt = sg.cnt, ok = sg.ok;
+struct BlockAt {
+    bool records;
+    int dc_base;
+};
+__device__ __forceinline__ bool place_segment_blocks(const SyncSinks& in, const Segment& sg, bool dense_only, const FrameGeom& g,
+                                                     uint32_t lane, uint8_t* s_img, BlockAt& where, bool& skip, uint32_t& big_ac) {
+    const uint32_t f = sg.f, segidx = sg.segidx, nsegs = sg.nsegs, mcu0 = sg.mcu0, cnt = sg.cnt, ok = sg.ok;
     const uint32_t nb = cnt * 6u;
     uint32_t rc = 0xffffffffu, r0 = 0u, r1 = 0u;
     if (in.rec != nullptr && !dense_only) {
@@ -55,6 +59,9 @@
         r1 = ss[3];
     }
     const bool records = rc != 0xffffffffu;
+    big_ac = (uint32_t)__builtin_amdgcn_readfirstlane((int)(rc & kRecBigAc));
+    where.records = records;
+    where.dc_base = 0;
     skip = !records && in.rec != nullptr && !dense_only;
     if (skip) return false;
     int dc_base = 0;
@@ -124,8 +131,15 @@
         }
         seg_sync();
     }
-    if (lane >= nb) return false;
-    if (records) {
+    where.dc_base = dc_base;
+    return lane < nb;
+}
+
+__device__ __forceinline__ void read_block(const SyncSinks& in, const Segment& sg, const FrameGeom& g, uint32_t lane, const uint8_t* s_img,
+                                           const BlockAt& where, uint32_t (&c)[32]) {
+    const uint32_t slot = sg.slot, mcu0 = sg.mcu0;
+    const int dc_base = where.dc_base;
+    if (where.records) {
         const uint4* src = reinterpret_cast<const uint4*>(s_img) + lane * 8u;
         const uint32_t swz = (lane + mcu0 * 6u - g.blocks) & 7u;
 #pragma unroll
@@ -142,7 +156,20 @@
             c[4 * i] = q.x; c[4 * i + 1] = q.y; c[4 * i + 2] = q.z; c[4 * i + 3] = q.w;
         }
     }
+}
+
+__device__ __forceinline__ bool load_segment_blocks(const SyncSinks& in, const Segment& sg, bool dense_only, const FrameGeom& g,
+                                                    uint32_t lane, uint8_t* s_img, uint32_t (&c)[32], bool& skip, uint32_t& big_ac) {
+    BlockAt where;
+    if (!place_segment_blocks(in, sg, dense_only, g, lane, s_img, where, skip, big_ac)) return false;
+    read_block(in, sg, g, lane, s_img, where, c);
     return true;
+}
+
+__device__ __forceinline__ bool load_segment_blocks(const SyncSinks& in, const Segment& sg, bool dense_only, const FrameGeom& g,
+                                                    uint32_t lane, uint8_t* s_img, uint32_t (&c)[32], bool& skip) {
+    uint32_t big_ac;
+    return load_segment_blocks(in, sg, dense_only, g, lane, s_img, c, skip, big_ac);
 }
 
 __device__ __forceinline__ int coef_at(const uint32_t (&c)[32], int i) {
diff --git a/amv-codec-tools_amd/csrc/amv_decode_sync.hip b/amv-codec-tools_amd/csrc/amv_decode_sync.hip
--- a/amv-codec-tools_amd/csrc/amv_decode_sync.hip
+++ b/amv-codec-tools_amd/csrc/amv_decode_sync.hip
@@ -321,6 +321,12 @@
     return e1 | e2;
 }
 
+__device__ __forceinline__ uint32_t max_low_byte(uint32_t e, uint32_t seen) {
+    uint32_t d;
+    asm("v_max_u32_sdwa %0, %1, %2 dst_sel:DWORD dst_unused:UNUSED_PAD src0_sel:BYTE_0 src1_sel:DWORD" : "=v"(d) : "v"(e), "v"(seen));
+    return d;
+}
+
 template <uint32_t kFlush, bool kLimit>
 __device__ __forceinline__ void fast_stride(uint32_t ringb, uint32_t stageb, uint32_t sumb, uint32_t lim1, FastState& s, uint32_t& seen,
                                             uint32_t& worst) {
@@ -333,7 +339,7 @@
         uint32_t run = (uint32_t)((int32_t)s.togo6 >> 31);
         if (kLimit) run &= (uint32_t)((int32_t)(s.t - lim1) >> 31);
         const uint32_t e = fast_lookup(s, v) & run;
-        seen |= e;
+        seen = max_low_byte(e, seen);
         const uint32_t used = e >> 24;
         const int x = __builtin_amdgcn_sbfe((int)v, 0u - used, e);
         const uint32_t full = __builtin_amdgcn_ubfe(0xffffffffu, 0u, e);
@@ -468,7 +474,7 @@
 
         FastState s{0xffffffffu, 0u, 5u, live ? 0u - (blocks_per_frame << 6) : 0u, 0u, ~0u};
         bool alive = live;
-        uint32_t stop = 0;
+        uint32_t seen = 0u;
         uint32_t stride_no = 0;
         bool have_words = true;
         uint32_t recpos = 0;
@@ -485,18 +491,18 @@
                 const bool running = alive;
                 s.rp8 = stride_no << 11;
                 const FastState start = s;
-                uint32_t worst = ~0u, seen = 0u;
+                uint32_t worst = ~0u;
                 fast_stride<kFlush, false>(ringb, stageb, sumb, 0u, s, seen, worst);
                 const bool trouble = alive && (worst < 15u || (seen & kFastInvalid) != 0u);
                 if (__ballot(trouble) != 0ull) {
                     if (trouble) {
                         s = start;
-                        stop = fast_replay<false>(ringb, 0u, s);
+                        seen |= fast_replay<false>(ringb, 0u, s) << 8;
                         alive = false;
                         for (uint32_t q = s.rp8 >> 8; q < stride_no * 8u + 8u; ++q) stage_put<kFlush>(stage, q, kDummyRecord);
                     }
                 }
-                if (alive && s.togo6 == 0u) { stop = 3u; alive = false; }
+                if (alive && s.togo6 == 0u) { seen |= 3u << 8; alive = false; }
                 stage_put<kFlush>(stage, s.rp8 >> 8, kDummyRecord);
                 {
                     uint32_t* p = stage + ((stride_no & 1u) * kFlush) * kWave;
@@ -533,6 +539,7 @@
             }
         } while (__ballot(alive) != 0ull);
         if (live) {
+            const uint32_t stop = seen >> 8;
             const uint32_t bits = s.t + 1u + (stop == 1u ? 17u : 0u);
             uint32_t st = stop == 1u ? kStFormat : (stop == 2u ? kStOverrun : 0u);
             if (bits > valid_bits) st |= kStTruncated;
@@ -545,7 +552,9 @@
             } else {
                 status[frame] = (int32_t)st;
                 nmcu_ok[frame] = out.ok_in_blocks ? end_blocks : end_blocks / 6u;
-                out.rec_count[frame] = recpos;
+                const bool big = (seen & 255u) >= kBigAcSize;
+                if (big) atomicAdd(out.retry_count + kBigAcCounter, 1u);
+                out.rec_count[frame] = recpos | (big ? kRecBigAc : 0u);
             }
         }
     }
@@ -776,7 +785,7 @@
         if (!alive) s.togo6 = 0u;
         const uint32_t wlim1 = sub == L - 1 ? kNoLimit : (sub + 1u) * S - 1u;
         const uint32_t dc_first = blk0 + (s.k ? 1u : 0u);
-        uint32_t stop = 0;
+        uint32_t seen = 0u;
         uint32_t flushed = rec0;
         uint32_t end_blocks = 0;
         uint32_t seg_next, seg_col, seg_blk;
@@ -801,17 +810,17 @@
             }
             const bool running = alive;
             const FastState start = s;
-            uint32_t worst = ~0u, seen = 0u;
+            uint32_t worst = ~0u;
             fast_stride<kFlush, true>(ringb, stageb, sumb, wlim1, s, seen, worst);
             const bool trouble = alive && (worst < 15u || (seen & kFastInvalid) != 0u);
             if (__ballot(trouble) != 0ull) {
                 if (trouble) {
                     s = start;
-                    stop = fast_replay<true>(ringb, wlim1, s);
+                    seen |= fast_replay<true>(ringb, wlim1, s) << 8;
                     alive = false;
                 }
             }
-            if (alive && s.togo6 == 0u) { stop = 3u; alive = false; }
+            if (alive && s.togo6 == 0u) { seen |= 3u << 8; alive = false; }
             if (alive && (int32_t)(s.t - wlim1) >= 0) alive = false;
             bool hit = false;
             if (running) {
@@ -830,6 +839,7 @@
         } while (__ballot(alive) != 0ull);
         }
         const uint32_t recpos = s.rp8 >> 8;
+        const uint32_t stop = seen >> 8;
         {
             const uint32_t end = (recpos + kFlush - 1u) & ~(kFlush - 1u);
             for (uint32_t q = recpos; q < end; ++q) stage_put<kFlush>(stage, q, kDummyRecord);
@@ -842,8 +852,10 @@
         const uint32_t err = stop == 1u ? kStFormat : (stop == 2u ? kStOverrun : 0u);
         const uint32_t stop_p = s.t + 1u + (stop == 1u ? 17u : 0u);
         const uint64_t stop_mask = __ballot(stop != 0u) & seg;
+        const uint64_t big_mask = __ballot((seen & 255u) >= kBigAcSize) & seg;
         uint32_t st = 0, good_blocks = blocks_per_frame, rec_total = 0, seg_seen = 0;
         int stop_lane = 0;
+        bool big = big_mask != 0ull;
         if (stop_mask) {
             stop_lane = __builtin_ctzll(stop_mask);
             const uint32_t e = __shfl(err, stop_lane);
@@ -851,6 +863,7 @@
             const uint32_t sp = __shfl(stop_p, stop_lane);
             rec_total = __shfl(recpos, stop_lane);
             seg_seen = __shfl(seg_next, stop_lane);
+            big = (big_mask & ((2ull << stop_lane) - 1ull)) != 0ull;
             st = e;
             if (e) good_blocks = eb;
             if (sp > valid_bits) st |= kStTruncated;
@@ -897,7 +910,8 @@
             } else {
                 status[frame] = (int32_t)st;
                 nmcu_ok[frame] = out.ok_in_blocks ? good_blocks : good_blocks / 6u;
-                out.rec_count[frame] = rec_total | ((uint32_t)(L - 1) << 24);
+                if (big) atomicAdd(out.retry_count + kBigAcCounter, 1u);
+                out.rec_count[frame] = rec_total | ((uint32_t)(L - 1) << 24) | (big ? kRecBigAc : 0u);
             }
         }
     }
diff --git a/amv-codec-tools_amd/csrc/amv_idct_rows.h b/amv-codec-tools_amd/csrc/amv_idct_rows.h
--- /dev/null
+++ b/amv-codec-tools_amd/csrc/amv_idct_rows.h
@@ -0,0 +1,160 @@
+#pragma once
+#include "amv_tables.h"
+
+namespace amv {
+
+constexpr uint32_t pair16(int lo, int hi) { return ((uint32_t)lo & 0xffffu) | ((uint32_t)hi << 16); }
+
+#if defined(__HIPCC__)
+#define AMV_ROWS __device__ __forceinline__
+#define AMV_ROWS_UNROLL _Pragma("unroll")
+AMV_ROWS int mad24(int x, int w, int c) {
+    int d;
+    asm("v_mad_i32_i24 %0, %1, %2, %3" : "=v"(d) : "v"(x), "s"(w), "v"(c));
+    return d;
+}
+template <int kC>
+AMV_ROWS int mad24c(int x, int w) {
+    static_assert(kC >= 0 && kC <= 64, "an inline constant");
+    int d;
+    asm("v_mad_i32_i24 %0, %1, %2, %3" : "=v"(d) : "v"(x), "s"(w), "n"(kC));
+    return d;
+}
+AMV_ROWS int dot2_i16(uint32_t a, uint32_t w) {
+    int d;
+    asm("v_dot2_i32_i16 %0, %1, %2, 0" : "=v"(d) : "v"(a), "s"(w));
+    return d;
+}
+AMV_ROWS uint32_t pk_mul_lo16(uint32_t a, uint32_t b) {
+    uint32_t d;
+    asm("v_pk_mul_lo_u16 %0, %1, %2" : "=v"(d) : "v"(a), "v"(b));
+    return d;
+}
+AMV_ROWS uint32_t perm_bytes(uint32_t hi, uint32_t lo, uint32_t sel) { return __builtin_amdgcn_perm(hi, lo, sel); }
+#else
+#define AMV_ROWS static inline
+#define AMV_ROWS_UNROLL
+AMV_ROWS int mad24(int x, int w, int c) { return (int)((uint32_t)x * (uint32_t)w + (uint32_t)c); }
+template <int kC>
+AMV_ROWS int mad24c(int x, int w) { return mad24(x, w, kC); }
+AMV_ROWS int dot2_i16(uint32_t a, uint32_t w) {
+    return (int)((uint32_t)((int)(int16_t)(a & 0xffffu) * (int)(int16_t)(w & 0xffffu)) + (uint32_t)((int)(int16_t)(a >> 16) * (int)(int16_t)(w >> 16)));
+}
+AMV_ROWS uint32_t pk_mul_lo16(uint32_t a, uint32_t b) {
+    return (((a & 0xffffu) * (b & 0xffffu)) & 0xffffu) | (((a >> 16) * (b >> 16)) << 16);
+}
+AMV_ROWS uint32_t perm_bytes(uint32_t hi, uint32_t lo, uint32_t sel) {
+    const uint64_t both = ((uint64_t)hi << 32) | lo;
+    uint32_t d = 0;
+    for (int q = 0; q < 4; ++q) d |= (uint32_t)((both >> (8u * ((sel >> (8 * q)) & 7u))) & 255u) << (8 * q);
+    return d;
+}
+#endif
+
+enum RowKind { kRowPlain, kRow0, kRow4 };
+
+constexpr int kW1 = 2841, kW2 = 2676, kW3 = 2408, kW5 = 1609, kW6 = 1108, kW7 = 565;
+
+template <bool kColumn, RowKind kKind>
+AMV_ROWS void idct8_tail(int a0, int a1, int a2, int a3, int a4, int a5, int a6, int a7,
+                         int& v0, int& v1, int& v2, int& v3, int& v4, int& v5, int& v6, int& v7) {
+    constexpr int kOut = kColumn ? 14 : 8;
+    int t = a0 + a1;
+    a0 -= a1;
+    a1 = a4 + a6;
+    a4 -= a6;
+    a6 = a5 + a7;
+    a5 -= a7;
+    a7 = t + a3;
+    t -= a3;
+    a3 = a0 + a2;
+    a0 -= a2;
+    a2 = (181 * (a4 + a5) + 128) >> 8;
+    a4 = (181 * (a4 - a5) + 128) >> 8;
+    v0 = a7 + a1;
+    v1 = a3 + a2;
+    v2 = a0 + a4;
+    v3 = t + a6;
+    v4 = t - a6;
+    v5 = a0 - a4;
+    v6 = a3 - a2;
+    v7 = a7 - a1;
+    if (kKind == kRowPlain) {
+        v0 >>= kOut; v1 >>= kOut; v2 >>= kOut; v3 >>= kOut; v4 >>= kOut; v5 >>= kOut; v6 >>= kOut; v7 >>= kOut;
+    } else {
+        v0 &= ~255; v1 &= ~255; v2 &= ~255; v3 &= ~255; v4 &= ~255; v5 &= ~255; v6 &= ~255; v7 &= ~255;
+    }
+}
+
+template <bool kColumn, RowKind kKind = kRowPlain>
+AMV_ROWS void idct8(int& v0, int& v1, int& v2, int& v3, int& v4, int& v5, int& v6, int& v7) {
+    constexpr int kBias = kKind == kRow0 ? 128 + 8192 : 128;
+    constexpr int kRound = kColumn ? 4 : 0;
+    constexpr int kDown = kColumn ? 3 : 0;
+    const int a0 = kColumn ? v0 : v0 * 2048 + kBias, a1 = kColumn ? v4 : v4 * 2048;
+    const int i2 = v6, i3 = v2, i4 = v1, i5 = v7, i6 = v5, i7 = v3;
+    const int a4 = mad24(i4, kW1, mad24c<kRound>(i5, kW7)) >> kDown;
+    const int a5 = mad24(i4, kW7, mad24c<kRound>(i5, -kW1)) >> kDown;
+    const int a6 = mad24(i6, kW5, mad24c<kRound>(i7, kW3)) >> kDown;
+    const int a7 = mad24(i6, kW3, mad24c<kRound>(i7, -kW5)) >> kDown;
+    const int a2 = mad24(i3, kW6, mad24c<kRound>(i2, -kW2)) >> kDown;
+    const int a3 = mad24(i3, kW2, mad24c<kRound>(i2, kW6)) >> kDown;
+    idct8_tail<kColumn, kKind>(a0, a1, a2, a3, a4, a5, a6, a7, v0, v1, v2, v3, v4, v5, v6, v7);
+}
+
+
+struct QuantPairs { uint32_t w[2][32]; };
+constexpr QuantPairs pack_quant_pairs() {
+    QuantPairs q{};
+    for (int i = 0; i < 64; ++i) {
+        q.w[0][i >> 1] |= (uint32_t)kQuantLuma[i] << (16 * (i & 1));
+        q.w[1][i >> 1] |= (uint32_t)kQuantChroma[i] << (16 * (i & 1));
+    }
+    return q;
+}
+
+struct RowIn {
+    int x0, x4;
+    uint32_t p17, p53, p26;
+};
+
+AMV_ROWS int half_at(const uint32_t (&d)[32], int scan) {
+    return (scan & 1) ? ((int)d[scan >> 1] >> 16) : (int)(int16_t)(d[scan >> 1] & 0xffffu);
+}
+AMV_ROWS uint32_t pair_at(const uint32_t (&d)[32], int sa, int sb) {
+    if ((sa >> 1) == (sb >> 1) && !(sa & 1) && (sb & 1)) return d[sa >> 1];
+    const uint32_t la = 2u * (uint32_t)(sa & 1), hb = 4u + 2u * (uint32_t)(sb & 1);
+    return perm_bytes(d[sb >> 1], d[sa >> 1], la | ((la + 1u) << 8) | (hb << 16) | ((hb + 1u) << 24));
+}
+
+AMV_ROWS void dequant_pairs(const uint32_t (&c)[32], const uint32_t (&qp)[32], uint32_t (&d)[32], int& dc) {
+    AMV_ROWS_UNROLL
+    for (int i = 0; i < 32; ++i) d[i] = pk_mul_lo16(c[i], qp[i]);
+    dc = (int)(int16_t)(c[0] & 0xffffu) * (int)(qp[0] & 0xffffu);
+}
+AMV_ROWS RowIn row_in(const uint32_t (&d)[32], int dc, int r, bool zigzag_fixed) {
+    const uint8_t* sc = kScanOfNatural + 8 * r;
+    RowIn in;
+    in.x0 = r == 0 ? dc : half_at(d, sc[0]);
+    in.x4 = half_at(d, sc[4]);
+    if (8 * r + 4 == kAmvlibQuirkNatural && !zigzag_fixed) in.x4 = half_at(d, kAmvlibQuirkScan);
+    in.p17 = pair_at(d, sc[1], sc[7]);
+    in.p53 = pair_at(d, sc[5], sc[3]);
+    in.p26 = pair_at(d, sc[2], sc[6]);
+    return in;
+}
+
+template <RowKind kKind>
+AMV_ROWS void idct_row_packed(const RowIn& in, int& v0, int& v1, int& v2, int& v3, int& v4, int& v5, int& v6, int& v7) {
+    constexpr int kBias = kKind == kRow0 ? 128 + 8192 : 128;
+    const int a0 = in.x0 * 2048 + kBias, a1 = in.x4 * 2048;
+    const int a4 = dot2_i16(in.p17, pair16(kW1, kW7));
+    const int a5 = dot2_i16(in.p17, pair16(kW7, -kW1));
+    const int a6 = dot2_i16(in.p53, pair16(kW5, kW3));
+    const int a7 = dot2_i16(in.p53, pair16(kW3, -kW5));
+    const int a2 = dot2_i16(in.p26, pair16(kW6, -kW2));
+    const int a3 = dot2_i16(in.p26, pair16(kW2, kW6));
+    idct8_tail<false, kKind>(a0, a1, a2, a3, a4, a5, a6, a7, v0, v1, v2, v3, v4, v5, v6, v7);
+}
+
+}
diff --git a/amv-codec-tools_amd/csrc/amv_reconstruct.hip b/amv-codec-tools_amd/csrc/amv_reconstruct.hip
--- a/amv-codec-tools_amd/csrc/amv_reconstruct.hip
+++ b/amv-codec-tools_amd/csrc/amv_reconstruct.hip
@@ -1,4 +1,5 @@
 #include "amv_block_load.h"
+#include "amv_idct_rows.h"
 
 namespace amv {
 
@@ -7,57 +8,6 @@
 struct __attribute__((aligned(4))) Px12 { uint32_t w[3]; };
 
 constexpr int kRowsPerGroup = 4;
-
-__device__ __forceinline__ int mad24(int x, int w, int c) {
-    int d;
-    asm("v_mad_i32_i24 %0, %1, %2, %3" : "=v"(d) : "v"(x), "s"(w), "v"(c));
-    return d;
-}
-
-enum RowKind { kRowPlain, kRow0, kRow4 };
-
-template <bool kColumn, RowKind kKind = kRowPlain>
-__device__ __forceinline__ void idct8(int& v0, int& v1, int& v2, int& v3, int& v4, int& v5, int& v6, int& v7) {
-    constexpr int W1 = 2841, W2 = 2676, W3 = 2408, W5 = 1609, W6 = 1108, W7 = 565;
-    constexpr int kBias = kKind == kRow0 ? 128 + 8192 : 128;
-    constexpr int kRound = kColumn ? 4 : 0;
-    constexpr int kDown = kColumn ? 3 : 0;
-    constexpr int kOut = kColumn ? 14 : 8;
-    int a0 = kColumn ? v0 : v0 * 2048 + kBias, a1 = kColumn ? v4 : v4 * 2048;
-    const int i2 = v6, i3 = v2, i4 = v1, i5 = v7, i6 = v5, i7 = v3;
-    int t;
-    int a4 = mad24(i4, W1, mad24(i5, W7, kRound)) >> kDown;
-    int a5 = mad24(i4, W7, mad24(i5, -W1, kRound)) >> kDown;
-    int a6 = mad24(i6, W5, mad24(i7, W3, kRound)) >> kDown;
-    int a7 = mad24(i6, W3, mad24(i7, -W5, kRound)) >> kDown;
-    t = a0 + a1;
-    a0 -= a1;
-    int a2 = mad24(i3, W6, mad24(i2, -W2, kRound)) >> kDown;
-    int a3 = mad24(i3, W2, mad24(i2, W6, kRound)) >> kDown;
-    a1 = a4 + a6;
-    a4 -= a6;
-    a6 = a5 + a7;
-    a5 -= a7;
-    a7 = t + a3;
-    t -= a3;
-    a3 = a0 + a2;
-    a0 -= a2;
-    a2 = (181 * (a4 + a5) + 128) >> 8;
-    a4 = (181 * (a4 - a5) + 128) >> 8;
-    v0 = a7 + a1;
-    v1 = a3 + a2;
-    v2 = a0 + a4;
-    v3 = t + a6;
-    v4 = t - a6;
-    v5 = a0 - a4;
-    v6 = a3 - a2;
-    v7 = a7 - a1;
-    if (kKind == kRowPlain) {
-        v0 >>= kOut; v1 >>= kOut; v2 >>= kOut; v3 >>= kOut; v4 >>= kOut; v5 >>= kOut; v6 >>= kOut; v7 >>= kOut;
-    } else {
-        v0 &= ~255; v1 &= ~255; v2 &= ~255; v3 &= ~255; v4 &= ~255; v5 &= ~255; v6 &= ~255; v7 &= ~255;
-    }
-}
 
 struct QuantWords { uint32_t w[2][16]; };
 constexpr QuantWords pack_quant() {
@@ -69,10 +19,10 @@
     return q;
 }
 __device__ const QuantWords kQuantWords = pack_quant();
+__device__ const QuantPairs kQuantPairs = pack_quant_pairs();
 
 __device__ __forceinline__ int clamp_iclp(int x) { return min(max(x, -256), 255); }
 
-constexpr uint32_t pair16(int lo, int hi) { return ((uint32_t)lo & 0xffffu) | ((uint32_t)hi << 16); }
 __device__ __forceinline__ uint32_t dot2_bias(uint32_t a, uint32_t w) {
     uint32_t d;
     asm("v_dot2_i32_i16 %0, %1, %2, %3" : "=v"(d) : "v"(a), "s"(w), "v"(32768u));
@@ -107,12 +57,21 @@
     uint8_t* const s_img = reinterpret_cast<uint8_t*>(s_mem);
 
     uint32_t qw[16];
-    {
-        const uint4* q4 = reinterpret_cast<const uint4*>(kQuantWords.w[lane % 6u >= 4u ? 1 : 0]);
+    const auto load_qw = [&](const uint4* q4) {
 #pragma unroll
         for (int i = 0; i < 4; ++i) {
             const uint4 q = q4[i];
             qw[4 * i] = q.x; qw[4 * i + 1] = q.y; qw[4 * i + 2] = q.z; qw[4 * i + 3] = q.w;
+        }
+    };
+    if (kRound) load_qw(reinterpret_cast<const uint4*>(kQuantWords.w[lane % 6u >= 4u ? 1 : 0]));
+    uint32_t qp[32];
+    if (!kRound) {
+        const uint4* q4 = reinterpret_cast<const uint4*>(kQuantPairs.w[lane % 6u >= 4u ? 1 : 0]);
+#pragma unroll
+        for (int i = 0; i < 8; ++i) {
+            const uint4 q = q4[i];
+            qp[4 * i] = q.x; qp[4 * i + 1] = q.y; qp[4 * i + 2] = q.z; qp[4 * i + 3] = q.w;
         }
     }
     do {
@@ -121,41 +80,74 @@
     const Segment sg = segment_of(f, slot, nmcu_ok, g, pm.nseg, my, seg);
     const uint32_t m0 = sg.m0, cnt = sg.cnt, ok = sg.ok, mcu0 = sg.mcu0;
 
-    uint32_t c[32];
     bool skip;
-    if (load_segment_blocks(in, sg, kRound, g, lane, s_img, c, skip)) {
+    uint32_t big_ac;
+    BlockAt where;
+    const bool have = place_segment_blocks(in, sg, kRound, g, lane, s_img, where, skip, big_ac);
+    const bool packed = !kRound && !big_ac;
+    {
         const uint32_t m = lane / 6u, k6 = lane % 6u;
         const bool chroma = k6 >= 4u;
-        int v[64];
-#pragma unroll
-        for (int nat = 0; nat < 64; ++nat) {
-            const int scan = kScanOfNatural[nat];
-            v[nat] = coef_at(c, scan) * (int)((qw[scan >> 2] >> (8 * (scan & 3))) & 255u);
-        }
-        if (!(flags & kFlagZigzagFixed))
-            v[kAmvlibQuirkNatural] = coef_at(c, kAmvlibQuirkScan) * (int)((qw[kAmvlibQuirkScan >> 2] >> (8 * (kAmvlibQuirkScan & 3))) & 255u);
-#pragma unroll
-        for (int r = 0; r < 8; ++r) {
-            if (r == 0) idct8<false, kRow0>(v[0], v[1], v[2], v[3], v[4], v[5], v[6], v[7]);
-            else if (r == 4) idct8<false, kRow4>(v[32], v[33], v[34], v[35], v[36], v[37], v[38], v[39]);
-            else idct8<false>(v[8 * r], v[8 * r + 1], v[8 * r + 2], v[8 * r + 3], v[8 * r + 4], v[8 * r + 5], v[8 * r + 6], v[8 * r + 7]);
-        }
-#pragma unroll
-        for (int col = 0; col < 8; ++col)
-            idct8<true>(v[col], v[8 + col], v[16 + col], v[24 + col], v[32 + col], v[40 + col], v[48 + col], v[56 + col]);
-        int16_t* dst = chroma ? (k6 == 4u ? s_u : s_v) + m * 8u
-                              : s_y + ((k6 >> 1) * 8u) * kPitchY + m * 16u + (k6 & 1u) * 8u;
-        const uint32_t pitch = chroma ? kPitchC : kPitchY;
-#pragma unroll
-        for (int r = 0; r < 8; ++r) {
-            uint32_t w[4];
-#pragma unroll
-            for (int q = 0; q < 4; ++q) {
-                const int lo = clamp_iclp(v[8 * r + 2 * q]);
-                const int hi = clamp_iclp(v[8 * r + 2 * q + 1]);
-                w[q] = __builtin_amdgcn_perm((uint32_t)hi, (uint32_t)lo, 0x05040100u);
-            }
-            *reinterpret_cast<uint4*>(dst + r * pitch) = make_uint4(w[0], w[1], w[2], w[3]);
+        const auto columns_and_planes = [&](int (&v)[64]) {
+#pragma unroll
+            for (int col = 0; col < 8; ++col)
+                idct8<true>(v[col], v[8 + col], v[16 + col], v[24 + col], v[32 + col], v[40 + col], v[48 + col], v[56 + col]);
+            int16_t* dst = chroma ? (k6 == 4u ? s_u : s_v) + m * 8u
+                                  : s_y + ((k6 >> 1) * 8u) * kPitchY + m * 16u + (k6 & 1u) * 8u;
+            const uint32_t pitch = chroma ? kPitchC : kPitchY;
+#pragma unroll
+            for (int r = 0; r < 8; ++r) {
+                uint32_t w[4];
+#pragma unroll
+                for (int q = 0; q < 4; ++q) {
+                    const int lo = clamp_iclp(v[8 * r + 2 * q]);
+                    const int hi = clamp_iclp(v[8 * r + 2 * q + 1]);
+                    w[q] = __builtin_amdgcn_perm((uint32_t)hi, (uint32_t)lo, 0x05040100u);
+                }
+                *reinterpret_cast<uint4*>(dst + r * pitch) = make_uint4(w[0], w[1], w[2], w[3]);
+            }
+        };
+        if (have && packed) {
+            uint32_t c[32], d[32];
+            int dc, v[64];
+            read_block(in, sg, g, lane, s_img, where, c);
+            dequant_pairs(c, qp, d, dc);
+#pragma unroll
+            for (int r = 0; r < 8; ++r) {
+                const RowIn in = row_in(d, dc, r, (flags & kFlagZigzagFixed) != 0u);
+                int* o = v + 8 * r;
+                if (r == 0) idct_row_packed<kRow0>(in, o[0], o[1], o[2], o[3], o[4], o[5], o[6], o[7]);
+                else if (r == 4) idct_row_packed<kRow4>(in, o[0], o[1], o[2], o[3], o[4], o[5], o[6], o[7]);
+                else idct_row_packed<kRowPlain>(in, o[0], o[1], o[2], o[3], o[4], o[5], o[6], o[7]);
+            }
+            columns_and_planes(v);
+            asm volatile("; stage B, packed: end" ::: "memory");
+        }
+        if (have && !packed) {
+            uint32_t c[32];
+            int v[64];
+            read_block(in, sg, g, lane, s_img, where, c);
+            if (!kRound) {
+                const uint4* q4 = reinterpret_cast<const uint4*>(kQuantWords.w[chroma ? 1 : 0]);
+                asm volatile("" : "+v"(q4));
+                load_qw(q4);
+            }
+            const auto step_at = [&](int scan) { return (int)((qw[scan >> 2] >> (8 * (scan & 3))) & 255u); };
+#pragma unroll
+            for (int nat = 0; nat < 64; ++nat) {
+                const int scan = kScanOfNatural[nat];
+                v[nat] = coef_at(c, scan) * step_at(scan);
+            }
+            if (!(flags & kFlagZigzagFixed))
+                v[kAmvlibQuirkNatural] = coef_at(c, kAmvlibQuirkScan) * step_at(kAmvlibQuirkScan);
+#pragma unroll
+            for (int r = 0; r < 8; ++r) {
+                if (r == 0) idct8<false, kRow0>(v[0], v[1], v[2], v[3], v[4], v[5], v[6], v[7]);
+                else if (r == 4) idct8<false, kRow4>(v[32], v[33], v[34], v[35], v[36], v[37], v[38], v[39]);
+                else idct8<false>(v[8 * r], v[8 * r + 1], v[8 * r + 2], v[8 * r + 3], v[8 * r + 4], v[8 * r + 5], v[8 * r + 6], v[8 * r + 7]);
+            }
+            columns_and_planes(v);
+            asm volatile("; stage B, general: end" ::: "memory");
         }
     }
     if (skip) return;
diff --git a/amv-codec-tools_amd/csrc/amv_segment.h b/amv-codec-tools_amd/csrc/amv_segment.h
--- a/amv-codec-tools_amd/csrc/amv_segment.h
+++ b/amv-codec-tools_amd/csrc/amv_segment.h
@@ -10,5 +10,8 @@
 constexpr uint32_t kSegMcus = 10;
 AMV_HD inline uint32_t segs_per_row(const FrameGeom& g) { return (g.mcu_cols + kSegMcus - 1u) / kSegMcus; }
 constexpr uint32_t kDummyRecord = 0x8000u;
+constexpr uint32_t kRecBigAc = 1u << 31;
+constexpr uint32_t kBigAcSize = 10u;
+constexpr uint32_t kBigAcCounter = 3u;
 constexpr uint32_t kRoundWalkers = 512;
 }
diff --git a/amv-codec-tools_amd/csrc/amvhip_context.hip b/amv-codec-tools_amd/csrc/amvhip_context.hip
--- a/amv-codec-tools_amd/csrc/amvhip_context.hip
+++ b/amv-codec-tools_amd/csrc/amvhip_context.hip
@@ -243,6 +243,17 @@
     return AMVHIP_OK;
 }
 
+extern "C" int amvhip_decode_marked_frames(amvhip_ctx* c, uint32_t* out) {
+    if (!c || !out) return AMVHIP_ERR_ARG;
+    if (int r = use_device(c)) return r;
+    std::lock_guard<std::mutex> lk(c->mu);
+    HIP_TRY(c, hipDeviceSynchronize());
+    *out = 0;
+    if (c->last_marks && c->last_decode_retry && c->last_decode_retry->p)
+        HIP_TRY(c, hipMemcpy(out, (const uint32_t*)c->last_decode_retry->p + amv::kBigAcCounter, 4, hipMemcpyDeviceToHost));
+    return AMVHIP_OK;
+}
+
 extern "C" void amvhip_prof_enable(amvhip_ctx* c, int on) { if (c) c->prof = on != 0; }
 
 extern "C" void amvhip_prof_reset(amvhip_ctx* c) {
diff --git a/amv-codec-tools_amd/csrc/amvhip_ctx.h b/amv-codec-tools_amd/csrc/amvhip_ctx.h
--- a/amv-codec-tools_amd/csrc/amvhip_ctx.h
+++ b/amv-codec-tools_amd/csrc/amvhip_ctx.h
@@ -57,6 +57,7 @@
     int sync_lanes = 0;
     bool split_heavy = true;
     uint32_t heavy_lanes = 16;
+    bool last_marks = false;
     bool last_split = false;
     uint32_t cus = 256;
     bool want_stats = false;
diff --git a/amv-codec-tools_amd/csrc/amvhip_decode.hip b/amv-codec-tools_amd/csrc/amvhip_decode.hip
--- a/amv-codec-tools_amd/csrc/amvhip_decode.hip
+++ b/amv-codec-tools_amd/csrc/amvhip_decode.hip
@@ -15,6 +15,7 @@
         HIP_TRY(c, hipMemsetAsync(sinks.rec_count, 0xff, (size_t)n * 4, st));
         fb = Fallback{nullptr, nullptr, n};
         c->last_split = false;
+        c->last_marks = false;
         return AMVHIP_OK;
     }
     if (int r = ensure(c, retry, ((size_t)n + 8) * 4)) return r;
@@ -38,6 +39,7 @@
     unsigned long long* stats = c->want_stats ? (unsigned long long*)c->stats.p : nullptr;
     const HuffDecodeImage* dec = (const HuffDecodeImage*)c->d_dec.p;
     c->last_split = heavy_lanes != 0;
+    c->last_marks = true;
     if (heavy_lanes) {
         if (int r = ensure(c, c->split, ((size_t)n * 2 + 8) * 4)) return r;
         uint32_t* split_count = (uint32_t*)c->split.p;
diff --git a/include/amvhip.h b/include/amvhip.h
--- a/include/amvhip.h
+++ b/include/amvhip.h
@@ -164,6 +164,7 @@
 int amvhip_entropy_stats(amvhip_ctx *ctx, int enable, uint64_t out[10]);
 int amvhip_entropy_trace(amvhip_ctx *ctx, uint64_t *out, uint32_t tasks);
 int amvhip_decode_split_stats(amvhip_ctx *ctx, uint32_t out[2]);
+int amvhip_decode_marked_frames(amvhip_ctx *ctx, uint32_t *out);
 
 int amvhip_huffman_decode_dev(amvhip_ctx *ctx, const uint8_t *d_blob, uint64_t blob_bytes,
                               const uint64_t *d_offs, const uint32_t *d_lens, uint32_t n,
```
